# TheBinaryCodeX/RayMarchRenderer

Hardware: AMD Instinct MI355X
Metric: Msamples/sec (pixels×spp) at 1920×1080; PSNR vs GLSL reference (higher is better)
Workload: dtype f32; 1 GPU; C2 Cornell-5 SDF (RayMarch.glsl semantics) 1920x1080 64 spp 4 bounces; config=c2, width=1920, height=1080, spp=64, max_bounces=4, tile=32, tile_order=rows, parallelism=tiles1, frame_streams=2, grid_reserve=64, launch_streams=0

## Files before the change

include/rmr.h:

```cpp
#ifndef RMR_H
#define RMR_H

#include <stddef.h>
#include <stdint.h>
#include "rmr_tables.h"

#ifdef __cplusplus
extern "C" {
#endif

#define RMR_OK          0
#define RMR_E_INVALID  (-1)
#define RMR_E_HIP      (-2)
#define RMR_E_SCENE    (-3)
#define RMR_E_IO       (-4)
#define RMR_E_STATE    (-5)
#define RMR_E_NOMEM    (-6)
#define RMR_E_UNSUPPORTED (-7)

typedef struct rmr_ctx rmr_ctx;

typedef struct rmr_params {
    float   max_dist;
    int32_t max_steps;
// ... 174 lines not shown
int rmr_read_tonemapped(rmr_ctx* ctx, float* rgba, size_t bytes);
void* rmr_tonemapped_device_ptr(rmr_ctx* ctx);
int rmr_read_exposure(rmr_ctx* ctx, double* log2_scale, float* scale);
int rmr_luminance_histogram(rmr_ctx* ctx, int source, uint32_t hist[256], uint64_t* skipped);
int rmr_tonemap_reset(rmr_ctx* ctx);
int rmr_luminance_bins(const float* rgba, size_t n, int32_t* bins);
int rmr_exposure_from_histogram(const uint32_t hist[256], const rmr_tonemap_params* p, double l_prev, double* l_out);
int rmr_tonemap_pixels(const rmr_tonemap_params* p, float scale, const float* rgba, size_t n, float* out);

#define RMR_OUTPUT_BLOOM 4
typedef struct rmr_bloom_params {
    int32_t levels;
    float threshold;
    float clamp;
    float scatter;
    float intensity;
    int32_t reserved[3];
} rmr_bloom_params;
void rmr_default_bloom_params(rmr_bloom_params* p);
int rmr_check_bloom_params(const rmr_bloom_params* p);
int rmr_bloom(rmr_ctx* ctx, int source, const rmr_bloom_params* p);
int rmr_read_bloom(rmr_ctx* ctx, float* rgba, size_t bytes);
void* rmr_bloom_device_ptr(rmr_ctx* ctx);
int rmr_bloom_pixels(const rmr_bloom_params* p, const float* rgba, int w, int h, float* out);

typedef struct rmr_ray {
    float   o[3], time;
    float   d[3], rc;
    int32_t gx, gy;
} rmr_ray;

#define RMR_CAMERA_VIEW 0
#define RMR_CAMERA_THIN_LENS 1
#define RMR_CAMERA_EQUIRECT 2
#define RMR_CAMERA_ORTHO 3
typedef struct rmr_camera_model {
    int32_t model;
    float   aperture;
    float   focus;
    float   width;
    float   height;
} rmr_camera_model;
void rmr_default_camera_model(rmr_camera_model* m);
int rmr_check_camera_model(const rmr_camera_model* m);
int rmr_set_camera_model(rmr_ctx* ctx, const rmr_camera_model* m);
int rmr_get_camera_model(const rmr_ctx* ctx, rmr_camera_model* m);
int rmr_camera_frame(const float view[15], float out[9]);
int rmr_check_rays(const rmr_ray* rays, size_t n);
int rmr_trace_rays(rmr_ctx* ctx, const rmr_ray* rays, size_t n, float* out_rgba);
int rmr_camera_rays(rmr_ctx* ctx, const float* times, uint32_t nspp, int x0, int y0, int x1, int y1, rmr_ray* out);

typedef struct rmr_hit {
    float pos[3], t;
    float n[3], id;
} rmr_hit;
#define RMR_CAST_NORMALS 1
int rmr_cast_rays(rmr_ctx* ctx, const rmr_ray* rays, size_t n, int flags, rmr_hit* out);
int rmr_eval_map(rmr_ctx* ctx, const float* xyz, size_t n, float* out_dist_id);
int rmr_trace_rays_device(rmr_ctx* ctx, const rmr_ray* d_rays, size_t n, float origin_extent, float* d_out_rgba);
int rmr_cast_rays_device(rmr_ctx* ctx, const rmr_ray* d_rays, size_t n, int flags, rmr_hit* d_out);
int rmr_eval_map_device(rmr_ctx* ctx, const float* d_xyz, size_t n, float* d_out_dist_id);
int rmr_query_rejects(rmr_ctx* ctx, uint64_t* out);
int rmr_set_query_grid(rmr_ctx* ctx, int blocks);

int rmr_display(rmr_ctx* ctx, float centre_x, float centre_y, float zoom, float min_x, float min_y, float max_x,
                float max_y, int screen_w, int screen_h, uint8_t* rgba8, size_t nbytes);
int rmr_display_device(rmr_ctx* ctx, float centre_x, float centre_y, float zoom, float min_x, float min_y,
                       float max_x, float max_y, int screen_w, int screen_h, void* rgba8_dev, size_t nbytes);
int rmr_srgb_thresholds(float out[256]);
int rmr_candidate_grid(const float* prims, int n, int n_large, double E, double target, double pad, int32_t idims[5],
                       float geom[12], uint32_t* cells, size_t cells_cap, uint16_t* list, size_t list_cap);
int rmr_set_jit(rmr_ctx* ctx, int mode);
#define RMR_CULL_ESCAPE 1
#define RMR_CULL_NPC 2
#define RMR_CULL_APPROX 4
#define RMR_CULL_EYE 8
int rmr_set_culling(rmr_ctx* ctx, int flags);
#define RMR_INSTR_COUNT_FLOPS 1
int rmr_set_instrument(rmr_ctx* ctx, int flags);
int rmr_jit_compile_scene(int variant, const char* json, size_t len, char* log, size_t loglen);
int rmr_jit_compile_scene_rays(int variant, const char* json, size_t len, char* log, size_t loglen);
int rmr_set_tuning(rmr_ctx* ctx, int shade_threshold, int grid_per_cu, long long samp_budget_bytes);
int rmr_set_grid_reserve(rmr_ctx* ctx, int blocks);
int rmr_trace_samples(rmr_ctx* ctx, const float* times, int x0, int y0, int x1, int y1, uint32_t nspp, float* out);
int rmr_abi_sizes(int32_t* out, int n);

#ifdef __cplusplus
}
#endif
#endif
```

raymarchrenderer_amd/_lib.py:

```python
import ctypes as C
import os

from . import abi

HERE = os.path.dirname(os.path.abspath(__file__))
LIB_PATH = os.path.join(HERE, "librmr.so")
LIB_DIAG_PATH = os.path.join(HERE, "librmr_diag.so")
_libs = {}

EXPORTS = [
    "rmr_create", "rmr_destroy", "rmr_last_error", "rmr_build_info", "rmr_set_stream",
    "rmr_set_image_size", "rmr_get_image_size", "rmr_set_params", "rmr_get_params",
    "rmr_default_params", "rmr_set_view", "rmr_camera_view", "rmr_load_scene_json",
    "rmr_load_scene_tables", "rmr_load_builtin_scene", "rmr_reload", "rmr_render",
    "rmr_render_spp", "rmr_render_tiles", "rmr_read_accum", "rmr_write_accum",
    "rmr_accum_device_ptr", "rmr_bind_accum", "rmr_save_bmp", "rmr_encode_bmp",
    "rmr_save_accum", "rmr_load_accum", "rmr_sync", "rmr_get_stats", "rmr_reset_stats", "rmr_get_section_cycles", "rmr_get_counters", "rmr_get_counters_n", "rmr_set_culling",
    "rmr_set_kernel", "rmr_set_tuning", "rmr_set_grid_reserve", "rmr_trace_samples", "rmr_abi_sizes", "rmr_set_jit", "rmr_set_instrument", "rmr_jit_compile_scene", "rmr_set_env_map",
    "rmr_scene_compile", "rmr_scene_view", "rmr_scene_free", "rmr_display", "rmr_display_device",
    "rmr_srgb_thresholds", "rmr_candidate_grid", "rmr_set_call_batching", "rmr_set_launch_streams", "rmr_get_launch_streams",
    "rmr_default_denoise_params", "rmr_render_guides", "rmr_read_guide", "rmr_guide_device_ptr", "rmr_denoise",
    "rmr_read_denoised", "rmr_denoised_device_ptr", "rmr_set_output_source", "rmr_encode_pfm",
    "rmr_set_error_estimate", "rmr_read_half_accum", "rmr_half_device_ptr", "rmr_tile_error", "rmr_tile_error_images",
    "rmr_default_adaptive_params", "rmr_check_adaptive_params", "rmr_render_adaptive", "rmr_read_sample_counts",
    "rmr_adaptive_select",
    "rmr_default_camera_model", "rmr_check_camera_model", "rmr_set_camera_model", "rmr_get_camera_model",
    "rmr_camera_frame", "rmr_check_rays", "rmr_trace_rays", "rmr_camera_rays", "rmr_jit_compile_scene_rays",
    "rmr_cast_rays", "rmr_eval_map", "rmr_trace_rays_device", "rmr_cast_rays_device", "rmr_eval_map_device",
    "rmr_query_rejects", "rmr_set_query_grid",
    "rmr_default_variance_params", "rmr_check_variance_params", "rmr_denoise_variance", "rmr_read_variance",
    "rmr_variance_device_ptr", "rmr_denoise_variance_images",
    "rmr_default_temporal_params", "rmr_check_temporal_params", "rmr_temporal_view_inverse", "rmr_temporal_accumulate",
    "rmr_temporal_reset", "rmr_read_temporal", "rmr_read_temporal_count", "rmr_temporal_device_ptr", "rmr_temporal_images",
    "rmr_default_tonemap_params", "rmr_check_tonemap_params", "rmr_tonemap", "rmr_read_tonemapped",
    "rmr_tonemapped_device_ptr", "rmr_read_exposure", "rmr_luminance_histogram", "rmr_tonemap_reset",
    "rmr_luminance_bins", "rmr_exposure_from_histogram", "rmr_tonemap_pixels",
    "rmr_default_bloom_params", "rmr_check_bloom_params", "rmr_bloom", "rmr_read_bloom", "rmr_bloom_device_ptr",
    "rmr_bloom_pixels",
]


class RMRError(RuntimeError):
    def __init__(self, code, msg):
        super().__init__("%s (%d): %s" % (abi.ERRORS.get(code, "RMR_E?"), code, msg))
        self.code = code


def build():
    import subprocess
    subprocess.check_call(["make", "-s", "-C", os.path.join(HERE, "csrc"), "-j8"])


def lib(diag=None):
    if diag is None:
        diag = os.environ.get("RMR_LIB", "") == "diag"
    if isinstance(diag, str):
        path = os.path.abspath(diag)
    else:
        path = LIB_DIAG_PATH if diag else LIB_PATH
    if path in _libs:
        return _libs[path]
    if not os.path.exists(path):
        raise RuntimeError("%s not built: run `python -c 'import __graft_entry__ as g; g.build()'` "
                           "(expected at %s)" % (os.path.basename(path), path))
    try:
        import torch
    except ImportError:
        pass
    L = C.CDLL(path)
    vp, fp, ip = C.c_void_p, C.POINTER(C.c_float), C.POINTER(C.c_int)
    dp = C.POINTER(C.c_double)
    sig = {
        "rmr_create": (C.c_int, [C.POINTER(vp), C.c_int]),
        "rmr_destroy": (None, [vp]),
        "rmr_last_error": (C.c_char_p, [vp]),
        "rmr_build_info": (C.c_char_p, []),
        "rmr_set_stream": (C.c_int, [vp, vp]),
        "rmr_set_image_size": (C.c_int, [vp, C.c_int, C.c_int]),
        "rmr_get_image_size": (C.c_int, [vp, ip, ip]),
        "rmr_set_params": (C.c_int, [vp, C.POINTER(abi.Params)]),
        "rmr_get_params": (C.c_int, [vp, C.POINTER(abi.Params)]),
        "rmr_default_params": (None, [C.POINTER(abi.Params)]),
        "rmr_set_view": (C.c_int, [vp, fp, fp, fp, fp, fp]),
        "rmr_camera_view": (None, [dp, dp, C.c_float, C.c_float, fp, fp, fp, fp, fp]),
        "rmr_load_scene_json": (C.c_int, [vp, C.c_int, C.c_char_p, C.c_size_t]),
        "rmr_load_scene_tables": (C.c_int, [vp, C.POINTER(abi.Scene)]),
        "rmr_load_builtin_scene": (C.c_int, [vp, C.c_int]),
        "rmr_reload": (C.c_int, [vp]),
        "rmr_render": (C.c_int, [vp, C.c_float, C.c_float, C.c_float, C.c_float, C.c_float, C.c_uint32]),
        "rmr_render_spp": (C.c_int, [vp, fp, C.c_int, C.c_int, C.c_int, C.c_int, C.c_uint32, C.c_uint32]),
        "rmr_render_tiles": (C.c_int, [vp, fp, C.POINTER(C.c_int32), C.c_int, C.c_int, C.c_uint32, C.c_uint32]),
        "rmr_read_accum": (C.c_int, [vp, fp, C.c_size_t]),
        "rmr_write_accum": (C.c_int, [vp, fp, C.c_size_t]),
        "rmr_accum_device_ptr": (vp, [vp]),
        "rmr_bind_accum": (C.c_int, [vp, vp, C.c_size_t]),
        "rmr_save_bmp": (C.c_int, [vp, C.c_char_p]),
        "rmr_encode_bmp": (C.c_int, [fp, C.c_int, C.c_int, C.c_char_p]),
        "rmr_save_accum": (C.c_int, [vp, C.c_char_p, C.c_uint32]),
        "rmr_load_accum": (C.c_int, [vp, C.c_char_p, C.POINTER(C.c_uint32)]),
        "rmr_sync": (C.c_int, [vp]),
        "rmr_get_stats": (C.c_int, [vp, C.POINTER(abi.Stats)]),
        "rmr_reset_stats": (C.c_int, [vp]),
        "rmr_get_section_cycles": (C.c_int, [vp, C.POINTER(C.c_uint64)]),
        "rmr_get_counters": (C.c_int, [vp, C.POINTER(C.c_uint64)]),
        "rmr_get_counters_n": (C.c_int, [vp, C.POINTER(C.c_uint64), C.c_int]),
        "rmr_set_culling": (C.c_int, [vp, C.c_int]),
        "rmr_set_kernel": (C.c_int, [vp, C.c_int]),
        "rmr_set_tuning": (C.c_int, [vp, C.c_int, C.c_int, C.c_longlong]),
        "rmr_set_grid_reserve": (C.c_int, [vp, C.c_int]),
        "rmr_set_call_batching": (C.c_int, [vp, C.c_int]),
        "rmr_set_launch_streams": (C.c_int, [vp, C.c_int]),
        "rmr_get_launch_streams": (C.c_int, [vp]),
        "rmr_set_jit": (C.c_int, [vp, C.c_int]),
        "rmr_set_instrument": (C.c_int, [vp, C.c_int]),
        "rmr_set_env_map": (C.c_int, [vp, C.c_void_p, C.c_int, C.c_int]),
        "rmr_jit_compile_scene": (C.c_int, [C.c_int, C.c_char_p, C.c_size_t, C.c_char_p, C.c_size_t]),
        "rmr_trace_samples": (C.c_int, [vp, fp, C.c_int, C.c_int, C.c_int, C.c_int, C.c_uint32, fp]),
        "rmr_abi_sizes": (C.c_int, [C.POINTER(C.c_int32), C.c_int]),
        "rmr_scene_compile": (C.c_int, [C.c_int, C.c_char_p, C.c_size_t, C.POINTER(vp), C.c_char_p, C.c_size_t]),
        "rmr_scene_view": (C.c_int, [vp, C.POINTER(abi.Scene)]),
        "rmr_scene_free": (None, [vp]),
        "rmr_display": (C.c_int, [vp] + [C.c_float] * 7 + [C.c_int, C.c_int, C.c_void_p, C.c_size_t]),
        "rmr_display_device": (C.c_int, [vp] + [C.c_float] * 7 + [C.c_int, C.c_int, C.c_void_p, C.c_size_t]),
        "rmr_srgb_thresholds": (C.c_int, [fp]),
        "rmr_candidate_grid": (C.c_int, [fp, C.c_int, C.c_int, C.c_double, C.c_double, C.c_double,
                                         C.POINTER(C.c_int32), fp, C.POINTER(C.c_uint32), C.c_size_t,
                                         C.POINTER(C.c_uint16), C.c_size_t]),
        "rmr_default_denoise_params": (None, [C.POINTER(abi.DenoiseParams)]),
        "rmr_render_guides": (C.c_int, [vp, C.c_int, C.c_int, C.c_int, C.c_int]),
        "rmr_read_guide": (C.c_int, [vp, C.c_int, fp, C.c_size_t]),
        "rmr_guide_device_ptr": (vp, [vp, C.c_int]),
        "rmr_denoise": (C.c_int, [vp, C.POINTER(abi.DenoiseParams)]),
        "rmr_read_denoised": (C.c_int, [vp, fp, C.c_size_t]),
        "rmr_denoised_device_ptr": (vp, [vp]),
        "rmr_set_output_source": (C.c_int, [vp, C.c_int]),
        "rmr_encode_pfm": (C.c_int, [fp, C.c_int, C.c_int, C.c_char_p]),
        "rmr_set_error_estimate": (C.c_int, [vp, C.c_int]),
        "rmr_read_half_accum": (C.c_int, [vp, fp, C.c_size_t]),
        "rmr_half_device_ptr": (vp, [vp]),
        "rmr_tile_error": (C.c_int, [vp, C.c_float, fp, C.c_size_t]),
        "rmr_tile_error_images": (C.c_int, [vp, fp, fp, C.c_int, C.c_int, C.c_float, fp]),
        "rmr_default_adaptive_params": (None, [C.POINTER(abi.AdaptiveParams)]),
        "rmr_check_adaptive_params": (C.c_int, [C.POINTER(abi.AdaptiveParams)]),
        "rmr_render_adaptive": (C.c_int, [vp, fp, C.POINTER(abi.AdaptiveParams), C.POINTER(abi.AdaptiveResult)]),
        "rmr_read_sample_counts": (C.c_int, [vp, C.POINTER(C.c_uint32), C.c_size_t]),
        "rmr_adaptive_select": (C.c_int, [fp, C.c_int, C.c_int, C.c_int, C.c_float, C.POINTER(C.c_uint8)]),
        "rmr_default_camera_model": (None, [C.POINTER(abi.CameraModel)]),
        "rmr_check_camera_model": (C.c_int, [C.POINTER(abi.CameraModel)]),
        "rmr_set_camera_model": (C.c_int, [vp, C.POINTER(abi.CameraModel)]),
        "rmr_get_camera_model": (C.c_int, [vp, C.POINTER(abi.CameraModel)]),
        "rmr_camera_frame": (C.c_int, [fp, fp]),
        "rmr_check_rays": (C.c_int, [C.c_void_p, C.c_size_t]),
        "rmr_trace_rays": (C.c_int, [vp, C.c_void_p, C.c_size_t, fp]),
        "rmr_camera_rays": (C.c_int, [vp, fp, C.c_uint32, C.c_int, C.c_int, C.c_int, C.c_int, C.c_void_p]),
        "rmr_jit_compile_scene_rays": (C.c_int, [C.c_int, C.c_char_p, C.c_size_t, C.c_char_p, C.c_size_t]),
        "rmr_cast_rays": (C.c_int, [vp, C.c_void_p, C.c_size_t, C.c_int, C.c_void_p]),
        "rmr_eval_map": (C.c_int, [vp, fp, C.c_size_t, fp]),
        "rmr_trace_rays_device": (C.c_int, [vp, C.c_void_p, C.c_size_t, C.c_float, C.c_void_p]),
        "rmr_cast_rays_device": (C.c_int, [vp, C.c_void_p, C.c_size_t, C.c_int, C.c_void_p]),
        "rmr_eval_map_device": (C.c_int, [vp, C.c_void_p, C.c_size_t, C.c_void_p]),
        "rmr_query_rejects": (C.c_int, [vp, C.POINTER(C.c_uint64)]),
        "rmr_set_query_grid": (C.c_int, [vp, C.c_int]),
        "rmr_default_variance_params": (None, [C.POINTER(abi.VarianceParams)]),
        "rmr_check_variance_params": (C.c_int, [C.POINTER(abi.VarianceParams)]),
        "rmr_denoise_variance": (C.c_int, [vp, C.POINTER(abi.DenoiseParams), C.POINTER(abi.VarianceParams)]),
        "rmr_read_variance": (C.c_int, [vp, C.c_int, fp, C.c_size_t]),
        "rmr_variance_device_ptr": (vp, [vp, C.c_int]),
        "rmr_denoise_variance_images": (C.c_int, [vp, fp, fp, fp, fp, C.c_int, C.c_int, C.POINTER(abi.DenoiseParams),
                                                  C.POINTER(abi.VarianceParams), fp, fp, fp]),
        "rmr_default_temporal_params": (None, [C.POINTER(abi.TemporalParams)]),
        "rmr_check_temporal_params": (C.c_int, [C.POINTER(abi.TemporalParams)]),
        "rmr_temporal_view_inverse": (C.c_int, [fp, dp]),
        "rmr_temporal_accumulate": (C.c_int, [vp, C.c_int, C.c_float, C.POINTER(abi.TemporalParams)]),
        "rmr_temporal_reset": (C.c_int, [vp]),
        "rmr_read_temporal": (C.c_int, [vp, fp, C.c_size_t]),
        "rmr_read_temporal_count": (C.c_int, [vp, fp, C.c_size_t]),
        "rmr_temporal_device_ptr": (vp, [vp]),
        "rmr_temporal_images": (C.c_int, [vp, fp, fp, fp, fp, fp, fp, fp, fp, fp, C.c_int, C.c_int, C.c_float,
                                          C.POINTER(abi.TemporalParams), fp, fp, fp]),
        "rmr_default_tonemap_params": (None, [C.POINTER(abi.TonemapParams)]),
        "rmr_check_tonemap_params": (C.c_int, [C.POINTER(abi.TonemapParams)]),
        "rmr_tonemap": (C.c_int, [vp, C.c_int, C.POINTER(abi.TonemapParams)]),
        "rmr_read_tonemapped": (C.c_int, [vp, fp, C.c_size_t]),
        "rmr_tonemapped_device_ptr": (vp, [vp]),
        "rmr_read_exposure": (C.c_int, [vp, dp, fp]),
        "rmr_luminance_histogram": (C.c_int, [vp, C.c_int, C.POINTER(C.c_uint32), C.POINTER(C.c_uint64)]),
        "rmr_tonemap_reset": (C.c_int, [vp]),
        "rmr_luminance_bins": (C.c_int, [fp, C.c_size_t, C.POINTER(C.c_int32)]),
        "rmr_exposure_from_histogram": (C.c_int, [C.POINTER(C.c_uint32), C.POINTER(abi.TonemapParams), C.c_double, dp]),
        "rmr_tonemap_pixels": (C.c_int, [C.POINTER(abi.TonemapParams), C.c_float, fp, C.c_size_t, fp]),
        "rmr_default_bloom_params": (None, [C.POINTER(abi.BloomParams)]),
        "rmr_check_bloom_params": (C.c_int, [C.POINTER(abi.BloomParams)]),
# ... 21 lines not shown
```

raymarchrenderer_amd/csrc/rmr_api.cpp:

```cpp
#include <hip/hip_runtime.h>

#include <algorithm>
#include <cfloat>
#include <cmath>
#include <cstddef>
#include <cstdio>
#include <cstdlib>
#include <cstring>
#include <fstream>
#include <initializer_list>
#include <new>
#include <sstream>
#include <string>
#include <thread>
#include <unordered_map>
#include <vector>

#include "../../include/rmr.h"
#include "rmr_internal.h"
#include "accel.hpp"
#include "adaptive.hpp"
#include "rmr_camera.hpp"
#include "rmr_ray_check.h"
#include "rmr_jit.hpp"
#include "scene.hpp"
#include "temporal.hpp"
#include "tonemap.hpp"
#include "bloom.hpp"
#include "stage_state.hpp"

namespace rmr {
hipError_t launch_trace(const KParams& P, int variant, int np, bool prog, bool persistent, int grid, hipStream_t s);
hipError_t launch_fold(const KParams& P, hipStream_t s);
hipError_t launch_trace_rays(const KParams& P, const float4* rays, int variant, int np, bool prog, bool persistent,
                             int grid, hipStream_t s);
int trace_rays_occupancy(int variant, int np, bool prog, int* blocks_per_cu);
hipError_t launch_camera_rays(const KParams& P, const CamParams& C, float4* rays, hipStream_t s);
hipError_t launch_ray_exit(const KParams& P, const float* rays, float* out, int n, hipStream_t s);
hipError_t launch_display(const float4* accum, int img_w, int img_h, float cx, float cy, float zoom, float min_x,
                          float min_y, float max_x, float max_y, int scr_w, int scr_h, uint32_t* rgba8,
                          const float* thr, hipStream_t s);
int trace_occupancy(int variant, int np, bool prog, int* blocks_per_cu);
hipError_t launch_guides(const KParams& P, int np, float4* ray, float4* hit, float4* nrm, hipStream_t s);
hipError_t launch_atrous(const DenoisePass& A, bool tiled, hipStream_t s);
hipError_t launch_fold_half(const KParams& P, float4* half, hipStream_t s);
hipError_t launch_tile_error(const float4* A, const float4* B, int W, int H, float offset, float* out, hipStream_t s);
hipError_t launch_cast_rays(const KParams& P, int np, bool normals, const rmr_ray* rays, uint64_t n, rmr_hit* out,
                            unsigned long long* rejects, unsigned long long* first_bad, int grid_cap, hipStream_t s);
hipError_t launch_eval_map(const KParams& P, int np, const float* xyz, uint64_t n, float* out, int grid_cap, hipStream_t s);
hipError_t launch_pack_rays(const rmr_ray* rays, uint64_t n, uint64_t u0, uint32_t units, float extent, float4* rec,
                            unsigned long long* rejects, unsigned long long* first_bad, hipStream_t s);
hipError_t launch_unpack_rgba(const float4* samp, const float4* rec, float* out, uint32_t cnt, hipStream_t s);
}

using rmr::CompiledScene;
using rmr::KParams;
using rmr::TileXY;

struct EventPair { hipEvent_t a, b, c; };

constexpr int kSlotGridReserve = 32;
constexpr int kDenoiseTiledSteps = 3;
constexpr int kDenoiseVarTiledSteps = 3;

struct rmr_ctx {
    int device = 0;
    int n_cu = 256;
    hipStream_t stream = nullptr;
    bool own_stream = false;
    int W = 1024, H = 1024;
    int pend_W = 1024, pend_H = 1024;
    rmr_params params{};
    float view[15];
    bool view_set = false;
    CompiledScene scene;
    bool scene_loaded = false;
    rmr_prim* d_prims = nullptr;
    rmr_op* d_ops = nullptr;
    float* d_consts = nullptr;
    rmr_material* d_mats = nullptr;
    rmr_spectral* d_spec = nullptr;
    rmr_rm2_consts* d_rm2 = nullptr;
    rmr::DPrim* d_dprims = nullptr;
    rmr::DMat* d_dmats = nullptr;
    rmr::BvhNode* d_bvh = nullptr;
    rmr::SceneAccel accel;
    KParams scene_kp{};
    float* d_esc = nullptr;
    double esc_infl_dev = -1.0;
    float4* d_env = nullptr;
    float* d_srgb_thr = nullptr;
    uint32_t* d_screen = nullptr;
    size_t screen_cap = 0;
    int env_w = 0, env_h = 0;
    uint4* d_grid = nullptr;
    uint16_t* d_grid_list = nullptr;
    int npc_ksel = 0;
    float4* d_accum = nullptr;
    bool accum_external = false;
    float4* d_samp = nullptr;
    size_t samp_cap = 0;
    rmr_camera_model camera{RMR_CAMERA_VIEW, 0.0f, 1.0f, 1.0f, 1.0f};
    float4* d_rays = nullptr;
    size_t rays_cap = 0;
    unsigned long long* d_query = nullptr;
    void* d_qin = nullptr;
    void* d_qout = nullptr;
    size_t qin_cap = 0, qout_cap = 0;
    int query_grid = 0;
    rmr::StageState st;
    float4* d_guide[3] = {nullptr, nullptr, nullptr};
    float4* d_dn[2] = {nullptr, nullptr};
    int output_source = RMR_OUTPUT_ACCUM;
    int dn_tiled_steps = kDenoiseTiledSteps;
    float* d_var[3] = {nullptr, nullptr, nullptr};
    int dnv_tiled_steps = kDenoiseVarTiledSteps;
    float4* d_tcol[2] = {nullptr, nullptr};
    float* d_tn[2] = {nullptr, nullptr};
    float4* d_tguide[2] = {nullptr, nullptr};
    float t_view[15];
    bool t_keep = false;
    float4* d_tm = nullptr;
    uint32_t* d_tm_slab = nullptr;
    rmr::ToneState* d_tm_state = nullptr;
    double* d_tm_lc = nullptr;
    double tm_lc[255];
    int tm_used = 0;
    double tm_ev = 0.0;
    float tm_scale = 1.0f;
    bool tm_fold = false;
    float4* d_bl = nullptr;
    float4* d_bl_pyr = nullptr;
    int bl_tail = rmr::kBloomTailDefault;
    bool est_on = false;
    bool est_valid = false;
    bool rendered = false;
    float4* d_half = nullptr;
    float* d_tile_err = nullptr;
    std::vector<uint32_t> sample_counts;
    struct Slot {
        hipStream_t s = nullptr;
        float4* samp = nullptr;
        size_t cap = 0;
        unsigned long long* queue = nullptr;
        bool queue_dirty = true;
        hipEvent_t done = nullptr, freed = nullptr;
        bool in_use = false;
    };
    std::vector<Slot> slots;
    int launch_streams = 2;
    int slot_reserve = kSlotGridReserve;
    size_t next_slot = 0;
    float4* last_samp = nullptr;
    hipEvent_t trace_end = nullptr;
    struct TileList { std::vector<TileXY> host; TileXY* dev; uint64_t hash; uint64_t used; };
    std::vector<TileList> tile_cache;
    uint64_t tile_clock = 0;
    float* d_times = nullptr;
    float* h_times = nullptr;
    size_t times_cap = 0, times_pos = 0;
    bool queue_dirty = false;
    std::vector<rmr::DeferredCall> deferred;
    uint64_t deferred_units = 0;
    int call_batching = -1;
    unsigned long long* d_queue = nullptr;
    unsigned long long* d_counters = nullptr;
    std::vector<EventPair> pending, pool;
    rmr_stats stats{};
    int kernel_mode = 0;
    int shade_threshold = 16;
    bool shade_auto = true;
    int refill_threshold = -1;
    int lane_slots = -1;
    int park_threshold = 0, slot_threshold = 0;
    int jit_slots = -1;
    int full_threshold = 40 | (8 << 8);
    int cull = RMR_CULL_ESCAPE | RMR_CULL_NPC | RMR_CULL_APPROX | RMR_CULL_EYE;
    int instrument = 0;
    int grid_per_cu = 0;
    int grid_reserve = 0;
    bool diag_no_fold = false;
    int small_chunk = 64;
    int jit_mode = 2;
    uint64_t jit_min_units = (uint64_t)1 << 16;
    bool jit_ready = false;
    bool jit_failed = false;
    rmr::JitKernel jit;
    bool jit_rays_ready = false;
    rmr::JitKernel jit_rays;
    std::string jit_struct_src;
    std::vector<rmr_prim> jit_base;
    std::vector<char> jit_live;
    std::vector<rmr::JitKernel> jit_loaded;
    size_t samp_budget = (size_t)48 << 30;
    std::string err;
    std::unordered_map<const void*, size_t> dev_caps;
};

namespace {

int refill_for(int setting, int shade_t) {
    if (setting > 0) return setting;
    if (setting == 0) return shade_t;
    return std::max(2, shade_t / 2);
}

int fail(rmr_ctx* c, int code, const std::string& m) {
    if (c) c->err = m;
    return code;
}
#define HIPCHK(ctx, expr)                                                                          \
    do {                                                                                           \
        hipError_t e_ = (expr);                                                                    \
        if (e_ != hipSuccess) return fail(ctx, RMR_E_HIP, std::string(#expr ": ") + hipGetErrorString(e_)); \
    } while (0)

template <class T>
int dev_upload(rmr_ctx* c, T** dst, const T* src, size_t n) {
    const size_t bytes = std::max<size_t>(1, n) * sizeof(T);
    size_t& cap = c->dev_caps[(const void*)dst];
    if (!*dst || cap < bytes) {
        if (*dst) {
            HIPCHK(c, hipStreamSynchronize(c->stream));
            (void)hipFree(*dst);
            *dst = nullptr;
        }
        HIPCHK(c, hipMalloc((void**)dst, bytes));
        cap = bytes;
    }
    if (n) {
        HIPCHK(c, hipMemcpyAsync(*dst, src, n * sizeof(T), hipMemcpyHostToDevice, c->stream));
        HIPCHK(c, hipStreamSynchronize(c->stream));
    }
    return RMR_OK;
}

struct Buf {
    void** p;
    size_t bytes;
    template <class T>
    Buf(T** q, size_t b = 0) : p((void**)q), bytes(b) {}
};
int alloc_all(rmr_ctx* c, std::initializer_list<Buf> list, const char* msg) {
    for (const Buf* a = list.begin(); a != list.end(); ++a) {
        if (hipMalloc(a->p, a->bytes) == hipSuccess) continue;
        (void)hipGetLastError();
        *a->p = nullptr;
        for (const Buf* k = list.begin(); k != a; ++k) { (void)hipFree(*k->p); *k->p = nullptr; }
        return fail(c, RMR_E_NOMEM, msg);
    }
    return RMR_OK;
}
void free_all(std::initializer_list<Buf> list) {
    for (const Buf& b : list) { if (*b.p) (void)hipFree(*b.p); *b.p = nullptr; }
}

int read_back(rmr_ctx* c, void* dst, const void* src, size_t bytes) {
// ... 172 lines not shown
    if ((r = dev_upload(c, &c->d_dprims, a.dprims.data(), a.dprims.size()))) return r;
    if (a.map_np == -2 && (r = dev_upload(c, &c->d_bvh, a.nodes.data(), a.nodes.size()))) return r;
    if (a.grid_on) {
        if ((r = dev_upload(c, &c->d_grid, a.grid_cells.data(), a.grid_cells.size()))) return r;
        if ((r = dev_upload(c, &c->d_grid_list, a.grid.list.data(), a.grid.list.size()))) return r;
    }
    a.grid_cells = {};
    a.grid.cells = {};
    a.grid.list = {};
    c->esc_infl_dev = -1.0;
    c->scene_kp = scene_params(c);
    c->st.scene_loaded();
    c->scene_loaded = true;
    c->jit_ready = false;
    c->jit_rays_ready = false;
    c->jit_failed = false;
    c->stats.flops_per_map = s.flops_per_map();
    return RMR_OK;
}

int slots_request(const rmr_ctx* c) {
    if (c->params.separate_channels != 0 || c->params.use_env_tex != 0 || c->params.max_bounces >= (1 << 21)) return 0;
    return c->lane_slots;
}

int ensure_jit(rmr_ctx* c, bool rays = false) {
    const int slots = rays ? 0 : slots_request(c);
    rmr::JitKernel& jk = rays ? c->jit_rays : c->jit;
    bool& ready = rays ? c->jit_rays_ready : c->jit_ready;
    if (ready && (rays || c->jit_slots == slots)) return RMR_OK;
    ready = false;
    if (!rays) c->jit_slots = slots;
    const std::string struct_src = rmr::jit_source(c->scene, c->accel.has_prog, false, c->cull);
    const auto& prims = c->scene.prims;
    if (struct_src != c->jit_struct_src || c->jit_base.size() != prims.size()) {
        c->jit_base = prims;
        c->jit_live.assign(prims.size(), 0);
    } else {
        for (size_t j = 0; j < prims.size(); j++)
            if (std::memcmp(&prims[j], &c->jit_base[j], sizeof(rmr_prim)) != 0) c->jit_live[j] = 1;
    }
    c->jit_struct_src = struct_src;
    const rmr::CacheFacts cache = rmr::cache_kernel_facts(c->accel, c->accel.grid_on);
    rmr::JitFacts facts;
    const std::string src = rmr::jit_source(c->scene, c->accel.has_prog, true, c->cull, &c->jit_live,
                                            c->npc_ksel ? c->npc_ksel : cache.npc_k, cache.npc_spheres, &facts, slots, rays);
    std::vector<char> code;
    std::string key, log;
    std::vector<std::string> opts;
    if (c->instrument & RMR_INSTR_COUNT_FLOPS) opts.push_back("-DRMR_COUNT_FLOPS");
    if (!rmr::jit_compile(src, code, key, log, opts)) {
        c->jit_failed = true;
        return fail(c, RMR_E_HIP, "hipRTC specialisation failed: " + log.substr(0, 2000));
    }
    for (const auto& k : c->jit_loaded) {
        if (k.key == key) {
            jk = k;
            ready = true;
            return RMR_OK;
        }
    }
    rmr::JitKernel k;
    k.key = key;
    if (hipModuleLoadData(&k.module, code.data()) != hipSuccess) {
        c->jit_failed = true;
        return fail(c, RMR_E_HIP, "hipModuleLoadData of the specialised kernel failed (key " + key + ")");
    }
    const char* entry = rays ? "rmr_jit_trace_rays" : "rmr_jit_trace";
    if (hipModuleGetFunction(&k.fn, k.module, entry) != hipSuccess) {
        (void)hipModuleUnload(k.module);
        c->jit_failed = true;
        return fail(c, RMR_E_HIP, std::string(entry) + " missing from the specialised code object (key " + key + ")");
    }
    k.block = 256;
    k.chunk = facts.chunk();
    int b = 0;
    if (hipModuleOccupancyMaxActiveBlocksPerMultiprocessor(&b, k.fn, k.block, 0) != hipSuccess || b <= 0) b = 4;
    k.blocks_per_cu = b;
    k.shade_t = facts.shade_t();
    k.slots = facts.slots;
    k.park_t = facts.park_t();
    k.slot_t = facts.slot_t();
    k.slot_t_small = facts.slot_t_small();
    c->jit_loaded.push_back(k);
    jk = k;
    ready = true;
    return RMR_OK;
}

int ensure_rays(rmr_ctx* c, size_t units) {
    if (units <= c->rays_cap) return RMR_OK;
    if (c->d_rays) {
        HIPCHK(c, hipStreamSynchronize(c->stream));
        (void)hipFree(c->d_rays);
        c->d_rays = nullptr;
        c->rays_cap = 0;
    }
    if (hipMalloc((void**)&c->d_rays, units * rmr::kRayRecordBytes) != hipSuccess) {
        (void)hipGetLastError();
        c->d_rays = nullptr;
        return fail(c, RMR_E_NOMEM, "cannot allocate the ray buffer (" + std::to_string(units * rmr::kRayRecordBytes) +
                                        " bytes; lower the plane budget, rmr_set_tuning)");
    }
    c->rays_cap = units;
    return RMR_OK;
}

int ensure_samp(rmr_ctx* c, size_t n) {
    if (n <= c->samp_cap) return RMR_OK;
    if (c->d_samp) { (void)hipFree(c->d_samp); c->d_samp = nullptr; c->samp_cap = 0; }
    HIPCHK(c, hipMalloc((void**)&c->d_samp, n * sizeof(float4)));
    c->samp_cap = n;
    return RMR_OK;
}


int make_slots(rmr_ctx* c) {
    c->slots.resize(c->launch_streams >= 2 ? (size_t)c->launch_streams : 0);
    c->next_slot = 0;
    for (auto& S : c->slots) {
        if (S.s) continue;
        HIPCHK(c, hipStreamCreateWithFlags(&S.s, hipStreamNonBlocking));
        HIPCHK(c, hipEventCreateWithFlags(&S.done, hipEventDisableTiming));
        HIPCHK(c, hipEventCreateWithFlags(&S.freed, hipEventDisableTiming));
        HIPCHK(c, hipMalloc((void**)&S.queue, rmr::kQueueBytes));
        S.queue_dirty = true;
    }
    return RMR_OK;
}

int slot_prepare(rmr_ctx* c, size_t units, rmr_ctx::Slot** out) {
    int r;
    if (c->slots.empty() || !c->slots[0].s) {
        if ((r = make_slots(c))) return r;
    }
    if (units > c->slots[c->next_slot].cap) {
        for (auto& T : c->slots) {
            if (units <= T.cap) continue;
            if (T.samp) {
                if (T.in_use) HIPCHK(c, hipEventSynchronize(T.freed));
                (void)hipFree(T.samp);
                T.samp = nullptr;
                T.cap = 0;
            }
            HIPCHK(c, hipMalloc((void**)&T.samp, units * sizeof(float4)));
            T.cap = units;
        }
    }
    rmr_ctx::Slot& S = c->slots[c->next_slot];
    c->next_slot = (c->next_slot + 1) % c->slots.size();
    if (S.in_use) HIPCHK(c, hipStreamWaitEvent(S.s, S.freed, 0));
    *out = &S;
    return RMR_OK;
}

int free_slots(rmr_ctx* c) {
    if (c->slots.empty() && !c->trace_end) return RMR_OK;
    const hipError_t e = c->stream ? hipStreamSynchronize(c->stream) : hipSuccess;
    for (auto& S : c->slots) {
        if (S.s) {
            (void)hipStreamSynchronize(S.s);
            (void)hipStreamDestroy(S.s);
        }
        if (S.done) (void)hipEventDestroy(S.done);
        if (S.freed) (void)hipEventDestroy(S.freed);
        if (S.samp) (void)hipFree(S.samp);
// ... 271 lines not shown
    }
    const TileXY* d_tiles = nullptr;
    if (!rl) {
        c->st.accum_changed();
        c->rendered = true;
        if ((r = tile_list(c, tiles, &d_tiles))) return r;
    }
    const size_t plane = rl ? 64 : tiles.size() * 64;
    const rmr::SamplePlan sp = rmr::plan_samples(plane, nspp, c->samp_budget, rays ? 0 : c->launch_streams,
                                                 rays ? sizeof(float4) + rmr::kRayRecordBytes : sizeof(float4));
    const size_t chunk = sp.per_launch;
    if (sp.slotted && c->slots.size() != (size_t)c->launch_streams) {
        if ((r = free_slots(c)) || (r = make_slots(c))) return r;
    }
    KParams P;
    if ((r = view_params(c, P, org_extent))) return r;
    P.x0 = x0; P.y0 = y0; P.x1 = x1; P.y1 = y1;
    P.tiles = d_tiles;
    P.n_tiles = rl ? 1 : (int)tiles.size();

    bool use_jit = false;
    if (c->kernel_mode == 0 && c->jit_mode != 0 && !(c->jit_mode == 2 && c->jit_failed)) {
        if (c->jit_mode == 1 || (uint64_t)chunk * plane >= c->jit_min_units) {
            const int jr = ensure_jit(c, rays);
            if (jr == RMR_OK) use_jit = true;
            else if (c->jit_mode == 1) return jr;
        }
    }
    const rmr::JitKernel& jk = rays ? c->jit_rays : c->jit;
    int bpc = c->grid_per_cu;
    if (bpc <= 0) {
        if (use_jit) bpc = jk.blocks_per_cu;
        else if ((rays ? rmr::trace_rays_occupancy(c->scene.variant, c->accel.map_np, c->accel.has_prog, &bpc)
                       : rmr::trace_occupancy(c->scene.variant, c->accel.map_np, c->accel.has_prog, &bpc)) != 0 || bpc <= 0)
            bpc = 4;
    }
    const int full_grid = c->n_cu * bpc;
    for (uint32_t k0 = 0; k0 < nspp; k0 += (uint32_t)chunk) {
        const uint32_t n = (uint32_t)std::min<size_t>(chunk, nspp - k0);
        rmr_ctx::Slot* S = nullptr;
        if (sp.slotted && c->trace_end && hipEventQuery(c->trace_end) == hipErrorNotReady) {
            if ((r = slot_prepare(c, plane * n, &S))) return r;
            P.samp = S->samp;
            P.queue = S->queue;
        } else {
            if ((r = ensure_samp(c, plane * n))) return r;
            P.samp = c->d_samp;
            P.queue = c->d_queue;
        }
        if (rays && (r = ensure_rays(c, plane * n))) return r;
        const float* d_times = nullptr;
        if (!rl && n > 1 && (r = stage_times(c, times + k0, n, &d_times, S ? S->s : c->stream))) return r;
        c->last_samp = P.samp;
        P.nspp = n;
        P.first_sample = first_sample + k0;
        P.times = d_times;
        P.time1 = rl ? 0.0f : times[k0];
        P.n_units = (uint64_t)n * plane;
        std::vector<float4> h_rays;
        if (rl && rl->d_rays) {
            HIPCHK(c, rmr::launch_pack_rays(rl->d_rays, rl->n, (uint64_t)k0 * 64, (uint32_t)P.n_units, rl->extent, c->d_rays,
                                            c->d_query + kQueryRejects, c->d_query + kQueryFirstBad, c->stream));
        } else if (rl) {
            h_rays.resize(3 * (size_t)P.n_units);
            pack_rays(*rl, (size_t)k0 * 64, h_rays);
            HIPCHK(c, hipMemcpyAsync(c->d_rays, h_rays.data(), h_rays.size() * sizeof(float4), hipMemcpyHostToDevice, c->stream));
        } else if (rays) {
            HIPCHK(c, rmr::launch_camera_rays(P, cam, c->d_rays, c->stream));
        }
        const int reserve = (S && c->grid_reserve == 0) ? c->slot_reserve : c->grid_reserve;
        const rmr::GridPlan gp = rmr::plan_grid(P.n_units, full_grid, reserve, (use_jit ? jk.block : 256) / 64,
                                                use_jit ? jk.chunk : 128, c->small_chunk, P.max_bounces,
                                                c->grid_per_cu, c->kernel_mode);
        P.chunk_units = gp.chunk_units;
        if (c->shade_auto) {
            P.shade_threshold = use_jit ? jk.shade_t : 16;
            P.refill_threshold = refill_for(c->refill_threshold, P.shade_threshold);
        }
        if (use_jit && jk.slots) {
            const int park = c->park_threshold > 0 ? c->park_threshold : jk.park_t;
            const bool small = P.n_units < (uint64_t)gp.grid * (uint64_t)(jk.block / 64) * (uint64_t)jk.chunk *
                                               (uint64_t)rmr::JitFacts::kSlotSmallClaims;
            const int batch = c->slot_threshold > 0 ? c->slot_threshold : (small ? jk.slot_t_small : jk.slot_t);
            P.shade_threshold = park | (batch << 8);
            P.refill_threshold = refill_for(c->refill_threshold, park);
        }
        if ((r = submit_launch(c, P, S, use_jit, gp.grid, rays ? c->d_rays : nullptr, !rl))) return r;
        if (rl && rl->d_rays) {
            const size_t u0 = (size_t)k0 * 64, cnt = std::min<size_t>((size_t)P.n_units, rl->n - u0);
            HIPCHK(c, rmr::launch_unpack_rgba(P.samp, c->d_rays, rl->d_out + 4 * u0, (uint32_t)cnt, c->stream));
        } else if (rl) {
            const size_t u0 = (size_t)k0 * 64, cnt = std::min<size_t>((size_t)P.n_units, rl->n - u0);
            HIPCHK(c, hipMemcpyAsync(rl->out + 4 * u0, P.samp, cnt * sizeof(float4), hipMemcpyDeviceToHost, c->stream));
            HIPCHK(c, hipStreamSynchronize(c->stream));
        }
    }
    return RMR_OK;
}

using rmr::rect_tiles;

const float4* source_image(const rmr_ctx* c, int source, int i) {
    switch (source) {
    case RMR_OUTPUT_DENOISED: return c->d_dn[i];
    case RMR_OUTPUT_TEMPORAL: return c->d_tcol[i];
    case RMR_OUTPUT_TONEMAPPED: return c->d_tm;
    case RMR_OUTPUT_BLOOM: return c->d_bl;
    default: return c->d_accum;
    }
}
const char* const kSourceName[5] = {"", "denoised", "temporal", "tonemapped", "bloom"};
const char* const kSourceCall[5] = {"", "rmr_denoise", "rmr_temporal_accumulate", "rmr_tonemap", "rmr_bloom"};
int no_valid(rmr_ctx* c, int source) {
    return fail(c, RMR_E_STATE, std::string("no valid ") + kSourceName[source] + " image (call " + kSourceCall[source] + ")");
}

int output_image(rmr_ctx* c, const char* who, const float4** out) {
    const int src = c->output_source, i = c->st.readable(src);
    if (i < 0)
        return fail(c, RMR_E_STATE, std::string(who) + ": output source is the " + kSourceName[src] + " image, but none is valid (call " +
                                        kSourceCall[src] + ")");
    *out = source_image(c, src, i);
    return RMR_OK;
}

bool batching_on(const rmr_ctx* c) {
    return c->call_batching > 0 || (c->call_batching < 0 && c->own_stream && !c->accum_external);
}

constexpr uint64_t kDeferredUnitsMax = (uint64_t)1 << 28;
constexpr size_t kDeferredRectsMax = 4096;

int flush_calls(rmr_ctx* c) {
    if (c->deferred.empty()) return RMR_OK;
    std::vector<rmr::DeferredCall> d;
    d.swap(c->deferred);
    c->deferred_units = 0;
    for (const rmr::CallLaunch& l : rmr::group_deferred(d)) {
        const int r = render_tiles(c, rect_tiles(l.x0, l.y0, l.x1, l.y1), l.x0, l.y0, l.x1, l.y1, l.times, l.s0, l.n);
        if (r) return r;
    }
    return RMR_OK;
}

bool flushed(rmr_ctx* c) { return c->deferred.empty() || flush_calls(c) == RMR_OK; }

#if RMR_DIAG
template <class Round>
int timed_rounds(rmr_ctx* c, bool fold, bool run_meter, int n, float* ms, Round round) {
    const size_t px = (size_t)c->W * c->H;
    const int blocks = rmr::lum_hist_blocks(px);
    rmr_tonemap_params tq;
    rmr_default_tonemap_params(&tq);
    const rmr::ToneMeter M = rmr::tonemap_meter(tq);
    hipEvent_t ev[2] = {nullptr, nullptr};
    HIPCHK(c, hipEventCreate(&ev[0]));
    hipError_t e = hipEventCreate(&ev[1]);
    if (e == hipSuccess) e = rmr::launch_lum_hist(c->d_accum, px, c->d_tm_slab, blocks, fold, c->stream);
    for (int i = 0; i < 32 && e == hipSuccess; i++)
        e = rmr::launch_meter(c->d_tm_slab, blocks, c->d_tm_state, c->d_tm_lc, M, run_meter, c->stream);
    if (e == hipSuccess) e = hipEventRecord(ev[0], c->stream);
    for (int i = 0; i < n && e == hipSuccess; i++) e = round();
    if (e == hipSuccess) e = hipEventRecord(ev[1], c->stream);
    const hipError_t es = hipStreamSynchronize(c->stream);
    if (e == hipSuccess) e = es;
    float t = 0.0f;
    if (e == hipSuccess) e = hipEventElapsedTime(&t, ev[0], ev[1]);
// ... 597 lines not shown
                           (float)rgba8[4 * i + 2] / 255.0f, (float)rgba8[4 * i + 3] / 255.0f);
    int r;
    if ((r = dev_upload(c, &c->d_env, t.data(), t.size()))) return r;
    c->env_w = w;
    c->env_h = h;
    return RMR_OK;
}

int rmr_set_jit(rmr_ctx* c, int mode) {
    if (!c || mode < 0 || mode > 2) return RMR_E_INVALID;
    RMR_FLUSH(c);
    c->jit_mode = mode;
    c->jit_failed = false;
    return RMR_OK;
}

int rmr_set_culling(rmr_ctx* c, int flags) {
    if (!c || (flags & ~(RMR_CULL_ESCAPE | RMR_CULL_NPC | RMR_CULL_APPROX | RMR_CULL_EYE))) return RMR_E_INVALID;
    RMR_FLUSH(c);
    if (flags != c->cull) c->jit_ready = c->jit_rays_ready = false;
    c->cull = flags;
    return RMR_OK;
}

static int jit_compile_scene(int variant, const char* json, size_t len, char* log, size_t loglen, bool rays) {
    std::string lg;
    try {
        CompiledScene s = (json && len) ? rmr::compile_scene(std::string(json, len), variant) : rmr::builtin_scene(variant);
        rmr::AccelOptions opt;
        opt.grid = false;
        const rmr::SceneAccel a = rmr::build_scene_accel(s, opt);
        const rmr::CacheFacts cache = rmr::cache_kernel_facts(a, true);
        std::vector<char> code;
        std::string key;
        const bool ok = rmr::jit_compile(
            rmr::jit_source(s, a.has_prog, true, RMR_CULL_ESCAPE | RMR_CULL_NPC | RMR_CULL_APPROX | RMR_CULL_EYE, nullptr,
                            cache.npc_k, cache.npc_spheres, nullptr, -1, rays),
            code, key, lg);
        if (log && loglen) std::snprintf(log, loglen, "%s", ok ? key.c_str() : lg.c_str());
        return ok ? RMR_OK : RMR_E_HIP;
    } catch (const std::exception& e) {
        if (log && loglen) std::snprintf(log, loglen, "%s", e.what());
        return RMR_E_SCENE;
    }
}
int rmr_jit_compile_scene(int variant, const char* json, size_t len, char* log, size_t loglen) {
    return jit_compile_scene(variant, json, len, log, loglen, false);
}
int rmr_jit_compile_scene_rays(int variant, const char* json, size_t len, char* log, size_t loglen) {
    return jit_compile_scene(variant, json, len, log, loglen, true);
}

int rmr_set_instrument(rmr_ctx* c, int flags) {
    if (!c || (flags & ~RMR_INSTR_COUNT_FLOPS)) return RMR_E_INVALID;
    RMR_FLUSH(c);
    if (flags != c->instrument) {
        c->instrument = flags;
        c->jit_ready = c->jit_rays_ready = false;
        c->jit_failed = false;
    }
    return RMR_OK;
}

int rmr_set_tuning(rmr_ctx* c, int shade_threshold, int grid_per_cu, long long samp_budget_bytes) {
    if (!c) return RMR_E_INVALID;
    RMR_FLUSH(c);
    if (shade_threshold > 0) {
        if (shade_threshold & 0xff) {
            c->shade_threshold = std::max(1, std::min(64, shade_threshold & 0xff));
            c->shade_auto = false;
        }
        const int tr = (shade_threshold >> 8) & 0xff;
        if ((shade_threshold & 0xffff) || !(shade_threshold & (1 << 23)))
            c->refill_threshold = tr ? std::min(64, tr) : -1;
        if (shade_threshold & (1 << 23)) {
            const int park = (shade_threshold >> 16) & 0x7f;
            c->lane_slots = park == 127 ? 0 : -1;
            c->park_threshold = park == 127 ? 0 : std::min(64, park);
            c->slot_threshold = std::min(64, (shade_threshold >> 24) & 0x7f);
        }
    }
    if (grid_per_cu >= 0) c->grid_per_cu = grid_per_cu;
    if (samp_budget_bytes > 0) c->samp_budget = (size_t)samp_budget_bytes;
    return RMR_OK;
}

int rmr_set_grid_reserve(rmr_ctx* c, int blocks) {
    if (!c || blocks < 0) return RMR_E_INVALID;
    RMR_FLUSH(c);
    c->grid_reserve = blocks;
    return RMR_OK;
}

int rmr_trace_samples(rmr_ctx* c, const float* times, int x0, int y0, int x1, int y1, uint32_t nspp, float* out) {
    if (!c || !times || !out) return RMR_E_INVALID;
    RMR_FLUSH(c);
    if (!rmr::clamp_rect(c->W, c->H, x0, y0, x1, y1) || nspp == 0) return RMR_OK;
    std::vector<TileXY> tiles = rect_tiles(x0, y0, x1, y1);
    const size_t saved_budget = c->samp_budget;
    const size_t plane = tiles.size() * 64;
    const size_t unit_bytes = sizeof(float4) + (c->camera.model != RMR_CAMERA_VIEW ? rmr::kRayRecordBytes : 0);
    c->samp_budget = std::max(saved_budget, plane * nspp * unit_bytes);
    std::vector<float> keep((size_t)c->W * c->H * 4);
    int r = rmr_read_accum(c, keep.data(), keep.size() * sizeof(float));
    if (!r) r = render_tiles(c, tiles, x0, y0, x1, y1, times, 0, nspp);
    c->samp_budget = saved_budget;
    if (r) return r;
    std::vector<float4> h(plane * nspp);
    HIPCHK(c, hipMemcpyAsync(h.data(), c->last_samp, h.size() * sizeof(float4), hipMemcpyDeviceToHost, c->stream));
    HIPCHK(c, hipStreamSynchronize(c->stream));
    const int w = x1 - x0, hh = y1 - y0;
    const int tx = (w + 7) / 8;
    for (uint32_t k = 0; k < nspp; k++)
        for (int y = 0; y < hh; y++)
            for (int x = 0; x < w; x++) {
                const size_t tile = (size_t)(y / 8) * tx + (x / 8);
                const size_t lane = (size_t)(y % 8) * 8 + (x % 8);
                const float4 v = h[(size_t)k * plane + tile * 64 + lane];
                float* o = out + (((size_t)k * hh + y) * w + x) * 4;
                o[0] = v.x; o[1] = v.y; o[2] = v.z; o[3] = v.w;
            }
    return rmr_write_accum(c, keep.data(), keep.size() * sizeof(float));
}

int rmr_set_camera_model(rmr_ctx* c, const rmr_camera_model* m) {
    if (!c || !m) return RMR_E_INVALID;
    RMR_FLUSH(c);
    if (!rmr::camera_model_ok(*m))
        return fail(c, RMR_E_INVALID, "bad camera model (thin lens: aperture finite >= 0, focus finite > 0; ortho: width, "
                                      "height finite > 0)");
    c->camera = *m;
    return RMR_OK;
}

int rmr_get_camera_model(const rmr_ctx* c, rmr_camera_model* m) {
    if (!c || !m) return RMR_E_INVALID;
    *m = c->camera;
    return RMR_OK;
}

int rmr_trace_rays(rmr_ctx* c, const rmr_ray* rays, size_t n, float* out_rgba) {
    if (!c || (n && (!rays || !out_rgba))) return RMR_E_INVALID;
    RMR_FLUSH(c);
    int r;
    if ((r = launch_precheck(c))) return r;
    if (c->params.separate_channels != 0)
        return fail(c, RMR_E_STATE, "rmr_trace_rays with separate_channels set: a caller's ray has no channel passes");
    if (n >= ((size_t)1 << 37)) return fail(c, RMR_E_INVALID, "rmr_trace_rays: too many rays");
    const long long bad = rmr::first_bad_ray(rays, n);
    if (bad >= 0)
        return fail(c, RMR_E_INVALID, "rmr_trace_rays: ray " + std::to_string(bad) + " fails rmr_check_rays");
    if (n == 0) return RMR_OK;
    HIPCHK(c, hipSetDevice(c->device));
    const RayList rl{rays, n, out_rgba, nullptr, nullptr, 0.0f};
    return render_tiles(c, std::vector<TileXY>(), 0, 0, 0, 0, nullptr, 0, 0, &rl);
}

int rmr_camera_rays(rmr_ctx* c, const float* times, uint32_t nspp, int x0, int y0, int x1, int y1, rmr_ray* out) {
    if (!c || (nspp && (!times || !out))) return RMR_E_INVALID;
    RMR_FLUSH(c);
    if (!rmr::clamp_rect(c->W, c->H, x0, y0, x1, y1) || nspp == 0) return RMR_OK;
    HIPCHK(c, hipSetDevice(c->device));
    if (!c->view_set) default_view(c);
    const rmr_camera_model& m = c->camera;
    rmr::CamParams cam{};
    cam.model = m.model;
// ... 1050 lines not shown
```

raymarchrenderer_amd/csrc/rmr_internal.h:

```cpp
#pragma once
#ifndef __HIPCC_RTC__
#include <stdint.h>
#endif
#include "../../include/rmr_tables.h"

namespace rmr {

struct TileXY { int32_t x, y; };

struct DPrim {
    float c[3];
    float r[3];
    int32_t type;
    float mat_id;
};

enum MatKind : int32_t {
    MAT_NONE = 0,
    MAT_DIFFUSE = 1,
    MAT_EMISSION = 2,
    MAT_PROGRAM = 3,
};
struct DMat {
    int32_t kind;
    float c[3];
    float p[3];
    float gray1;
};

struct BvhNode {
    float lo[3];
    int32_t first;
    float hi[3];
    int32_t count;
    int32_t skip;
    int32_t pad[3];
};

constexpr size_t kQueueBytes = 8192;
constexpr int kQueueWordStride = 32;

constexpr int kCounterSlots = 32;
constexpr int kCntOverflow = 16;
constexpr int kCntProfClaim = 17;
constexpr int kCntProfRays = 18;
constexpr int kCntProfUhits = 19;
constexpr int kCntProfUhitsCheap = 20;
constexpr int kCntProfFullLanes = 21;
constexpr int kCntProfOuter = 22;
constexpr int kCntProfPark = 23;
constexpr int kCntProfParkOvf = 24;
constexpr int kCntProfLostFin = 25;
constexpr int kCntProfLostWait = 26;
constexpr int kCntProfBatchEv = 27;
constexpr int kCntProfLostIdle = 28;
constexpr int kCntProfLostIdleExh = 29;
constexpr int kCntProfReadyWait = 30;

struct KParams {
    const rmr_prim* prims;
    const rmr_op* ops;
    const float* consts;
    const rmr_material* mats;
    const rmr_spectral* spec;
    const rmr_rm2_consts* rm2;
    const DPrim* dprims;
    const DMat* dmats;
    const BvhNode* bvh;
    int32_t n_nodes;
    float am_dmax;
    const uint4* grid;
    const uint16_t* grid_list;
    float grid_lo[3];
    float grid_inv;
    int32_t grid_dim[3];
    float grid_dimf[3];
    int32_t grid_n_large;
    float grid_sbox[6];
    float bvh_margin;
    float am_r2;
    float npc_eps0;
    float cert_k;
    int32_t esc_on;
    int32_t eye_step;
    const float* esc_boxes;
    int32_t n_esc;
    int32_t full_threshold;
    int32_t n_prims;
    int32_t n_mats;
    int32_t v2_begin, v2_end;
    rmr_spectral spec_sky;
    float sky[3];
    const float4* env;
    int32_t env_w, env_h, use_env;
    float rm2_light[3];
    float rm2_light_power;
    int32_t rm2_node_id;
    float max_dist, step_mult;
    int32_t max_steps, max_bounces, separate_channels;
    float eye[3], r00[3], r01[3], r10[3], r11[3];
    int32_t W, H;
    float dr01[3], dr11[3];
    float Wf, Hf;
    float env_wf[4];
    float eye_xy;
    int32_t x0, y0, x1, y1;
    const TileXY* tiles;
    int32_t n_tiles;
    uint32_t nspp;
    uint32_t first_sample;
    const float* times;
    float time1;
    uint64_t n_units;
    uint32_t chunk_units;
    float4* samp;
    float4* accum;
    unsigned long long* queue;
    unsigned long long* counters;
    int32_t flops_static;
    int32_t transc_static;
    int32_t shade_threshold;
    int32_t refill_threshold;
};

struct DenoisePass {
    const float4* in;
// ... 78 lines not shown
```

raymarchrenderer_amd/csrc/rmr_jit.cpp:

```cpp
#include "rmr_jit.hpp"

#include "../../include/rmr.h"

#include <hip/hiprtc.h>

#include <atomic>
#include <cmath>
#include <cstdio>
#include <cstring>
#include <cstdlib>
#include <fstream>
#include <map>
#include <mutex>
#include <sstream>
#include <sys/stat.h>
#include <thread>
#include <unistd.h>

#include "rmr_jit_src.inc"

namespace rmr {
namespace {

std::string flit(float v) {
// ... 1 lines not shown
    std::snprintf(b, sizeof b, "%af", (double)v);
    return b;
}
std::string v3lit(const float* c) { return "v3(" + flit(c[0]) + ", " + flit(c[1]) + ", " + flit(c[2]) + ")"; }
bool am_packable(float id) { return std::fabs(id) < 32768.0f && std::floor(id) == id; }
float am_pack_host(float id, int j) {
    uint32_t b;
    std::memcpy(&b, &id, 4);
    b |= (uint32_t)j;
    float r;
    std::memcpy(&r, &b, 4);
    return r;
}

uint64_t fnv1a(const std::string& s, uint64_t h = 1469598103934665603ull) {
    for (unsigned char ch : s) {
        h ^= ch;
        h *= 1099511628211ull;
    }
    return h;
}

const char* kOptions[] = {"--offload-arch=gfx950", "-O3", "-std=c++17", "-ffp-contract=off", "-Wno-unused-function",
                          "-fno-slp-vectorize", "-DRMR_MANDELBULB_INLINE=1",
#ifdef RMR_PROFILE
                          "-DRMR_PROFILE",
#endif
#define RMR_STR2(x) #x
#define RMR_STR(x) RMR_STR2(x)
#ifdef RMR_FAST_WAVES
                          "-DRMR_FAST_WAVES=" RMR_STR(RMR_FAST_WAVES),
#endif
#ifdef RMR_NPC_K
                          "-DRMR_NPC_K=" RMR_STR(RMR_NPC_K),
#endif
#ifdef RMR_GENERAL_WAVES
                          "-DRMR_GENERAL_WAVES=" RMR_STR(RMR_GENERAL_WAVES),
#endif
};
constexpr int kNumOptions = sizeof(kOptions) / sizeof(kOptions[0]);

std::mutex g_mu;

void write_cache(const std::string& dir, const std::string& path, const std::vector<char>& code) {
    std::string acc;
    for (size_t i = 1; i <= dir.size(); i++) {
        if (i == dir.size() || dir[i] == '/') {
            acc = dir.substr(0, i);
            mkdir(acc.c_str(), 0755);
        }
    }
    static std::atomic<unsigned> seq{0};
    const std::string tmp = path + ".tmp" + std::to_string((long)getpid()) + "." +
                            std::to_string(std::hash<std::thread::id>()(std::this_thread::get_id())) + "." +
                            std::to_string(seq.fetch_add(1));
    std::ofstream f(tmp, std::ios::binary);
    if (f && f.write(code.data(), (std::streamsize)code.size())) {
        f.close();
        std::rename(tmp.c_str(), path.c_str());
    }
}
std::map<std::string, std::vector<char>> g_code;

std::string cache_dir() {
    if (const char* d = std::getenv("RMR_JIT_CACHE")) return d;
    if (const char* h = std::getenv("HOME")) return std::string(h) + "/.cache/rmr-jit";
    return "";
}

}

namespace {
std::string opnd(const CompiledScene& s, int ref, bool allow_p) {
    if (ref == RMR_OPND_NONE) return "v3s(0.0f)";
    if (allow_p && ref == RMR_OPND_P) return "p";
    if (RMR_OPND_IS_CONST(ref)) return v3lit(&s.consts[3 * (size_t)RMR_OPND_CONST_INDEX(ref)]);
    if (ref >= 0) return "nv" + std::to_string(ref);
    return "v3s(0.0f)";
}
constexpr size_t kMaxInlinePrims = 32;
constexpr int kSlotsDefault = 1;
constexpr int kBatchProbesDefault = 1;
constexpr int kSlotOverflowDefault = 1;

std::string var_decls() {
    std::string d = "    V3 nv0 = v3s(0.0f)";
    for (int i = 1; i < RMR_MAX_VARS; i++) d += ", nv" + std::to_string(i) + " = v3s(0.0f)";
    return d + ";\n";
}
}

std::string jit_source(const CompiledScene& s, bool prog, bool bake, int cull_flags, const std::vector<char>* live,
                       int npc_k, bool npc_spheres, JitFacts* facts, int slots, bool rays) {
    std::ostringstream o;
    if (rays) slots = 0;
    o << "// generated by rmr_jit.cpp for one scene\n";
    o << "#define RMR_NT_PLANES " << ((s.variant == RMR_VARIANT_RM2 || s.prims.size() > kMaxInlinePrims) ? 1 : 0) << "\n";
    if (npc_k == 1 && s.prims.size() > kMaxInlinePrims) o << "#define RMR_NPC_K 1\n";
    if (npc_spheres && s.prims.size() > kMaxInlinePrims) o << "#define RMR_NPC_SPHERES 1\n";
    if (s.prims.size() > kMaxInlinePrims) {
        o << "#define RMR_NPC_NPRIMS " << s.prims.size() << "\n";
        o << "#define RMR_NPC_DP_LDS " << (s.prims.size() <= 256 ? 1 : 0) << "\n";
        bool simple_q = true;
        for (const rmr_prim& q : s.prims) simple_q = simple_q && (q.type == RMR_PRIM_SPHERE || q.type == RMR_PRIM_BOX);
        const bool cache_q = simple_q && (cull_flags & RMR_CULL_NPC) && !prog && s.variant != RMR_VARIANT_RM2;
        if (cache_q && s.prims.size() <= 256) o << "#define RMR_NPC_TAB_SOA 1\n";
        bool packed = s.prims.size() <= 256;
        for (const rmr_prim& q : s.prims) packed = packed && am_packable(q.mat_id);
        if (packed) o << "#define RMR_NPC_PACKED 1\n";
    }
    o << "#include \"rmr_trace.h\"\nnamespace rmr {\n";
    for (size_t j = 0; j < s.prims.size(); j++) {
        const rmr_prim& q = s.prims[j];
        if (q.type != RMR_PRIM_PROGRAM) continue;
        o << "RMR_D float jit_obj_" << j << "(V3 p) {\n" << var_decls();
        for (int k = q.prog_begin; k < q.prog_end; k++) {
            const rmr_op& op = s.ops[(size_t)k];
            if (op.out[0] < 0) continue;
            o << "    nv" << op.out[0] << " = obj_node(" << op.code << ", " << opnd(s, op.in[0], true) << ", "
              << opnd(s, op.in[1], true) << ", " << opnd(s, op.in[2], true) << ");\n";
        }
        o << "    return nv" << q.dist_var << ".x;\n}\n";
    }
    bool general = false;
    bool cache_map = false;
    bool simple = true;
    for (const rmr_prim& q : s.prims) simple = simple && (q.type == RMR_PRIM_SPHERE || q.type == RMR_PRIM_BOX);
    bool cert = false;
    bool sched_mc = false;
    int fast_waves = 0;
    bool am_direct = false;
    const bool inline_map = s.prims.size() <= kMaxInlinePrims;
    bool has_mb = false;
    for (const rmr_prim& q : s.prims) has_mb = has_mb || q.type == RMR_PRIM_MANDELBULB;
    int cull = has_mb ? 1 : 0;
    if (const char* e = RMR_ENV("RMR_JIT_CULL")) cull = std::atoi(e);
    if (const char* e = RMR_ENV("RMR_JIT_BAKE")) bake = std::atoi(e) != 0;
    if (!inline_map) {
        general = !simple;
        const bool ho = !prog && s.variant != RMR_VARIANT_RM2;
        const int np = simple ? ((cull_flags & RMR_CULL_NPC) && ho ? -3 : -2) : -1;
        cache_map = np == -3;
        o << "struct JitMap : TableMap<" << np << "> {};\n";
    } else {
    const bool approx = (cull_flags & RMR_CULL_APPROX) && simple && s.prims.size() >= 4 && cull == 0;
    sched_mc = !prog;
    am_direct = approx && s.variant == RMR_VARIANT_RM1;
    fast_waves = (!prog && (s.variant == RMR_VARIANT_RM3 || (approx && s.variant == RMR_VARIANT_RM1))) ? 7 : 0;
    auto loaded = [&](size_t j) { return !bake || (live && j < live->size() && (*live)[j]); };
    bool any_loaded = false;
    for (size_t j = 0; j < s.prims.size(); j++) any_loaded = any_loaded || loaded(j);
    std::vector<std::string> stmt(s.prims.size());
    int n_mb = 0;
    size_t mb_j = 0;
    std::string mb_c, mb_r, mb_m;
    for (size_t j = 0; j < s.prims.size(); j++) {
        const rmr_prim& q = s.prims[j];
        const std::string mid = flit(q.mat_id);
        std::ostringstream st;
        if (loaded(j) && (q.type == RMR_PRIM_SPHERE || q.type == RMR_PRIM_BOX || q.type == RMR_PRIM_MANDELBULB)) {
            const std::string J = std::to_string(j);
            const std::string c = "v3(pr[" + J + "].c[0], pr[" + J + "].c[1], pr[" + J + "].c[2])";
            const std::string r = "v3(pr[" + J + "].r[0], pr[" + J + "].r[1], pr[" + J + "].r[2])";
            const std::string m = "pr[" + J + "].mat_id";
            if (q.type == RMR_PRIM_SPHERE) st << "        opu(d, sd_sphere(p, " << c << ", pr[" << J << "].r[0]), " << m << ");\n";
            else if (q.type == RMR_PRIM_BOX) st << "        opu(d, sd_box(p, " << c << ", " << r << "), " << m << ");\n";
            else {
                general = true;
                st << "        opu(d, sd_mandelbulb(p, " << c << ", " << r << ", P.counters), " << m << ");\n";
                n_mb++; mb_j = j; mb_c = c; mb_r = r; mb_m = m;
            }
            stmt[j] = st.str();
            continue;
        }
        switch (q.type) {
        case RMR_PRIM_SPHERE:
            if (j > 0 && (cull & 2))
                st << "        opu_sphere_culled(d, p, " << v3lit(q.c) << ", " << flit(q.r[0]) << ", " << mid << ");\n";
            else
                st << "        opu(d, sd_sphere(p, " << v3lit(q.c) << ", " << flit(q.r[0]) << "), " << mid << ");\n";
            break;
        case RMR_PRIM_BOX:
            if (j > 0 && (cull & 1))
                st << "        opu_box_culled(d, p, " << v3lit(q.c) << ", " << v3lit(q.r) << ", " << mid << ");\n";
            else
                st << "        opu(d, sd_box(p, " << v3lit(q.c) << ", " << v3lit(q.r) << "), " << mid << ");\n";
            break;
        case RMR_PRIM_MANDELBULB:
            general = true;
            st << "        opu(d, sd_mandelbulb(p, " << v3lit(q.c) << ", " << v3lit(q.r) << ", P.counters), " << mid << ");\n";
            n_mb++; mb_j = j; mb_c = v3lit(q.c); mb_r = v3lit(q.r); mb_m = mid;
            break;
        default:
            general = true;
            st << "        opu(d, jit_obj_" << j << "(p), " << mid << ");\n";
            break;
        }
        stmt[j] = st.str();
    }
    bool stepped = n_mb == 1;
    if (const char* e = RMR_ENV("RMR_JIT_STEP")) stepped = stepped && std::atoi(e) != 0;
    const char* pr_decl = any_loaded ? "        CPrim* pr = (CPrim*)P.prims;\n" : "";
    cert = approx && !prog && s.variant != RMR_VARIANT_RM2 && s.prims.size() <= 256;
    if (const char* e = RMR_ENV("RMR_JIT_CERT")) cert = cert && std::atoi(e) != 0;
    for (const rmr_prim& q : s.prims) cert = cert && am_packable(q.mat_id);
    o << "struct JitMap {\n    static constexpr bool kCache = false;\n    static constexpr bool kCounts = false;\n"
      << "    static constexpr bool kStepped = " << (stepped ? "RMR_MB_STEPPED" : "false") << ";\n"
      << "    static constexpr bool kCert = " << (cert ? "true" : "false") << ";\n";
    if (stepped) {
        o << "    static RMR_D void begin(const KParams& P, V3 p, MBStep& s) {\n" << pr_decl
          << "        const V3 prm = " << mb_r << ";\n"
          << "        mb_begin(s, p - " << mb_c << ", (int)prm.y, prm.z);\n    }\n"
          << "    static RMR_D bool step(const KParams& P, MBStep& s) {\n" << pr_decl
          << "        const V3 prm = " << mb_r << ";\n"
          << "        return mb_step(s, prm.x, (int)prm.y, prm.z, P.counters);\n    }\n"
          << "    static RMR_D V2 finish_exact(const KParams& P, V3 p, float db) {\n" << pr_decl
          << "        V2 d = v2(P.max_dist, -1.0f);\n";
        for (size_t j = 0; j < mb_j; j++) o << stmt[j];
        o << "        opu(d, db, " << mb_m << ");\n";
        for (size_t j = mb_j + 1; j < s.prims.size(); j++) o << stmt[j];
        o << "        return d;\n    }\n";
        o << "    static RMR_D V2 finish(const KParams& P, V3 p, const MBStep& s) {\n" << pr_decl
          << "        return finish_exact(P, p, mb_de(s.r, s.dr));\n    }\n";
    }
    o << "    static RMR_D V2 " << (approx ? "exact" : "eval") << "(const KParams& P, V3 p) {\n" << pr_decl
      << "        V2 d = v2(P.max_dist, -1.0f);\n";
    for (size_t j = 0; j < s.prims.size(); j++) o << stmt[j];
    o << "        return d;\n    }\n";
    if (approx) {
        if (cert)
            o << "    static RMR_D V2 eval(const KParams& P, V3 p) {\n        int w;\n        bool c;\n"
              << "        return eval_c(P, p, w, c);\n    }\n"
              << "    static RMR_D V2 eval_c(const KParams& P, V3 p, int& w, bool& cert) {\n        AMin m;\n";
        else
            o << "    static RMR_D V2 eval(const KParams& P, V3 p) {\n        AMin m;\n";
        if (any_loaded) o << "        CPrim* pr = (CPrim*)P.prims;\n";
        size_t nbox = 0;
        for (const rmr_prim& q : s.prims) nbox += q.type == RMR_PRIM_BOX;
        bool bkey = nbox >= 2;
        if (const char* e = RMR_ENV("RMR_JIT_BKEY")) bkey = bkey && std::atoi(e) != 0;
        bool first = true;
        for (int pass = bkey ? 0 : 1; pass < 2; pass++) {
            if (pass == 1 && bkey) {
                o << "        am_boxes(m, b);\n";
                first = false;
            }
            bool bfirst = true;
            for (size_t j = 0; j < s.prims.size(); j++) {
                const rmr_prim& q = s.prims[j];
                if (bkey && (pass == 0) != (q.type == RMR_PRIM_BOX)) continue;
                const std::string J = std::to_string(j);
                const bool lit = !loaded(j);
                const std::string c = lit ? v3lit(q.c) : "v3(pr[" + J + "].c[0], pr[" + J + "].c[1], pr[" + J + "].c[2])";
                const std::string r = lit ? v3lit(q.r) : "v3(pr[" + J + "].r[0], pr[" + J + "].r[1], pr[" + J + "].r[2])";
                const std::string r0 = lit ? flit(q.r[0]) : "pr[" + J + "].r[0]";
                const std::string m = !cert ? (lit ? flit(q.mat_id) : "pr[" + J + "].mat_id")
                                            : (lit ? flit(am_pack_host(q.mat_id, (int)j)) : "am_pack(pr[" + J + "].mat_id, " + J + ")");
                if (pass == 0) {
                    if (bfirst) o << "        BMin b;\n";
                    o << "        bm_box" << (bfirst ? "0" : "") << "(b, p, " << c << ", " << r << ", " << m << ");\n";
                    bfirst = false;
                    continue;
                }
                const char* f0 = first ? "0" : "";
                first = false;
                if (q.type == RMR_PRIM_SPHERE) o << "        am_sphere" << f0 << "(m, p, " << c << ", " << r0 << ", " << m << ");\n";
                else o << "        am_box" << f0 << "(m, p, " << c << ", " << r << ", " << m << ");\n";
            }
        }
        const std::string r2 = !any_loaded ? flit(2.0f * max_sphere_radius(s)) : std::string("P.am_r2");
        o << "        V2 d = " << (cert ? "am_result_packed" : "am_result") << "(P, m);\n"
          << "        const bool amb = !am_unique(m, " << r2 << ") | am_far(P, m);\n";
        if (cert) o << "        w = am_w_of(m.id);\n        cert = am_normal_cert(P, m);\n";
        bool ambcount = false;
        if (const char* e = RMR_ENV("RMR_JIT_AMBCOUNT")) ambcount = std::atoi(e) != 0;
        if (ambcount) {
            o << "        const uint64_t bal = __ballot(amb);\n"
              << "        if (bal) {\n            if (amb) d = exact(P, p);\n"
              << "            const float sm_ = p.x + p.y + p.z;\n"
              << "            const uint64_t bn = __ballot(amb && !(sm_ == sm_)), bt = __ballot(amb && m.s2 == m.a);\n"
              << "            const uint64_t bs = __ballot(amb && fabsf(m.a) < 0.01f), bl = __ballot(amb && m.l2 > 0.0f && m.l2 < 0x1p-96f);\n"
              << "            if (__lane_id() == __ffsll((unsigned long long)bal) - 1) {\n"
              << "                atomicAdd(P.counters + 4, (unsigned long long)__popcll(bal));\n"
              << "                atomicAdd(P.counters + 5, 1ull);\n"
              << "                atomicAdd(P.counters + 6, (unsigned long long)__popcll(bn));\n"
              << "                atomicAdd(P.counters + 7, (unsigned long long)__popcll(bt));\n"
              << "                atomicAdd(P.counters + 9, (unsigned long long)__popcll(bs));\n"
              << "                atomicAdd(P.counters + 10, (unsigned long long)__popcll(bl));\n            }\n"
              << "            if (bt && __lane_id() == __ffsll((unsigned long long)bt) - 1) {   // one sample tie point\n"
              << "                atomicExch(P.counters + 11, (unsigned long long)__float_as_uint(p.x));\n"
              << "                atomicExch(P.counters + 12, (unsigned long long)__float_as_uint(p.y));\n"
              << "                atomicExch(P.counters + 13, (unsigned long long)__float_as_uint(p.z));\n"
              << "                atomicExch(P.counters + 14, (unsigned long long)__float_as_uint(m.a));\n"
              << "                atomicExch(P.counters + 15, (unsigned long long)__float_as_uint(m.id));\n            }\n        }\n";
        } else {
            o << "        if (amb) d = exact(P, p);\n";
        }
        o << "        return d;\n    }\n";
    }
    o << "};\n";
    }
    if (prog) {
        for (size_t m = 0; m < s.materials.size(); m++) {
            const rmr_material& mt = s.materials[m];
            if (!mt.defined) continue;
            o << "RMR_D void jit_mat_" << m << "(const KParams& P, Lane& L, V3& oc, V3& od, V3& oi, V3& oh) {\n"
              << var_decls();
            for (int k = mt.prog_begin; k < mt.prog_end; k++) {
                const rmr_op& op = s.ops[(size_t)k];
                o << "    {\n        const V3 in[7] = {";
                for (int i = 0; i < 7; i++) o << (i ? ", " : "") << opnd(s, op.in[i], false);
                o << "};\n        V3 o0, o1, o2, o3;\n        mat_node(P, L, " << op.code << ", in, o0, o1, o2, o3);\n";
                for (int w = 0; w < 4; w++)
                    if (op.out[w] >= 0) o << "        nv" << op.out[w] << " = o" << w << ";\n";
                o << "    }\n";
            }
            if (mt.color_var >= 0) o << "    oc = nv" << mt.color_var << ";\n";
            if (mt.dir_var >= 0) o << "    od = nv" << mt.dir_var << ";\n";
            if (mt.inside_var >= 0) o << "    oi = nv" << mt.inside_var << ";\n";
            if (mt.hit_var >= 0) o << "    oh = nv" << mt.hit_var << ";\n";
            o << "}\n";
        }
        o << "struct JitMats : TableMats {\n    static RMR_D void run(const KParams& P, Lane& L, int m, V3& oc, V3& od, V3& oi, V3& oh) {\n"
          << "        switch (m) {\n";
        for (size_t m = 0; m < s.materials.size(); m++)
            if (s.materials[m].defined)
                o << "        case " << m << ": jit_mat_" << m << "(P, L, oc, od, oi, oh); break;\n";
        o << "        default: break;\n        }\n    }\n};\n";
    }
    const bool v2mats = s.variant == RMR_VARIANT_RM2 && s.v2_end > s.v2_begin;
    if (v2mats) {
        o << "struct JitV2Mats : TableMats {\n    static RMR_D void run_v2(const KParams& P, Lane& L, V3 pos, V3 pdir, V3 N, "
             "V3 t0, V3 t1, V3 t2, V3& mat_color, V3& new_dir, bool& will_break) {\n"
          << var_decls();
        auto slot = [](int i) { return "nv" + std::to_string(i); };
        for (int k = s.v2_begin; k < s.v2_end; k++) {
            const rmr_op& op = s.ops[(size_t)k];
            const bool o0 = op.out[0] >= 0 && op.out[0] < RMR_MAX_VARS, o1 = op.out[1] >= 0 && op.out[1] < RMR_MAX_VARS;
            o << "    {\n";
            switch (op.code) {
            case RMR_OP_V2_DIFFUSE:
                o << "        const V3 dd = mat_mul(t0, t1, t2, diffuse_sample(L));\n";
                if (o0) o << "        " << slot(op.out[0]) << " = dd;\n";
                if (o1) o << "        " << slot(op.out[1]) << " = " << opnd(s, op.in[0], false) << ";\n";
                break;
            case RMR_OP_V2_GLOSSY: {
                const float rough = RMR_OPND_IS_CONST(op.in[1]) ? s.consts[3 * (size_t)RMR_OPND_CONST_INDEX(op.in[1])] : 0.0f;
                o << "        const V3 dd = mat_mul(t0, t1, t2, glossy_sample(L, pdir, N, " << flit(rough) << "));\n";
                if (o0) o << "        " << slot(op.out[0]) << " = dd;\n";
                if (o1) o << "        " << slot(op.out[1]) << " = " << opnd(s, op.in[0], false) << ";\n";
                break;
            }
            case RMR_OP_V2_FRESNEL:
                if (o0)
                    o << "        " << slot(op.out[0])
                      << " = v3s(pow5(1.0f - clampf(dot(N, pdir), 0.0f, 1.0f)) * 0.96f + 0.04f);\n";
                break;
            case RMR_OP_V2_MIX:
                o << "        const float r = lrand(L, v2(pos.x, pos.z));\n"
                  << "        const bool second = r <= " << opnd(s, op.in[4], false) << ".x;\n"
                  << "        const V3 dsel = second ? " << opnd(s, op.in[2], false) << " : " << opnd(s, op.in[0], false) << ";\n"
                  << "        const V3 rsel = second ? " << opnd(s, op.in[3], false) << " : " << opnd(s, op.in[1], false) << ";\n";
                if (o0) o << "        " << slot(op.out[0]) << " = dsel;\n";
                if (o1) o << "        " << slot(op.out[1]) << " = rsel;\n";
                break;
            default:
                break;
            }
            o << "    }\n";
        }
        o << "    v2_tail(L, pos, nv1, nv0, mat_color, new_dir, will_break);\n    }\n};\n";
    }
    o << "}  // namespace rmr\n";
    const bool slots_ok = cert && s.variant == RMR_VARIANT_RM1 && !prog && inline_map;
    if (slots < 0) {
        slots = kSlotsDefault;
        if (const char* e = RMR_ENV("RMR_JIT_SLOTS")) slots = std::atoi(e) != 0;
    }
    const bool slots_on = slots_ok && slots != 0;
    if (slots_on) fast_waves = 6;
    const int var = s.variant;
    const std::string waves = cache_map ? std::string("(RMR_CACHE_WAVES)")
                                        : std::string("(rmr::trace_waves<") + std::to_string(var) + ", " +
                                              (general ? "true" : "false") + ", " + (prog ? "true" : "false") + ">())";
    bool sched_occ = cache_map;
    if (const char* e = RMR_ENV("RMR_JIT_SCHED")) {
        sched_mc = sched_mc && std::atoi(e) != 0;
        sched_occ = sched_occ && std::atoi(e) != 0;
    }
    int postsched = 0;
    if (const char* e = RMR_ENV("RMR_JIT_POSTSCHED")) postsched = std::atoi(e) != 0;
    if (sched_mc)
        o << "//@opts -mllvm --amdgpu-sched-strategy=max-memory-clause -mllvm -enable-post-misched=" << postsched << "\n";
    if (sched_occ) o << "//@opts -mllvm --amdgpu-sched-strategy=iterative-maxocc\n";
    if (rays) {
        o << "extern \"C\" __global__ __launch_bounds__(256, " << waves
          << ") void rmr_jit_trace_rays(rmr::KParams P, const float4* rays) {\n"
          << "    rmr::trace_main<" << var << ", rmr::JitMap, true, "
          << (prog ? "true, rmr::JitMats" : (v2mats ? "false, rmr::JitV2Mats" : "false, rmr::TableMats")) << ", (RMR_RAY_SRC != 0)>(P, rays);\n}\n";
    } else {
    o << "extern \"C\" __global__ __launch_bounds__(256, " << waves << ") void rmr_jit_trace(rmr::KParams P) {\n"
      << "    rmr::trace_main<" << var << ", rmr::JitMap, true, "
      << (prog ? "true, rmr::JitMats" : (v2mats ? "false, rmr::JitV2Mats" : "false")) << ">(P);\n}\n";
    }
    std::string src = o.str();
    if (facts) {
        facts->variant = var;
        facts->cache = cache_map;
        facts->general = general;
        facts->prog = prog;
        facts->cert = cert;
        facts->slots_ok = slots_ok;
        facts->slots = slots_on;
    }
    if (rays) src.insert(src.find('\n') + 1, "#define RMR_RAY_SRC 1\n");
    if (slots_on) src.insert(src.find('\n') + 1, "#define RMR_LANE_SLOTS 1\n");
    int bprobes = kBatchProbesDefault;
    if (const char* e = RMR_ENV("RMR_JIT_BPROBES")) bprobes = std::atoi(e) != 0;
    if (slots_on && bprobes) src.insert(src.find('\n') + 1, "#define RMR_BATCH_PROBES 1\n");
    int overflow = kSlotOverflowDefault;
    if (const char* e = RMR_ENV("RMR_JIT_OVERFLOW")) overflow = std::atoi(e) != 0;
    if (slots_on && overflow) src.insert(src.find('\n') + 1, "#define RMR_SLOT_OVERFLOW 1\n");
    if (facts) facts->overflow = slots_on && overflow != 0;
    if (am_direct) src.insert(src.find('\n') + 1, "#ifndef RMR_AM_DIRECT\n#define RMR_AM_DIRECT 1\n#endif\n");
    if (sched_mc && fast_waves)
        src.insert(src.find('\n') + 1, "#ifndef RMR_FAST_WAVES\n#define RMR_FAST_WAVES " + std::to_string(fast_waves) + "\n#endif\n");
    if (prog)
        src.insert(src.find('\n') + 1, "#ifndef RMR_PROG_WAVES\n#define RMR_PROG_WAVES 6\n#endif\n");
    return src;
}

bool jit_compile(const std::string& src, std::vector<char>& code, std::string& key, std::string& log,
                 const std::vector<std::string>& caller_opts) {
    uint64_t h = fnv1a(src);
    for (int i = 0; i < kJitHeaderCount; i++) h = fnv1a(kJitHeaders[i], h);
    for (int i = 0; i < kNumOptions; i++) h = fnv1a(kOptions[i], h);
    std::vector<std::string> extra(caller_opts);
    if (const char* e = RMR_ENV("RMR_JIT_OPTS")) {
        std::istringstream is(e);
        for (std::string w; is >> w;) extra.push_back(w);
    }
    for (size_t at = src.find("//@opts "); at != std::string::npos; at = src.find("//@opts ", at + 1)) {
        const size_t e = src.find('\n', at);
        std::istringstream is(src.substr(at + 8, e == std::string::npos ? std::string::npos : e - at - 8));
        for (std::string w; is >> w;) extra.push_back(w);
    }
    for (const auto& w : extra) h = fnv1a(w, h);
    {
        int maj = 0, mnr = 0;
        (void)hiprtcVersion(&maj, &mnr);
        h = fnv1a("hiprtc " + std::to_string(maj) + "." + std::to_string(mnr) + " " + std::to_string(HIP_VERSION), h);
    }
    char kb[32];
    std::snprintf(kb, sizeof kb, "%016llx", (unsigned long long)h);
    key = kb;
    if (const char* d = RMR_ENV("RMR_JIT_DUMP")) {
        std::ofstream f(std::string(d) + "/" + key + ".hip");
        f << src;
    }
    const std::string dir = cache_dir();
    const std::string path = dir.empty() ? "" : dir + "/" + key + ".hsaco";
    bool hit = false;
    {
        std::lock_guard<std::mutex> lk(g_mu);
        auto it = g_code.find(key);
        if (it != g_code.end()) {
            code = it->second;
            hit = true;
        }
    }
    if (hit) {
        struct stat st;
        if (!path.empty() && stat(path.c_str(), &st) != 0) write_cache(dir, path, code);
        return true;
    }
    if (!path.empty()) {
        std::ifstream f(path, std::ios::binary);
        if (f) {
            std::vector<char> c((std::istreambuf_iterator<char>(f)), std::istreambuf_iterator<char>());
            if (!c.empty()) {
                code = c;
                std::lock_guard<std::mutex> lk(g_mu);
                g_code[key] = c;
                return true;
            }
        }
    }
    hiprtcProgram prog;
    if (hiprtcCreateProgram(&prog, src.c_str(), "rmr_jit_scene.hip", kJitHeaderCount, kJitHeaders, kJitHeaderNames) !=
        HIPRTC_SUCCESS) {
        log = "hiprtcCreateProgram failed";
        return false;
    }
    std::vector<const char*> opts(kOptions, kOptions + kNumOptions);
    for (const auto& w : extra) opts.push_back(w.c_str());
    const hiprtcResult rc = hiprtcCompileProgram(prog, (int)opts.size(), opts.data());
    size_t ls = 0;
    hiprtcGetProgramLogSize(prog, &ls);
    if (ls > 1) {
        std::string l(ls, '\0');
        hiprtcGetProgramLog(prog, &l[0]);
        log = l;
    }
    if (rc != HIPRTC_SUCCESS) {
        hiprtcDestroyProgram(&prog);
        if (log.empty()) log = hiprtcGetErrorString(rc);
// ... 17 lines not shown
```

raymarchrenderer_amd/csrc/rmr_jit.hpp:

```cpp
#pragma once
#include <hip/hip_runtime.h>

#include <string>
#include <vector>

#include "scene.hpp"

#ifndef RMR_DIAG
#define RMR_DIAG 0
#endif
#if RMR_DIAG
#define RMR_ENV(name) std::getenv(name)
#else
#define RMR_ENV(name) ((const char*)nullptr)
#endif

namespace rmr {

struct JitKernel {
    std::string key;
    hipModule_t module = nullptr;
    hipFunction_t fn = nullptr;
    int blocks_per_cu = 0;
    int shade_t = 16;
    int block = 256;
    int chunk = 128;
    bool slots = false;
    int park_t = 0, slot_t = 0;
    int slot_t_small = 0;
};

struct JitFacts {
    int variant = 0;
    bool cache = false, general = false, prog = false, cert = false;
    bool slots_ok = false, slots = false;
    bool overflow = false;
    int chunk() const { return (cache || slots) ? 64 : 128; }
    int park_t() const { return 8; }
    int slot_t() const { return overflow ? 48 : 32; }
    int slot_t_small() const { return 32; }
    static constexpr int kSlotSmallClaims = 64;
    int shade_t() const {
        if (variant == RMR_VARIANT_RM1 && general && !prog) return 10;
        if (prog || cache || cert) return 20;
        return 16;
    }
};

std::string jit_source(const CompiledScene& s, bool prog, bool bake = true, int cull = 7,
                       const std::vector<char>* live = nullptr, int npc_k = 2, bool npc_spheres = false,
                       JitFacts* facts = nullptr, int slots = -1, bool rays = false);
bool jit_compile(const std::string& src, std::vector<char>& code, std::string& key, std::string& log,
                 const std::vector<std::string>& opts = {});

}
```

raymarchrenderer_amd/csrc/rmr_trace.h:

```cpp
#pragma once
#ifndef __HIPCC_RTC__
#include <hip/hip_runtime.h>
#endif
#include "rmr_math.h"
#include "rmr_internal.h"
#include "rmr_slot_rule.h"

namespace rmr {

typedef const __attribute__((address_space(4))) rmr_prim CPrim;
typedef const __attribute__((address_space(4))) rmr_op COp;
typedef const __attribute__((address_space(4))) float CFloat;
typedef const __attribute__((address_space(4))) rmr_material CMat;
typedef const __attribute__((address_space(4))) DPrim CDPrim;

#define PI_F 3.14159274101257324219f

enum Phase : int {
    PH_MARCH = 0,
    PH_NORMAL = 1,
    PH_SHADOW = 2,
    PH_IDLE = 3,
    PH_RESTART = 4,
    PH_HIT = 5,
    PH_MISS = 6,
    PH_NEE = 7,
};

struct Lane {
    uint32_t unit;
    float gxt, gyt, rc;
    V3 o, d;
    float t;
    int ctr;
    V3 hit;
    float mid;
    V3 nrm;
    V3 color;
    int chan, bounces;
    bool inside;
    float time;
    V3 fin;
    uint32_t wl;
    float power;
    int phase;
    int cw, cw2;
    float cs, cta;
    float texit;
    V3 e;
};
RMR_D void init_probe(Lane& L) { L.e = v3s(-0.0f); }
template <bool HO> RMR_D V3& hitref(Lane& L) {
    if constexpr (HO) return L.o;
    else return L.hit;
}
template <bool HO> RMR_D const V3& hitref(const Lane& L) {
    if constexpr (HO) return L.o;
    else return L.hit;
}
template <int VAR, bool PROG> constexpr bool hit_in_origin() { return VAR != RMR_VARIANT_RM2 && !PROG; }

#ifdef RMR_COUNT_FLOPS
RMR_D void count_work(unsigned long long* cnt, uint64_t lanes, uint64_t flops_per_lane, uint64_t transc_per_lane,
                      uint64_t mb_flops_per_lane = 0) {
    const uint64_t m = __ballot(1);
    if (cnt && lanes && __lane_id() == __ffsll((unsigned long long)m) - 1) {
        atomicAdd(cnt + 11, (unsigned long long)(lanes * flops_per_lane));
        if (transc_per_lane) atomicAdd(cnt + 12, (unsigned long long)(lanes * transc_per_lane));
        if (mb_flops_per_lane) atomicAdd(cnt + 13, (unsigned long long)(lanes * mb_flops_per_lane));
    }
}
#define RMR_COUNT(cnt, lanes, f, t) count_work((cnt), (lanes), (f), (t))
#define RMR_COUNT_MB(cnt, lanes, power)                                                            \
    ((power) == 8.0f ? (RMR_MB_POLY ? count_work((cnt), (lanes), 51, 2, 51) : count_work((cnt), (lanes), 59, 2, 59)) \
                     : count_work((cnt), (lanes), 27, 10, 27))
#else
#define RMR_COUNT(cnt, lanes, f, t) ((void)0)
#define RMR_COUNT_MB(cnt, lanes, power) ((void)0)
#endif
RMR_D uint64_t active_lanes() { return (uint64_t)__popcll(__ballot(1)); }

RMR_D float rand_step(float gxt, float gyt, float& rc, V2 co) {
    co.x = fmaf(gxt, rc, co.x);
    co.y = fmaf(gyt, rc, co.y);
    float dt = dot2(co, v2(12.9898f, 78.233f));
    float sn = mod_314(dt);
    rc = fractf(det_sin(sn) * 43758.5453f);
    return rc;
}
// ... 1817 lines not shown
    L.cta = L.t;
}


RMR_D float opq() {
    float v;
    __asm__ volatile("; lane init %0" : "=v"(v));
    return v;
}
RMR_D V3 opq3() { return v3(opq(), opq(), opq()); }
RMR_D void lane_define(Lane& L) {
    L.unit = __float_as_uint(opq());
    L.gxt = opq(); L.gyt = opq(); L.rc = opq();
    L.o = opq3(); L.d = opq3();
    L.t = opq();
    L.ctr = __float_as_int(opq());
    L.hit = opq3();
    L.mid = opq();
    L.nrm = opq3();
    L.color = opq3();
    L.chan = __float_as_int(opq()); L.bounces = __float_as_int(opq());
    L.inside = false;
    L.time = opq();
    L.fin = opq3();
    L.wl = __float_as_uint(opq());
    L.power = opq();
    L.cw = __float_as_int(opq()); L.cw2 = __float_as_int(opq());
    L.cs = opq(); L.cta = opq(); L.texit = opq();
    L.e = opq3();
}
RMR_D bool is_active(int ph) { return (uint32_t)ph <= (uint32_t)PH_SHADOW; }
RMR_D bool is_shade(int ph) { return ph >= PH_HIT; }

#ifndef RMR_FAST_WAVES
#define RMR_FAST_WAVES 8
#endif
#ifndef RMR_GENERAL_WAVES
#define RMR_GENERAL_WAVES 8
#endif
#ifndef RMR_CACHE_WAVES
#define RMR_CACHE_WAVES 6
#endif
#ifndef RMR_PROG_WAVES
#define RMR_PROG_WAVES 1
#endif
#ifndef RMR_RM2_WAVES
#define RMR_RM2_WAVES 1
#endif
template <int VAR, bool GENERAL, bool PROG>
constexpr int trace_waves() {
    return PROG ? RMR_PROG_WAVES
                : (VAR == RMR_VARIANT_RM2 ? RMR_RM2_WAVES : (GENERAL ? RMR_GENERAL_WAVES : RMR_FAST_WAVES));
}

#define RMR_MARCH_POINT(L) (HO ? march_point<HO>(L) : ((L.phase == PH_NORMAL) ? probe_point<HO>(L) : vfma(L.d, L.t, L.o)))
#ifndef RMR_CHUNK
#define RMR_CHUNK 128
#endif
#ifndef RMR_QUEUE_PARTS
#define RMR_QUEUE_PARTS 32
#endif
#ifndef RMR_QUEUE_SEQ
#define RMR_QUEUE_SEQ 1
#endif
#define RMR_QUEUE_STRIDE 32
static_assert(RMR_QUEUE_STRIDE == kQueueWordStride, "fold_main zeroes the counters at this stride");
static_assert(RMR_QUEUE_PARTS >= 1 && RMR_QUEUE_PARTS <= 64 && RMR_QUEUE_PARTS * RMR_QUEUE_STRIDE * 4 <= (int)kQueueBytes,
              "queue counters: one per lane of the scan");
#ifndef RMR_CHUNK_CACHE
#define RMR_CHUNK_CACHE 64
#endif
#ifndef RMR_LANE_SLOTS
#define RMR_LANE_SLOTS 0
#endif
#ifndef RMR_CHUNK_SLOTS
#define RMR_CHUNK_SLOTS 64
#endif
#ifndef RMR_BATCH_PROBES
#define RMR_BATCH_PROBES 0
#endif
#ifndef RMR_SLOT_OVERFLOW
#define RMR_SLOT_OVERFLOW 0
#endif
#ifndef RMR_EYE_CHUNK
#define RMR_EYE_CHUNK 1
#endif
typedef uint32_t WCount;
template <int VAR, class MAP, bool PERSIST, bool PROG, class MATS = TableMats, bool RAYS = false>
RMR_D void trace_main(const KParams& P, const float4* rays = nullptr) {
    constexpr bool HO = hit_in_origin<VAR, PROG>();
    constexpr bool CERT = HO && (MAP::kCert || (MAP::kCache && RMR_NPC_K == 1 && RMR_CACHE_CERT));
    Lane L;
    lane_define(L);
    L.phase = PH_IDLE;
    init_probe(L);
    MBStep mbs{};
    mbs.i = -1;
    mbs.fin = false;
    WCount maps = 0, iters = 0, shades = 0, fulls = 0, shaded = 0, bmaps = 0, ovfs = 0;
    constexpr bool SLOTS = RMR_LANE_SLOTS && PERSIST && VAR == RMR_VARIANT_RM1 && CERT && MAP::kCert && !MAP::kCache &&
                           !MAP::kStepped && !RAYS;
    constexpr bool BP = SLOTS && RMR_BATCH_PROBES;
    constexpr bool EYEC = SLOTS && RMR_EYE_CHUNK;
    constexpr bool OVF = SLOTS && RMR_SLOT_OVERFLOW;
    constexpr uint32_t CHUNK = MAP::kCache ? RMR_CHUNK_CACHE : (SLOTS ? RMR_CHUNK_SLOTS : RMR_CHUNK);
    const uint32_t n_units = (uint32_t)P.n_units;
    const uint32_t CK = P.chunk_units - 1u < CHUNK ? P.chunk_units : CHUNK;
    uint32_t rnext = 0, rend = 0;
    const uint32_t n_chunks = (n_units + CK - 1) / CK;
    auto part_begin = [&](uint32_t q) -> uint32_t {
        return (uint32_t)(((uint64_t)n_chunks * q) / (uint32_t)RMR_QUEUE_PARTS) * CK;
    };
    uint32_t part = blockIdx.x % (uint32_t)RMR_QUEUE_PARTS, tried = 0;
    const uint32_t q_seq = n_chunks < gridDim.x * 16u ? (uint32_t)RMR_QUEUE_SEQ : (uint32_t)RMR_QUEUE_PARTS;
    bool exhausted = false;
    if (!PERSIST) {
        const uint32_t u = blockIdx.x * blockDim.x + threadIdx.x;
        if (u < n_units) begin_trace<VAR, HO, RAYS>(P, L, u, true, rays);
        exhausted = true;
    }
    const int T = P.shade_threshold, TR = P.refill_threshold;
    const int PK = T & 0xff, T2 = (T >> 8) & 0xff;
    int sst = 0;
    uint32_t nev = 0;
    const bool eye1 = HO && !MAP::kCache && !RAYS && P.eye_step != 0;
    V2 meye = v2(0.0f, 0.0f);
    if (eye1) {
        meye = MAP::eval(P, v3(P.eye[0], P.eye[1], P.eye[2]));
        meye = v2(__int_as_float(__builtin_amdgcn_readfirstlane(__float_as_int(meye.x))),
                  __int_as_float(__builtin_amdgcn_readfirstlane(__float_as_int(meye.y))));
    }
    float eye_t1 = 0.0f;
    if (EYEC && eye1) {
        const float t1 = fmaf(meye.x, P.step_mult, 0.0f);
        if (meye.x >= 0.001f && P.max_steps > 1 && t1 > 0.0f && t1 < P.max_dist) eye_t1 = t1;
        eye_t1 = __int_as_float(__builtin_amdgcn_readfirstlane(__float_as_int(eye_t1)));
    }
#ifdef RMR_PROFILE
    uint64_t cyc[4] = {0, 0, 0, 0};
    uint64_t full_lanes = 0;
    uint64_t cyc_claim = 0, cyc_rays = 0;
    uint64_t uhits = 0, uhits_cheap = 0;
    uint64_t n_outer = 0, n_park = 0, n_park_ovf = 0, lost_fin = 0, lost_wait = 0, batch_ev = 0;
    uint64_t lost_idle = 0, lost_idle_exh = 0, ready_wait = 0;
    const uint64_t c_begin = __builtin_amdgcn_s_memtime();
#define RMR_STAMP(v) const uint64_t v = __builtin_amdgcn_s_memtime()
#else
#define RMR_STAMP(v)
#endif
    __shared__ ChunkRayT<RAYS> s_ray[4][CHUNK];
    __shared__ int s_tab[4][CERT ? 64 : 1];
    constexpr bool kStash = MAP::kCache && HO;
    __shared__ float s_cold[kStash ? kColdWords : 1][kStash ? 256 : 1];
    __shared__ float s_slot[SLOTS ? kSlotWords : 1][SLOTS ? 256 : 1];
    __shared__ float4 s_dp[MAP::kCache ? 2 * RMR_NPC_LDS_MAX : 1];
#ifndef RMR_SEED_LDS
#define RMR_SEED_LDS 1
#endif
    constexpr bool kSeeds = MAP::kStepped && PERSIST && RMR_SEED_LDS;
    __shared__ float s_rng[kSeeds ? 3 : 1][4][kSeeds ? 64 : 1];
    const bool dp_lds = MAP::kCache && (RMR_NPC_DP_LDS >= 0 ? RMR_NPC_DP_LDS == 1 : P.n_prims <= RMR_NPC_LDS_MAX);
    if (dp_lds) {
        if constexpr (kNpcPacked) {
            for (int i = (int)threadIdx.x; i < P.n_prims; i += (int)blockDim.x) {
                float4 a = ((const float4*)P.dprims)[2 * i], b = ((const float4*)P.dprims)[2 * i + 1];
                npc_pack_entry(a, b);
                s_dp[kTabStep * i] = a;
                s_dp[kTabStep * i + kTabHi] = b;
            }
        } else {
            for (int i = (int)threadIdx.x; i < 2 * P.n_prims; i += (int)blockDim.x)
                s_dp[kTabStep * (i >> 1) + (i & 1) * kTabHi] = ((const float4*)P.dprims)[i];
        }
        __syncthreads();
    }
#define RMR_PRIM_DIST(k, p, mid, j) (dp_lds ? prim_dist_tab(s_dp + kTabStep * (k), p, mid, j) : prim_dist(P, k, p, mid, j))
    static_assert(!RMR_NPC_TAB_SOA || MAP::kCache, "an SoA table kernel reads dtab as the LDS copy only");
#define RMR_DTAB (dp_lds ? (const float4*)s_dp : (const float4*)P.dprims)
    const int wv = __builtin_amdgcn_readfirstlane((threadIdx.x >> 6) & 3);
    uint32_t chunk_base = 0;
#ifdef RMR_WAVE_TIMES
    unsigned long long t_exh = 0;
    if (lane_now() == 0) atomicMax(P.counters + 9, ~(unsigned long long)__builtin_amdgcn_s_memrealtime());
#endif
    for (;;) {
        RMR_STAMP(c0);
        bool fresh = false;
        uint32_t fu = 0;
        if constexpr (SLOTS) {
            const bool tk = L.phase == PH_IDLE && sst == 2;
            if (__ballot(tk)) {
                if (tk) {
                    {
                        const int st = (wv << 6) + (int)lane_now();
                        slot_start_ray(s_slot, st, L, slot_read_ray(s_slot, st));
                    }
                    sst = 0;
                }
            }
        }
        if (PERSIST && !exhausted) {
            uint64_t idle = __ballot(L.phase == PH_IDLE);
            uint64_t act0 = __ballot(is_active(L.phase));
            if (idle && (__popcll(idle) >= TR || act0 == 0)) {
                if (rnext >= rend) {
                    unsigned int base = 0;
#ifdef RMR_PROFILE
                    const uint64_t q0 = __builtin_amdgcn_s_memtime();
#endif
                    for (;;) {
                        const uint32_t pb = part_begin(part), pe = part_begin(part + 1);
                        unsigned int off = 0;
                        if (lane_now() == 0) off = atomicAdd((unsigned int*)P.queue + RMR_QUEUE_STRIDE * part, CK);
                        off = __builtin_amdgcn_readfirstlane(off);
                        if (off < pe - pb) {
                            base = pb + off;
                            rend = n_units - base > CK ? base + CK : n_units;
                            break;
                        }
                        if (++tried < q_seq) {
                            part = part + 1 == (uint32_t)RMR_QUEUE_PARTS ? 0 : part + 1;
                            continue;
                        }
                        if (q_seq >= (uint32_t)RMR_QUEUE_PARTS) {
                            exhausted = true;
                            break;
                        }
                        const uint32_t q = lane_now();
                        bool left = false;
                        if (q < (uint32_t)RMR_QUEUE_PARTS) {
                            const unsigned int c = __hip_atomic_load((unsigned int*)P.queue + RMR_QUEUE_STRIDE * q,
                                                                     __ATOMIC_RELAXED, __HIP_MEMORY_SCOPE_AGENT);
                            left = c < part_begin(q + 1) - part_begin(q);
                        }
                        const uint64_t lm = __ballot(left);
                        if (lm == 0) {
                            exhausted = true;
                            break;
                        }
                        uint64_t m = lm;
                        for (int k = (int)((blockIdx.x * 4u + (uint32_t)wv + tried) % (uint32_t)__popcll(lm)); k > 0; k--)
                            m &= m - 1;
                        part = (uint32_t)__builtin_ctzll(m);
                    }
                    rnext = base;
#ifdef RMR_PROFILE
                    const uint64_t q1 = __builtin_amdgcn_s_memtime();
                    cyc_claim += q1 - q0;
#endif
#ifdef RMR_WAVE_TIMES
                    if (exhausted && lane_now() == 0) {
                        const unsigned long long te = __builtin_amdgcn_s_memrealtime();
                        t_exh = te;
                        atomicMax(P.counters + 11, ~te);
                        atomicMax(P.counters + 10, te);
                    }
#endif
                    if (!exhausted) {
                        chunk_base = base;
                        for (uint32_t sl = lane_now(); sl < CK; sl += 64) {
                            if (base + sl < rend) {
// ... 125 lines not shown
                    RMR_STAMP(f1);
                    cyc[3] += f1 - f0;
                    full_lanes += (uint64_t)nf;
#endif
                }
#ifdef RMR_NPC_CHECK
                if (done) {
                    const V2 ex = map_bvh(P, p);
                    if (__float_as_uint(ex.x) != __float_as_uint(m.x) || __float_as_uint(ex.y) != __float_as_uint(m.y))
                        printf("NPC mismatch unit %u ph %d ctr %d t %a cta %a p (%a %a %a) m (%a %a) exact (%a %a) ok %d "
                               "cw %d cw2 %d F %a cs %a\n",
                               L.unit, L.phase, L.ctr, L.t, L.cta, p.x, p.y, p.z, m.x, m.y, ex.x, ex.y, (int)ok, L.cw, L.cw2,
                               F, L.cs);
                }
#endif
                if (done) {
                    if (L.phase == PH_NORMAL) normal_update(L, m.x);
                    else march_update<HO, true>(P, L, m, 0, false, p);
                }
                const uint64_t dm = __ballot(done);
                maps += (WCount)__popcll(dm);
                iters += dm ? 1 : 0;
                const uint64_t sm = __ballot(is_shade(L.phase));
                go = __ballot(is_active(L.phase)) && __popcll(sm) < T;
            }
            if constexpr (kStash) {
                if (amask) {
                    __asm__ volatile("" ::: "memory");
                    cold_get<VAR>(s_cold, (int)threadIdx.x, L);
                }
            }
        } else if constexpr (MAP::kStepped) {
          if (amask) {
            if (is_active(L.phase) && mbs.i < 0) MAP::begin(P, RMR_MARCH_POINT(L), mbs);
            uint32_t lmaps = 0, liters = 0;
            for (;;) {
                if (is_active(L.phase) && !mbs.fin) mbs.fin = MAP::step(P, mbs);
                liters++;
                const uint64_t fm = __ballot(is_active(L.phase) && mbs.fin);
                const uint64_t rm = __ballot(is_active(L.phase) && !mbs.fin);
                if (fm && (!rm || __popcll(fm) >= RMR_MB_FIN)) {
#ifdef RMR_MB_STATS
                    {
                        const bool fin_l = is_active(L.phase) && mbs.fin;
                        const bool nrm_l = L.phase == PH_NORMAL;
                        uint32_t it_m = (fin_l && !nrm_l) ? (uint32_t)mbs.i : 0u, it_n = (fin_l && nrm_l) ? (uint32_t)mbs.i : 0u;
                        for (int o = 32; o > 0; o >>= 1) {
                            it_m += (uint32_t)__shfl_xor((int)it_m, o);
                            it_n += (uint32_t)__shfl_xor((int)it_n, o);
                        }
                        const uint64_t bm_ = __ballot(fin_l && !nrm_l), bn_ = __ballot(fin_l && nrm_l);
                        if (lane_now() == 0) {
                            atomicAdd(P.counters + 9, (unsigned long long)__popcll(bm_));
                            atomicAdd(P.counters + 10, (unsigned long long)it_m);
                            atomicAdd(P.counters + 12, (unsigned long long)__popcll(bn_));
                            atomicAdd(P.counters + 13, (unsigned long long)it_n);
                            atomicAdd(P.counters + 11, (unsigned long long)liters);
                            atomicAdd(P.counters + 15, 1ull);
                        }
                        liters = 0;
                    }
#endif
                    if (is_active(L.phase) && mbs.fin) {
                        if constexpr (!MAP::kCounts)
                            RMR_COUNT(P.counters, active_lanes(), (uint64_t)P.flops_static, (uint64_t)P.transc_static);
                        const V2 m = MAP::finish(P, RMR_MARCH_POINT(L), mbs);
                        if (L.phase == PH_NORMAL) normal_update(L, m.x);
                        else march_update<HO>(P, L, m);
                        mbs.i = -1;
                        if (is_active(L.phase)) MAP::begin(P, RMR_MARCH_POINT(L), mbs);
                    }
                    lmaps += (uint32_t)__popcll(fm);
                    const uint64_t sm = __ballot(is_shade(L.phase));
                    const uint64_t am = __ballot(is_active(L.phase));
                    if (!am || __popcll(sm) >= T) break;
                }
            }
            maps += (WCount)__builtin_amdgcn_readfirstlane(lmaps);
            iters += (WCount)__builtin_amdgcn_readfirstlane(liters);
          }
        } else if (amask) {
            uint64_t am = amask;
            uint32_t lmaps = 0, liters = 0;
            const int TL = SLOTS ? __popcll(__ballot(is_shade(L.phase))) + PK : T;
#ifdef RMR_PROFILE
            const uint64_t wait0 = __ballot(is_shade(L.phase));
            uint64_t sm0 = wait0;
#endif
            for (;;) {
#ifdef RMR_PROFILE
                lost_wait += (uint64_t)__popcll(wait0);
                lost_fin += (uint64_t)__popcll(sm0 & ~wait0);
                if (exhausted) lost_idle_exh += (uint64_t)__popcll(__ballot(L.phase == PH_IDLE));
                else lost_idle += (uint64_t)__popcll(__ballot(L.phase == PH_IDLE));
                if constexpr (SLOTS) ready_wait += (uint64_t)__popcll(__ballot(sst == 2));
#endif
                if (is_active(L.phase)) {
                    const V3 p = BP ? vfma(L.d, L.t, L.o) : RMR_MARCH_POINT(L);
                    if constexpr (!MAP::kCounts)
                        RMR_COUNT(P.counters, active_lanes(), (uint64_t)P.flops_static, (uint64_t)P.transc_static);
                    if constexpr (BP) {
                        int w;
                        bool cert;
                        const V2 m = MAP::eval_c(P, p, w, cert);
                        march_update<HO, false, true, true>(P, L, m, w, cert);
                    } else if constexpr (MAP::kCert && HO) {
                        int w;
                        bool cert;
                        const V2 m = MAP::eval_c(P, p, w, cert);
                        if (L.phase == PH_NORMAL) normal_update(L, m.x);
                        else march_update<HO, false, SLOTS>(P, L, m, w, cert);
                    } else {
                        const V2 m = MAP::eval(P, p);
                        if (L.phase == PH_NORMAL) normal_update(L, m.x);
                        else march_update<HO>(P, L, m);
                    }
                }
                lmaps += (uint32_t)__popcll(am);
                liters++;
                const uint64_t sm = __ballot(is_shade(L.phase));
                am = __ballot(is_active(L.phase));
#ifdef RMR_PROFILE
                sm0 = sm;
#endif
                if (!am || __popcll(sm) >= TL) break;
            }
            maps += (WCount)__builtin_amdgcn_readfirstlane(lmaps);
            iters += (WCount)__builtin_amdgcn_readfirstlane(liters);
        }
        RMR_STAMP(c2);
        if constexpr (SLOTS) {
#ifdef RMR_PROFILE
            n_outer++;
#endif
            for (;;) {
                const int st = (wv << 6) + (int)lane_now();
                const bool sh = is_shade(L.phase);
                if (__ballot(sh)) {
#ifdef RMR_PROFILE
                    n_park++;
#endif
#ifdef RMR_PROFILE
                    const bool uhit0 = L.phase == PH_HIT && L.ctr >= 0;
#endif
                    bool cheap = false;
                    if (sh) {
                        V3 nc = v3s(0.0f);
                        if (L.phase == PH_MISS) {
                            const float g = 1.0f;
                            nc = sky_color(P, L.d) * g;
                            cheap = true;
                        } else {
                            const int id = (int)L.mid;
                            int kind = MAT_NONE;
                            DMat dm{};
                            if (id >= 0 && id < P.n_mats) {
                                dm = P.dmats[id];
                                kind = dm.kind;
                            }
                            if (kind == MAT_DIFFUSE) nc = v3(dm.c[0], dm.c[1], dm.c[2]);
                            else if (kind == MAT_EMISSION) nc = v3(dm.c[0], dm.c[1], dm.c[2]) * dm.gray1;
                            cheap = kind != MAT_DIFFUSE || !(L.bounces < P.max_bounces);
                        }
                        if (cheap) {
                            const V3 res = L.color * nc;
                            store_sample(P.samp + __float_as_uint(s_slot[16][st]), make_float4(res.x, res.y, res.z, 1.0f));
                            L.phase = PH_IDLE;
                            L.e = v3s(-0.0f);
                        }
                    }
                    shaded += (WCount)__popcll(__ballot(cheap));
#ifdef RMR_PROFILE
                    {
                        const bool uh = uhit0 && (cheap || sst != 1);
                        uhits += (uint64_t)__popcll(__ballot(uh));
                        uhits_cheap += (uint64_t)__popcll(__ballot(uh && cheap));
                    }
#endif
                    const bool park = sh && !cheap && sst != 1;
                    if (__ballot(park)) {
                        if (park) {
                            const bool swap = sst == 2;
                            SlotRay r{};
                            if (swap) r = slot_read_ray(s_slot, st);
                            slot_put_event<BP>(s_slot, st, L, vfma(L.d, L.t, L.o), st);
                            L.phase = PH_IDLE;
                            if (swap) slot_start_ray(s_slot, st, L, r);
                            L.e = v3s(-0.0f);
                            sst = 1;
                        }
                        nev += (uint32_t)__popcll(__ballot(park));
                    }
                    if constexpr (OVF) {
                        const bool cand = is_shade(L.phase);
                        const uint64_t cm = __ballot(cand);
                        if (cm) {
                            const bool free_ = sst == 0;
                            const uint64_t em = __ballot(free_);
                            if (em) {
                                const int n = slot_deposits(cm, em);
                                const int rk_e = (int)__builtin_amdgcn_mbcnt_hi((uint32_t)(em >> 32), __builtin_amdgcn_mbcnt_lo((uint32_t)em, 0u));
                                if (slot_in_step(free_, rk_e, n)) {
                                    s_tab[wv][rk_e] = st & 63;
                                    sst = 1;
                                }
                                __builtin_amdgcn_wave_barrier();
                                const int rk_c = (int)__builtin_amdgcn_mbcnt_hi((uint32_t)(cm >> 32), __builtin_amdgcn_mbcnt_lo((uint32_t)cm, 0u));
                                const bool give = slot_in_step(cand, rk_c, n);
#ifdef RMR_PROFILE
                                uhits += (uint64_t)__popcll(__ballot(give && L.ctr >= 0));
#endif
// ... 45 lines not shown
                    maps += (WCount)(6 * __popcll(cm));
                    bmaps += (WCount)(6 * __popcll(cm));
#ifdef RMR_COUNT_FLOPS
                    const uint64_t bm = __ballot(mine && (__float_as_int(((const float4*)(P.dprims + E.cw))[1].z) & 0xff) == RMR_PRIM_BOX);
                    RMR_COUNT(P.counters, (uint64_t)__popcll(bm), 6 * (22 + 2), 6);
                    RMR_COUNT(P.counters, (uint64_t)__popcll(cm & ~bm), 6 * (10 + 2), 6);
#endif
                }
                if constexpr (BP) {
                    const bool mine = ev && E.ctr >= 0;
                    const uint64_t um = __ballot(mine);
                    if (um) {
                        probe_normals<true, MAP>(P, E, mine, um, s_tab[wv]);
                        maps += (WCount)(6 * __popcll(um));
                        bmaps += (WCount)(6 * __popcll(um));
                        if constexpr (!MAP::kCounts)
                            RMR_COUNT(P.counters, (uint64_t)(6 * __popcll(um)), (uint64_t)P.flops_static, (uint64_t)P.transc_static);
                    }
                    slot_get_shading(s_slot, st, E);
                }
                if (ev) {
                    shade<VAR, PROG, MATS, CERT>(P, E);
                    sst = 0;
                    if (E.phase == PH_MARCH) {
                        slot_put_ray(s_slot, st, E);
                        sst = 2;
                    }
                }
                if (__ballot(is_shade(L.phase)) == 0) break;
            }
        }
        const uint64_t smask = __ballot(is_shade(L.phase));
        const uint64_t amask2 = __ballot(is_active(L.phase));
        if (!SLOTS && smask && (__popcll(smask) >= T || amask2 == 0)) {
            shades++;
            shaded += (WCount)__popcll(smask);
            if constexpr (CERT) {
                const bool mine = L.phase == PH_HIT && L.ctr < 0;
                const uint64_t cm = __ballot(mine);
                if (cm) cert_normals(P, L, mine, cm, s_tab[wv], RMR_DTAB);
                maps += (WCount)(6 * __popcll(cm));
                bmaps += (WCount)(6 * __popcll(cm));
#ifdef RMR_COUNT_FLOPS
                const uint64_t bm = __ballot(L.phase == PH_HIT && L.ctr < 0 &&
                                             (__float_as_int(((const float4*)(P.dprims + L.cw))[1].z) & 0xff) == RMR_PRIM_BOX);
                RMR_COUNT(P.counters, (uint64_t)__popcll(bm), 6 * (22 + 2), 6);
                RMR_COUNT(P.counters, (uint64_t)__popcll(cm & ~bm), 6 * (10 + 2), 6);
#endif
            }
            if (is_shade(L.phase)) {
                uint32_t ln = 0;
                if constexpr (kSeeds) {
                    ln = lane_now();
                    L.gxt = s_rng[0][wv][ln];
                    L.gyt = s_rng[1][wv][ln];
                    L.rc = s_rng[2][wv][ln];
                }
                if constexpr (HO) {
                    L.o = vfma(L.d, L.t, L.o);
                    L.e = v3s(-0.0f);
                }
                shade<VAR, PROG, MATS, CERT>(P, L);
                if constexpr (kSeeds) s_rng[2][wv][ln] = L.rc;
            }
        }
        if (L.phase == PH_DONE) L.phase = PH_IDLE;
#ifdef RMR_PROFILE
        RMR_STAMP(c3);
        cyc[0] += c1 - c0;
        cyc[1] += c2 - c1;
        cyc[2] += c3 - c2;
#endif
        const uint64_t live = __ballot(L.phase != PH_IDLE);
        const bool last = live == 0 && exhausted && (!SLOTS || __ballot(sst != 0) == 0);
        if (last || ((maps | shaded) >> 30) != 0) {
            if (lane_now() == 0) {
                atomicAdd(P.counters + 0, (unsigned long long)maps);
                atomicAdd(P.counters + 1, (unsigned long long)iters);
                atomicAdd(P.counters + 2, (unsigned long long)shades);
                if (MAP::kCache) atomicAdd(P.counters + 3, (unsigned long long)fulls);
                atomicAdd(P.counters + 8, (unsigned long long)shaded);
                if (CERT) atomicAdd(P.counters + 14, (unsigned long long)bmaps);
                if (OVF) atomicAdd(P.counters + kCntOverflow, (unsigned long long)ovfs);
            }
            maps = iters = shades = fulls = shaded = bmaps = ovfs = 0;
        }
        if (last) break;
    }
#ifdef RMR_WAVE_TIMES
    if (lane_now() == 0) {
        const unsigned long long tn = __builtin_amdgcn_s_memrealtime();
        atomicMax(P.counters + 12, ~tn);
        atomicMax(P.counters + 13, tn);
        if (t_exh) atomicAdd(P.counters + 15, tn - t_exh);
    }
#endif
    if (lane_now() == 0) {
#ifdef RMR_PROFILE
        atomicAdd(P.counters + 4, (unsigned long long)cyc[0]);
        atomicAdd(P.counters + 5, (unsigned long long)cyc[1]);
        atomicAdd(P.counters + 6, (unsigned long long)cyc[2]);
        if (MAP::kCache) {
            atomicAdd(P.counters + 9, (unsigned long long)cyc[3]);
            atomicAdd(P.counters + kCntProfFullLanes, (unsigned long long)full_lanes);
        }
        atomicAdd(P.counters + kCntProfClaim, (unsigned long long)cyc_claim);
        atomicAdd(P.counters + kCntProfRays, (unsigned long long)cyc_rays);
        if (SLOTS) {
            atomicAdd(P.counters + kCntProfUhits, (unsigned long long)uhits);
            atomicAdd(P.counters + kCntProfUhitsCheap, (unsigned long long)uhits_cheap);
            atomicAdd(P.counters + kCntProfOuter, (unsigned long long)n_outer);
            atomicAdd(P.counters + kCntProfPark, (unsigned long long)n_park);
            atomicAdd(P.counters + kCntProfParkOvf, (unsigned long long)n_park_ovf);
            atomicAdd(P.counters + kCntProfLostFin, (unsigned long long)lost_fin);
            atomicAdd(P.counters + kCntProfLostWait, (unsigned long long)lost_wait);
            atomicAdd(P.counters + kCntProfBatchEv, (unsigned long long)batch_ev);
            atomicAdd(P.counters + kCntProfLostIdle, (unsigned long long)lost_idle);
            atomicAdd(P.counters + kCntProfLostIdleExh, (unsigned long long)lost_idle_exh);
            atomicAdd(P.counters + kCntProfReadyWait, (unsigned long long)ready_wait);
        }
        atomicAdd(P.counters + 7, (unsigned long long)(__builtin_amdgcn_s_memtime() - c_begin));
#endif
    }
}


RMR_D void fold_main(const KParams& P) {
    const int gid = blockIdx.x * blockDim.x + threadIdx.x;
    if (gid < (int)(kQueueBytes / (4 * kQueueWordStride))) ((uint32_t*)P.queue)[gid * kQueueWordStride] = 0u;
    const int tile = gid >> 6, lane = gid & 63;
    if (tile >= P.n_tiles) return;
    const TileXY txy = P.tiles[tile];
    const int px = txy.x + (lane & 7), py = txy.y + (lane >> 3);
    if (px < P.x0 || py < P.y0 || px >= P.x1 || py >= P.y1) return;
    float4* ap = P.accum + (size_t)py * P.W + px;
    float4 acc = *ap;
    const size_t plane = (size_t)P.n_tiles * 64;
    for (uint32_t k = 0; k < P.nspp; k++) {
        const float4 c = P.samp[(size_t)k * plane + (size_t)tile * 64 + lane];
        const uint32_t n = P.first_sample + k;
        if (n != 0u) {
            const float f1 = 1.0f / (float)(n + 1u);
            const float f2 = (float)n / (float)(n + 1u);
            acc.x = c.x * f1 + acc.x * f2;
            acc.y = c.y * f1 + acc.y * f2;
            acc.z = c.z * f1 + acc.z * f2;
        } else {
            acc.x = c.x; acc.y = c.y; acc.z = c.z;
        }
        acc.w = 1.0f;
    }
    *ap = acc;
}

}
```

raymarchrenderer_amd/renderer.py:

```python
import ctypes as C
import json
import math
import os
import time as _time

import numpy as np

from . import abi
from ._lib import RMRError, lib


def _fp(a):
    return a.ctypes.data_as(C.POINTER(C.c_float))


def _check(ctx, code, L=None):
    if code != abi.RMR_OK:
        msg = (L or lib()).rmr_last_error(ctx) if ctx else b""
        raise RMRError(code, (msg or b"").decode(errors="replace"))


def time_schedule(nspp, frame=0, first_sample=0):
    s = np.arange(first_sample, first_sample + nspp, dtype=np.float64)
    return (1000.0 * frame + 0.016 * s).astype(np.float32)
# ... 37 lines not shown
        if self._ctx:
            self._L.rmr_destroy(self._ctx)
            self._ctx = C.c_void_p()

    def __del__(self):
        try:
            self.close()
        except Exception:
            pass

    @property
    def ctx(self):
        return self._ctx

    @property
    def lib(self):
        return self._L

    def _chk(self, code):
        _check(self._ctx, code, self._L)

    def set_image_size(self, w, h):
        self._chk(self._L.rmr_set_image_size(self._ctx, int(w), int(h)))

    def image_size(self):
        w, h = C.c_int(), C.c_int()
        self._chk(self._L.rmr_get_image_size(self._ctx, C.byref(w), C.byref(h)))
        return w.value, h.value

    def set_params(self, params=None, **kw):
        p = params if params is not None else abi.default_params()
        for k, v in kw.items():
            setattr(p, k, v)
        self._chk(self._L.rmr_set_params(self._ctx, C.byref(p)))

    def params(self):
        p = abi.Params()
        self._chk(self._L.rmr_get_params(self._ctx, C.byref(p)))
        return p

    def set_view(self, view15):
        v = np.ascontiguousarray(view15, np.float32).reshape(15)
        parts = [np.ascontiguousarray(v[3 * i:3 * i + 3]) for i in range(5)]
        self._chk(self._L.rmr_set_view(self._ctx, *[_fp(x) for x in parts]))
        self._view = v

    def load_scene(self, scene, variant):
        if isinstance(variant, str):
            variant = abi.VARIANTS[variant]
        if isinstance(scene, dict):
            text = json.dumps(scene)
        elif isinstance(scene, str) and os.path.exists(scene):
            with open(scene, "r") as f:
                text = f.read()
        else:
            text = scene
        b = text.encode()
        self._chk(self._L.rmr_load_scene_json(self._ctx, variant, b, len(b)))
        self.variant = variant

    def load_builtin(self, variant):
        if isinstance(variant, str):
            variant = abi.VARIANTS[variant]
        self._chk(self._L.rmr_load_builtin_scene(self._ctx, variant))
        self.variant = variant

    def load_tables(self, tables):
        s = tables.to_ctypes()
        self._chk(self._L.rmr_load_scene_tables(self._ctx, C.byref(s)))
        self.variant = tables.variant

    def reload(self):
        self._chk(self._L.rmr_reload(self._ctx))

    def set_kernel(self, k):
        self._chk(self._L.rmr_set_kernel(self._ctx, int(k)))

    def set_tuning(self, shade_threshold=0, grid_per_cu=-1, samp_budget=0, park=None, slot_batch=None, lane_slots=None):
        st = int(shade_threshold)
        if not (park is None and slot_batch is None and lane_slots is None):
            p = 127 if lane_slots is False else min(64, int(park or 0))
            st |= 1 << 23 | p << 16 | min(64, int(slot_batch or 0)) << 24
        self._chk(self._L.rmr_set_tuning(self._ctx, st, int(grid_per_cu), int(samp_budget)))

    def set_grid_reserve(self, blocks):
        self._chk(self._L.rmr_set_grid_reserve(self._ctx, int(blocks)))
        self._grid_reserve = int(blocks)

    @property
    def grid_reserve(self):
        return getattr(self, "_grid_reserve", 0)

    def set_env_map(self, rgba8):
        if rgba8 is None:
            self._chk(self._L.rmr_set_env_map(self._ctx, None, 0, 0))
            return
        a = np.ascontiguousarray(rgba8, np.uint8)
        self._env = a
        self._chk(self._L.rmr_set_env_map(self._ctx, a.ctypes.data, a.shape[1], a.shape[0]))

    def set_jit(self, mode):
        self._chk(self._L.rmr_set_jit(self._ctx, int(mode)))

    def set_instrument(self, flags):
        self._chk(self._L.rmr_set_instrument(self._ctx, int(flags)))

    def set_culling(self, flags):
        self._chk(self._L.rmr_set_culling(self._ctx, int(flags)))

    def set_stream(self, hip_stream_handle):
        self._chk(self._L.rmr_set_stream(self._ctx, C.c_void_p(hip_stream_handle)))

    def render(self, time, vmin, vmax, current_sample):
        self._chk(self._L.rmr_render(self._ctx, float(time), float(vmin[0]), float(vmin[1]),
                                           float(vmax[0]), float(vmax[1]), int(current_sample)))

    def set_call_batching(self, mode):
        self._chk(self._L.rmr_set_call_batching(self._ctx, int(mode)))

    def set_launch_streams(self, n):
        self._chk(self._L.rmr_set_launch_streams(self._ctx, int(n)))

    @property
    def launch_streams(self):
        return int(self._L.rmr_get_launch_streams(self._ctx))

    def render_spp(self, times, rect=None, first_sample=0):
        times = np.ascontiguousarray(times, np.float32)
        if rect is None:
            w, h = self.image_size()
            rect = (0, 0, w, h)
        x0, y0, x1, y1 = rect
        self._chk(self._L.rmr_render_spp(self._ctx, _fp(times), x0, y0, x1, y1, int(first_sample), len(times)))

    def render_tiles(self, times, tiles_xy, tile_size, first_sample=0):
        times = np.ascontiguousarray(times, np.float32)
        t = np.ascontiguousarray(tiles_xy, np.int32).reshape(-1, 2)
        self._chk(self._L.rmr_render_tiles(self._ctx, _fp(times), t.ctypes.data_as(C.POINTER(C.c_int32)),
                                                 len(t), int(tile_size), int(first_sample), len(times)))

    def trace_samples(self, times, rect):
        times = np.ascontiguousarray(times, np.float32)
        x0, y0, x1, y1 = rect
        out = np.zeros((len(times), y1 - y0, x1 - x0, 4), np.float32)
        self._chk(self._L.rmr_trace_samples(self._ctx, _fp(times), x0, y0, x1, y1, len(times), _fp(out)))
        return out

    def set_camera_model(self, model=abi.CAMERA_VIEW, **fields):
        m = model if isinstance(model, abi.CameraModel) else abi.default_camera_model(model, **fields)
        self._chk(self._L.rmr_set_camera_model(self._ctx, C.byref(m)))

    def camera_model(self):
        m = abi.CameraModel()
        self._chk(self._L.rmr_get_camera_model(self._ctx, C.byref(m)))
        return m

    def camera_rays(self, times, rect=None):
        times = np.ascontiguousarray(times, np.float32)
        w, h = self.image_size()
        x0, y0, x1, y1 = (int(v) for v in (rect if rect is not None else (0, 0, w, h)))
        x0, y0, x1, y1 = max(x0, 0), max(y0, 0), min(x1, w), min(y1, h)
        out = np.zeros((len(times), max(y1 - y0, 0), max(x1 - x0, 0)), np.dtype(abi.RAY_DTYPE))
        self._chk(self._L.rmr_camera_rays(self._ctx, _fp(times), len(times), x0, y0, x1, y1, out.ctypes.data))
        return out

    def trace_rays(self, rays):
# ... 353 lines not shown
        w, h = self.image_size()
        out = np.zeros((h, w), np.float32)
        self._chk(self._L.rmr_read_variance(self._ctx, which, _fp(out), out.nbytes))
        return out

    def variance_device_ptr(self, which="filtered"):
        which = self._variance_plane("variance_device_ptr", which)
        return self._L.rmr_variance_device_ptr(self._ctx, which)

    def denoise_variance_images(self, A, B, hit, normal, params=None, variance=None, **kw):
        p, v = self._guided_params("denoise_variance_images", params, variance, kw)
        imgs = [np.ascontiguousarray(x, np.float32) for x in (A, B, hit, normal)]
        if imgs[0].ndim != 3 or imgs[0].shape[2] != 4 or any(x.shape != imgs[0].shape for x in imgs):
            raise ValueError("denoise_variance_images: A, B, hit and normal must be (h, w, 4) images of one shape, got %s"
                             % ", ".join(str(x.shape) for x in imgs))
        h, w = imgs[0].shape[:2]
        out = np.zeros((h, w, 4), np.float32)
        seed = np.zeros((h, w), np.float32)
        var = np.zeros((h, w), np.float32)
        self._chk(self._L.rmr_denoise_variance_images(self._ctx, _fp(imgs[0]), _fp(imgs[1]), _fp(imgs[2]), _fp(imgs[3]),
                                                       w, h, C.byref(p), C.byref(v), _fp(out), _fp(seed), _fp(var)))
        return out, seed, var

    def set_error_estimate(self, on=True):
        self._chk(self._L.rmr_set_error_estimate(self._ctx, 1 if on else 0))

    def read_half(self):
        w, h = self.image_size()
        out = np.zeros((h, w, 4), np.float32)
        self._chk(self._L.rmr_read_half_accum(self._ctx, _fp(out), out.nbytes))
        return out

    def half_device_ptr(self):
        return self._L.rmr_half_device_ptr(self._ctx)

    def tile_error(self, offset=1e-4):
        w, h = self.image_size()
        out = np.zeros(((h + 7) // 8, (w + 7) // 8), np.float32)
        self._chk(self._L.rmr_tile_error(self._ctx, float(offset), _fp(out), out.nbytes))
        return out

    def tile_error_images(self, A, B, offset=1e-4):
        A = np.ascontiguousarray(A, np.float32)
        B = np.ascontiguousarray(B, np.float32)
        if A.ndim != 3 or A.shape[2] != 4 or A.shape != B.shape:
            raise ValueError("tile_error_images: A and B must be (h, w, 4) images of one shape, got %s and %s"
                             % (A.shape, B.shape))
        h, w = A.shape[:2]
        out = np.zeros(((h + 7) // 8, (w + 7) // 8), np.float32)
        self._chk(self._L.rmr_tile_error_images(self._ctx, _fp(A), _fp(B), w, h, float(offset), _fp(out)))
        return out

    def render_adaptive(self, times, params=None, **kw):
        times = np.ascontiguousarray(times, np.float32)
        if params is not None and not isinstance(params, abi.AdaptiveParams):
            raise TypeError("render_adaptive: params must be an abi.AdaptiveParams")
        p = abi.default_adaptive_params() if params is None else abi.AdaptiveParams.from_buffer_copy(params)
        for k, v in kw.items():
            if k not in abi.ADAPTIVE_FIELDS:
                raise TypeError("render_adaptive: unknown parameter %r" % k)
            setattr(p, k, v)
        if p.max_samples == 0:
            p.max_samples = len(times)
        if p.max_samples > len(times):
            raise ValueError("render_adaptive: max_samples %d exceeds the %d seeds given" % (p.max_samples, len(times)))
        res = abi.AdaptiveResult()
        self._chk(self._L.rmr_render_adaptive(self._ctx, _fp(times), C.byref(p), C.byref(res)))
        return res

    def sample_counts(self):
        w, h = self.image_size()
        out = np.zeros(((h + 7) // 8, (w + 7) // 8), np.uint32)
        self._chk(self._L.rmr_read_sample_counts(self._ctx, out.ctypes.data_as(C.POINTER(C.c_uint32)), out.nbytes))
        return out

    def stats(self):
        s = abi.Stats()
        self._chk(self._L.rmr_get_stats(self._ctx, C.byref(s)))
        return s

    def reset_stats(self):
        self._chk(self._L.rmr_reset_stats(self._ctx))

    def counters(self):
        raw = (C.c_uint64 * 32)()
        self._chk(self._L.rmr_get_counters_n(self._ctx, raw, 32))
        return [int(v) for v in raw]


def jit_compile_scene(scene, variant, diag=None):
    if isinstance(variant, str):
        variant = abi.VARIANTS[variant]
    if scene is None:
        text = b""
    elif isinstance(scene, dict):
        text = json.dumps(scene).encode()
    elif os.path.exists(scene):
        text = open(scene, "rb").read()
    else:
        text = scene.encode()
    log = C.create_string_buffer(65536)
    rc = lib(diag=diag).rmr_jit_compile_scene(int(variant), text or None, len(text), log, len(log))
    if rc != abi.RMR_OK:
        raise RMRError(rc, log.value.decode(errors="replace"))
    return log.value.decode()


def camera_frame(view):
    v = np.ascontiguousarray(view, np.float32).reshape(15)
    out = np.zeros(9, np.float32)
    rc = lib().rmr_camera_frame(_fp(v), _fp(out))
    if rc != abi.RMR_OK:
        raise RMRError(rc, "rmr_camera_frame: degenerate view")
    return out.reshape(3, 3)


def check_camera_model(model, **fields):
    m = model if isinstance(model, abi.CameraModel) else abi.default_camera_model(model, **fields)
    return lib().rmr_check_camera_model(C.byref(m)) == abi.RMR_OK


def check_rays(rays):
    r = np.ascontiguousarray(rays, np.dtype(abi.RAY_DTYPE)).reshape(-1)
    return lib().rmr_check_rays(r.ctypes.data, len(r)) == abi.RMR_OK


def check_temporal_params(params=None, **fields):
    p = params if isinstance(params, abi.TemporalParams) else abi.default_temporal_params(**fields)
    return lib().rmr_check_temporal_params(C.byref(p)) == abi.RMR_OK


def check_bloom_params(params=None, **fields):
    p = params if isinstance(params, abi.BloomParams) else abi.default_bloom_params(**fields)
    return lib().rmr_check_bloom_params(C.byref(p)) == abi.RMR_OK


def bloom_pixels(rgba, params=None, **fields):
    p = params if isinstance(params, abi.BloomParams) else abi.default_bloom_params(**fields)
    a = np.ascontiguousarray(rgba, np.float32)
    if a.ndim != 3 or a.shape[2] != 4:
        raise ValueError("bloom_pixels: an (H, W, 4) image, got shape %r" % (a.shape,))
    out = np.zeros_like(a)
    rc = lib().rmr_bloom_pixels(C.byref(p), _fp(a), a.shape[1], a.shape[0], _fp(out))
    if rc != abi.RMR_OK:
        raise RMRError(rc, "rmr_bloom_pixels: bad params or image")
    return out


def check_tonemap_params(params=None, **fields):
    p = params if isinstance(params, abi.TonemapParams) else abi.default_tonemap_params(**fields)
    return lib().rmr_check_tonemap_params(C.byref(p)) == abi.RMR_OK


def luminance_bins(rgba):
    a = np.ascontiguousarray(rgba, np.float32).reshape(-1, 4)
    out = np.zeros(len(a), np.int32)
    rc = lib().rmr_luminance_bins(_fp(a), len(a), out.ctypes.data_as(C.POINTER(C.c_int32)))
    if rc != abi.RMR_OK:
        raise RMRError(rc, "rmr_luminance_bins")
    return out


def exposure_from_histogram(hist, l_prev=None, params=None, **fields):
    p = params if isinstance(params, abi.TonemapParams) else abi.default_tonemap_params(**fields)
    h = np.ascontiguousarray(hist, np.uint32).reshape(256)
    out = C.c_double(0.0)
    rc = lib().rmr_exposure_from_histogram(h.ctypes.data_as(C.POINTER(C.c_uint32)), C.byref(p),
                                           C.c_double(float("nan") if l_prev is None else l_prev), C.byref(out))
    if rc != abi.RMR_OK:
# ... 237 lines not shown
```

Measured before the change: 3343 Msamples/s.

## Add trailing march steps reusing winner primitive distance between full map evaluations

After each full SDF map evaluation, the march loop now takes up to a few extra cheap steps that evaluate only the winning primitive's distance, read from a copy in LDS. Each step is accepted only when a conservative bound built from the anchor distance and the travelled distance shows that no other primitive can be closer. This cuts the number of full map evaluations per ray. In exchange it adds ballot and divergence overhead, more register pressure and an LDS copy of the primitive table, and it adds counters and an API setter for the step count.

```diff
diff --git a/include/rmr.h b/include/rmr.h
--- a/include/rmr.h
+++ b/include/rmr.h
@@ -280,6 +280,7 @@
 int rmr_jit_compile_scene_rays(int variant, const char* json, size_t len, char* log, size_t loglen);
 int rmr_set_tuning(rmr_ctx* ctx, int shade_threshold, int grid_per_cu, long long samp_budget_bytes);
 int rmr_set_grid_reserve(rmr_ctx* ctx, int blocks);
+int rmr_set_trail_steps(rmr_ctx* ctx, int steps);
 int rmr_trace_samples(rmr_ctx* ctx, const float* times, int x0, int y0, int x1, int y1, uint32_t nspp, float* out);
 int rmr_abi_sizes(int32_t* out, int n);
 
diff --git a/profiles/trailing_steps_map_loop.s b/profiles/trailing_steps_map_loop.s
--- /dev/null
+++ b/profiles/trailing_steps_map_loop.s
@@ -0,0 +1,616 @@
+.LBB0_86:
+	v_cmp_gt_u32_e64 s[4:5], 3, v0
+	s_mov_b64 vcc, s[4:5]
+	s_cbranch_vccz .LBB0_124
+	s_mov_b32 s70, s54
+	s_mov_b32 s71, s55
+	s_mov_b32 s54, s76
+	s_mov_b32 s92, s69
+	s_mov_b32 s97, s66
+	v_cmp_lt_i32_e32 vcc, 4, v0
+	s_bcnt1_i32_b64 s6, vcc
+	v_readlane_b32 s7, v78, 30
+	s_add_i32 s35, s7, s6
+	s_mov_b32 s34, 0
+	s_mov_b32 s55, 0
+	s_mov_b32 s31, 0
+	s_mov_b32 s66, 0
+	s_mov_b32 s69, 0
+	s_branch .LBB0_89
+.LBB0_88:
+	s_add_i32 s66, s66, 1
+	v_cmp_lt_i32_e32 vcc, 4, v0
+	v_cmp_gt_u32_e64 s[4:5], 3, v0
+	s_cmp_lg_u64 s[4:5], 0
+	s_cselect_b64 s[6:7], -1, 0
+	s_bcnt1_i32_b64 s8, vcc
+	s_cmp_gt_u32 s35, s8
+	s_cselect_b64 s[8:9], -1, 0
+	s_and_b64 s[6:7], s[6:7], s[8:9]
+	s_and_b64 vcc, exec, s[6:7]
+	s_cbranch_vccz .LBB0_123
+.LBB0_89:
+	v_cmp_gt_u32_e32 vcc, 3, v0
+	v_mov_b32_e32 v22, 0
+	v_mov_b32_e32 v6, 0
+	v_mov_b32_e32 v7, 0
+	s_and_saveexec_b64 s[10:11], vcc
+	s_cbranch_execz .LBB0_102
+	v_fma_f32 v6, v15, v37, v18
+	v_fma_f32 v7, v16, v37, v19
+	v_fma_f32 v8, v17, v37, v14
+	v_add_f32_e32 v10, 0x3f833333, v7
+	v_add_f32_e64 v11, |v6|, -4.0
+	v_add_f32_e64 v10, |v10|, s82
+	v_add_f32_e64 v12, |v8|, -4.0
+	v_max3_f32 v13, v11, v10, v12
+	v_min_f32_e32 v13, 0, v13
+	v_max_f32_e32 v11, 0, v11
+	v_max_f32_e32 v10, 0, v10
+	v_max_f32_e32 v22, 0, v12
+	v_mul_f32_e32 v27, v22, v22
+	v_fma_f32 v33, v10, v10, v27
+	v_fmac_f32_e32 v33, v11, v11
+	v_add_f32_e32 v10, v13, v33
+	v_add_f32_e32 v11, 0x40400000, v6
+	v_add_f32_e32 v22, -1.0, v7
+	v_add_f32_e64 v11, |v11|, s82
+	v_add_f32_e64 v24, |v22|, s83
+	v_max_f32_e32 v12, v24, v12
+	v_max_f32_e32 v22, v11, v12
+	v_min_f32_e32 v22, 0, v22
+	v_max_f32_e32 v11, 0, v11
+	v_max_f32_e32 v24, 0, v24
+	v_fmac_f32_e32 v27, v24, v24
+	v_fma_f32 v32, v11, v11, v27
+	v_add_f32_e32 v11, v22, v32
+	v_max_f32_e32 v25, v10, v11
+	v_cmp_lt_f32_e32 vcc, v11, v10
+	s_nop 1
+	v_cndmask_b32_e32 v10, v10, v11, vcc
+	v_cndmask_b32_e32 v11, 0, v48, vcc
+	v_add_f32_e32 v24, 0xc0400000, v6
+	v_add_f32_e64 v26, |v24|, s82
+	v_max_f32_e32 v12, v26, v12
+	v_min_f32_e32 v24, 0, v12
+	v_max_f32_e32 v12, 0, v26
+	v_fmac_f32_e32 v27, v12, v12
+	v_add_f32_e32 v12, v24, v27
+	v_med3_f32 v28, v10, v12, v25
+	v_cmp_lt_f32_e32 vcc, v12, v10
+	s_nop 1
+	v_cndmask_b32_e32 v10, v10, v12, vcc
+	v_cndmask_b32_e32 v11, v11, v49, vcc
+	v_add_f32_e32 v12, -4.0, v7
+	v_add_f32_e64 v26, |v6|, s0
+	v_add_f32_e64 v12, |v12|, s82
+	v_add_f32_e64 v29, |v8|, s0
+	v_max3_f32 v25, v26, v12, v29
+	v_min_f32_e32 v25, 0, v25
+	v_max_f32_e32 v31, 0, v26
+	v_max_f32_e32 v12, 0, v12
+	v_max_f32_e32 v26, 0, v29
+	v_mul_f32_e32 v26, v26, v26
+	v_fmac_f32_e32 v26, v12, v12
+	v_fmac_f32_e32 v26, v31, v31
+	v_add_f32_e32 v12, v25, v26
+	v_med3_f32 v28, v10, v12, v28
+	v_cmp_lt_f32_e32 vcc, v12, v10
+	s_nop 1
+	v_cndmask_b32_e32 v10, v10, v12, vcc
+	v_cndmask_b32_e32 v29, v11, v50, vcc
+	v_cmp_lt_f32_e32 vcc, 0, v10
+	v_sqrt_f32_e32 v11, v10
+	s_nop 0
+	v_cndmask_b32_e32 v12, v10, v11, vcc
+	v_max_f32_e32 v34, 0, v10
+	v_cndmask_b32_e64 v10, v10, 0, vcc
+	v_cmp_lt_f32_e32 vcc, 0, v28
+	v_sqrt_f32_e32 v11, v28
+	s_nop 0
+	v_cndmask_b32_e32 v11, v28, v11, vcc
+	v_mul_f32_e32 v28, v8, v8
+	v_fmac_f32_e32 v28, v7, v7
+	v_fmac_f32_e32 v28, v6, v6
+	v_sqrt_f32_e32 v31, v28
+	s_nop 0
+	v_add_f32_e32 v35, -1.0, v31
+	v_med3_f32 v11, v12, v35, v11
+	v_cmp_lt_f32_e32 vcc, v35, v12
+	s_nop 1
+	v_cndmask_b32_e32 v12, v12, v35, vcc
+	v_cndmask_b32_e32 v35, v34, v28, vcc
+	v_cndmask_b32_e64 v34, v10, -1.0, vcc
+	v_cndmask_b32_e64 v10, v29, 3, vcc
+	v_sqrt_f32_e32 v29, v35
+	s_nop 0
+	v_add_u32_e32 v58, -1, v29
+	v_add_u32_e32 v59, 1, v29
+	v_fma_f32 v60, -v58, v29, v35
+	v_fma_f32 v61, -v59, v29, v35
+	v_cmp_ge_f32_e32 vcc, 0, v60
+	s_nop 1
+	v_cndmask_b32_e32 v29, v29, v58, vcc
+	v_cmp_lt_f32_e32 vcc, 0, v61
+	s_nop 1
+	v_cndmask_b32_e32 v29, v29, v59, vcc
+	v_add_f32_e32 v34, v34, v29
+	v_and_b32_e32 v29, 0x7fc00000, v10
+	v_add_f32_e64 v58, |v11|, |v12|
+	v_add_f32_e32 v58, 2.0, v58
+	v_fmamk_f32 v58, v58, 0x35800000, v45
+	v_add_u32_e32 v35, -1, v35
+	v_cmp_gt_u32_e32 vcc, s99, v35
+	v_sub_f32_e32 v35, v11, v12
+	v_cmp_ngt_f32_e64 s[6:7], v35, v58
+	s_or_b64 s[6:7], vcc, s[6:7]
+	v_cmp_ngt_f32_e32 vcc, s33, v12
+	s_or_b64 s[6:7], vcc, s[6:7]
+	s_and_saveexec_b64 s[8:9], s[6:7]
+	s_cbranch_execz .LBB0_97
+	v_sqrt_f32_e32 v29, v33
+	s_nop 0
+	v_add_u32_e32 v34, -1, v29
+	v_add_u32_e32 v35, 1, v29
+	v_fma_f32 v58, -v34, v29, v33
+	v_fma_f32 v59, -v35, v29, v33
+	v_cmp_ge_f32_e32 vcc, 0, v58
+	s_nop 1
+	v_cndmask_b32_e32 v29, v29, v34, vcc
+	v_cmp_lt_f32_e32 vcc, 0, v59
+	s_nop 1
+	v_cndmask_b32_e32 v29, v29, v35, vcc
+	v_cmp_gt_f32_e32 vcc, s78, v33
+	v_cmp_neq_f32_e64 s[6:7], 0, v33
+	s_and_b64 s[6:7], vcc, s[6:7]
+	s_and_saveexec_b64 s[48:49], s[6:7]
+	s_cbranch_execnz .LBB0_118
+.LBB0_92:
+	s_or_b64 exec, exec, s[48:49]
+	v_sqrt_f32_e32 v33, v32
+	s_nop 0
+	v_add_u32_e32 v34, -1, v33
+	v_add_u32_e32 v35, 1, v33
+	v_fma_f32 v58, -v34, v33, v32
+	v_fma_f32 v59, -v35, v33, v32
+	v_cmp_ge_f32_e32 vcc, 0, v58
+	s_nop 1
+	v_cndmask_b32_e32 v33, v33, v34, vcc
+	v_cmp_lt_f32_e32 vcc, 0, v59
+	s_nop 1
+	v_cndmask_b32_e32 v33, v33, v35, vcc
+	v_cmp_gt_f32_e32 vcc, s78, v32
+	v_cmp_neq_f32_e64 s[6:7], 0, v32
+	s_and_b64 s[6:7], vcc, s[6:7]
+	s_and_saveexec_b64 s[48:49], s[6:7]
+	s_cbranch_execnz .LBB0_119
+.LBB0_93:
+	s_or_b64 exec, exec, s[48:49]
+	v_sqrt_f32_e32 v32, v27
+	s_nop 0
+	v_add_u32_e32 v34, -1, v32
+	v_add_u32_e32 v35, 1, v32
+	v_fma_f32 v58, -v34, v32, v27
+	v_fma_f32 v59, -v35, v32, v27
+	v_cmp_ge_f32_e32 vcc, 0, v58
+	s_nop 1
+	v_cndmask_b32_e32 v32, v32, v34, vcc
+	v_cmp_lt_f32_e32 vcc, 0, v59
+	s_nop 1
+	v_cndmask_b32_e32 v32, v32, v35, vcc
+	v_cmp_gt_f32_e32 vcc, s78, v27
+	v_cmp_neq_f32_e64 s[6:7], 0, v27
+	s_and_b64 s[6:7], vcc, s[6:7]
+	s_and_saveexec_b64 s[48:49], s[6:7]
+	s_cbranch_execnz .LBB0_120
+.LBB0_94:
+	s_or_b64 exec, exec, s[48:49]
+	v_add_u32_e32 v27, -1, v31
+	v_add_u32_e32 v34, 1, v31
+	v_fma_f32 v35, -v27, v31, v28
+	v_fma_f32 v58, -v34, v31, v28
+	v_cmp_ge_f32_e32 vcc, 0, v35
+	s_nop 1
+	v_cndmask_b32_e32 v27, v31, v27, vcc
+	v_cmp_lt_f32_e32 vcc, 0, v58
+	s_nop 1
+	v_cndmask_b32_e32 v27, v27, v34, vcc
+	v_cmp_gt_f32_e32 vcc, s78, v28
+	v_cmp_neq_f32_e64 s[6:7], 0, v28
+	s_and_b64 s[6:7], vcc, s[6:7]
+	s_and_saveexec_b64 s[48:49], s[6:7]
+	s_cbranch_execnz .LBB0_121
+.LBB0_95:
+	s_or_b64 exec, exec, s[48:49]
+	v_sqrt_f32_e32 v28, v26
+	s_nop 0
+	v_add_u32_e32 v31, -1, v28
+	v_add_u32_e32 v34, 1, v28
+	v_fma_f32 v35, -v31, v28, v26
+	v_fma_f32 v58, -v34, v28, v26
+	v_cmp_ge_f32_e32 vcc, 0, v35
+	s_nop 1
+	v_cndmask_b32_e32 v28, v28, v31, vcc
+	v_cmp_lt_f32_e32 vcc, 0, v58
+	s_nop 1
+	v_cndmask_b32_e32 v28, v28, v34, vcc
+	v_cmp_gt_f32_e32 vcc, s78, v26
+	v_cmp_neq_f32_e64 s[6:7], 0, v26
+	s_and_b64 s[6:7], vcc, s[6:7]
+	s_and_saveexec_b64 s[48:49], s[6:7]
+	s_cbranch_execnz .LBB0_122
+.LBB0_96:
+	s_or_b64 exec, exec, s[48:49]
+	v_add_f32_e32 v13, v13, v29
+	v_cmp_ge_f32_e32 vcc, s36, v13
+	v_mov_b32_e32 v26, s36
+	s_nop 0
+	v_cndmask_b32_e32 v26, v26, v13, vcc
+	v_add_f32_e32 v22, v22, v33
+	v_cmp_ge_f32_e32 vcc, v26, v22
+	s_nop 1
+	v_cndmask_b32_e32 v29, v26, v22, vcc
+	v_add_f32_e32 v24, v24, v32
+	v_cmp_ge_f32_e32 vcc, v29, v24
+	s_nop 1
+	v_cndmask_b32_e32 v31, v29, v24, vcc
+	v_add_f32_e32 v27, -1.0, v27
+	v_cmp_ge_f32_e32 vcc, v31, v27
+	s_nop 1
+	v_cndmask_b32_e32 v32, v31, v27, vcc
+	v_cmp_nlt_f32_e32 vcc, s36, v13
+	s_nop 1
+	v_cndmask_b32_e64 v13, -1.0, 0, vcc
+	v_cmp_lt_f32_e32 vcc, v26, v22
+	s_nop 1
+	v_cndmask_b32_e32 v13, 1.0, v13, vcc
+	v_cmp_lt_f32_e32 vcc, v29, v24
+	s_nop 1
+	v_cndmask_b32_e32 v13, 2.0, v13, vcc
+	v_cmp_lt_f32_e32 vcc, v31, v27
+	s_nop 1
+	v_cndmask_b32_e32 v13, 0, v13, vcc
+	v_add_f32_e32 v22, v25, v28
+	v_cmp_lt_f32_e32 vcc, v32, v22
+	s_nop 1
+	v_cndmask_b32_e32 v29, v51, v13, vcc
+	v_cmp_ge_f32_e32 vcc, v32, v22
+	s_nop 1
+	v_cndmask_b32_e32 v34, v32, v22, vcc
+.LBB0_97:
+	s_or_b64 exec, exec, s[8:9]
+	v_and_b32_e32 v25, 0x7fffffff, v12
+	v_cmp_gt_f32_e32 vcc, s3, v34
+	v_cmp_ngt_f32_e64 s[6:7], s3, v34
+	v_fma_f32 v24, s37, v34, v37
+	v_add_u32_e32 v13, 1, v39
+	s_and_saveexec_b64 s[8:9], s[6:7]
+	s_xor_b64 s[48:49], exec, s[8:9]
+	s_cbranch_execz .LBB0_99
+	v_cmp_le_f32_e64 s[6:7], s36, v37
+	v_cmp_le_i32_e64 s[8:9], s38, v13
+	s_or_b64 s[8:9], s[6:7], s[8:9]
+	s_waitcnt lgkmcnt(1)
+	v_cmp_gt_f32_e64 s[6:7], v24, v38
+	s_or_b64 s[72:73], s[8:9], s[6:7]
+.LBB0_99:
+	s_or_saveexec_b64 s[50:51], s[48:49]
+	s_mov_b64 s[48:49], 0
+	s_xor_b64 exec, exec, s[50:51]
+	v_cmp_gt_f32_e64 s[6:7], s36, v37
+	v_cmp_ngt_f32_e64 s[8:9], s36, v37
+	s_and_b64 s[48:49], s[6:7], exec
+	s_andn2_b64 s[6:7], s[72:73], exec
+	s_and_b64 s[8:9], s[8:9], exec
+	s_or_b64 s[72:73], s[6:7], s[8:9]
+	s_or_b64 exec, exec, s[50:51]
+	v_max3_f32 v6, |v6|, |v7|, |v8|
+	v_mov_b32_e32 v7, s29
+	v_fmamk_f32 v6, v6, 0x37000000, v7
+	v_add_f32_e64 v7, s28, |v11|
+	v_fmamk_f32 v7, v7, 0x36000000, v45
+	v_sub_f32_e32 v7, v11, v7
+	v_sub_f32_e32 v6, v7, v6
+	v_and_b32_e32 v22, 0xff, v10
+	s_mov_b32 s6, 0x3b03126f
+	v_cmp_gt_f32_e64 s[6:7], s6, v25
+	s_mov_b32 s8, 0x3f7ffff0
+	v_fma_f32 v7, v11, s8, -v12
+	v_cmp_lt_f32_e64 s[8:9], s30, v7
+	s_and_b64 s[6:7], s[6:7], s[8:9]
+	v_mov_b32_e32 v7, s36
+	v_cndmask_b32_e64 v7, v24, v7, s[72:73]
+	v_cndmask_b32_e32 v8, v7, v37, vcc
+	v_cndmask_b32_e64 v7, v36, -1.0, s[72:73]
+	v_cndmask_b32_e64 v36, v7, v29, s[48:49]
+	v_bitop3_b32 v7, v10, s93, v10 bitop3:0x3f
+	v_cndmask_b32_e64 v7, 0, v7, s[6:7]
+	v_cndmask_b32_e64 v39, v13, v7, s[48:49]
+	v_cndmask_b32_e64 v0, v0, 6, s[72:73]
+	v_cndmask_b32_e64 v0, v0, 5, s[48:49]
+	v_mov_b32_e32 v7, v37
+	v_mov_b32_e32 v37, v8
+.LBB0_102:
+	s_or_b64 exec, exec, s[10:11]
+	s_bcnt1_i32_b64 s4, s[4:5]
+	s_add_i32 s69, s69, s4
+	s_andn2_b64 vcc, exec, s[84:85]
+	s_cbranch_vccnz .LBB0_88
+	v_cmp_gt_u32_e64 s[10:11], 3, v0
+	v_lshlrev_b32_e32 v8, 1, v22
+	v_not_b32_e32 v22, v22
+	s_mov_b32 s76, s67
+	s_branch .LBB0_106
+.LBB0_104:
+	v_cmp_gt_u32_e32 vcc, 3, v0
+	s_and_b64 s[10:11], s[10:11], vcc
+	s_add_i32 s76, s76, -1
+	s_cmp_eq_u32 s76, 0
+	s_cselect_b64 s[4:5], -1, 0
+.LBB0_105:
+	s_andn2_b64 vcc, exec, s[4:5]
+	s_cbranch_vccz .LBB0_88
+.LBB0_106:
+	v_cndmask_b32_e64 v10, 0, 1, s[10:11]
+	v_cmp_ne_u32_e64 s[4:5], 0, v10
+	s_mov_b64 vcc, s[4:5]
+	s_cbranch_vccz .LBB0_115
+	v_fma_f32 v28, v15, v37, v18
+	v_fma_f32 v29, v16, v37, v19
+	v_fma_f32 v31, v17, v37, v14
+	v_cndmask_b32_e64 v10, 0, v8, s[10:11]
+	v_lshlrev_b32_e32 v10, 4, v10
+	ds_read_b128 v[24:27], v10 offset:26624
+	ds_read_b128 v[10:13], v10 offset:26640
+	s_waitcnt lgkmcnt(0)
+	v_cmp_eq_u32_sdwa vcc, v12, v52 src0_sel:BYTE_0 src1_sel:DWORD
+	s_nop 1
+	v_cndmask_b32_e32 v11, 0, v11, vcc
+	v_cndmask_b32_e32 v10, 0, v10, vcc
+	v_cndmask_b32_e32 v12, 0, v27, vcc
+	v_cndmask_b32_e64 v27, v27, 0, vcc
+	v_sub_f32_e32 v24, v28, v24
+	v_sub_f32_e32 v25, v29, v25
+	v_sub_f32_e32 v26, v31, v26
+	v_sub_f32_e64 v12, |v24|, v12
+	v_sub_f32_e64 v10, |v25|, v10
+	v_sub_f32_e64 v11, |v26|, v11
+	v_max_f32_e32 v24, 0, v12
+	v_max_f32_e32 v25, 0, v10
+	v_max_f32_e32 v26, 0, v11
+	v_mul_f32_e32 v26, v26, v26
+	v_fmac_f32_e32 v26, v25, v25
+	v_fmac_f32_e32 v26, v24, v24
+	v_max3_f32 v10, v12, v10, v11
+	v_min_f32_e32 v10, 0, v10
+	v_sqrt_f32_e32 v11, v26
+	s_nop 0
+	v_add_u32_e32 v12, -1, v11
+	v_add_u32_e32 v24, 1, v11
+	v_fma_f32 v25, -v12, v11, v26
+	v_fma_f32 v32, -v24, v11, v26
+	v_cmp_ge_f32_e32 vcc, 0, v25
+	s_nop 1
+	v_cndmask_b32_e32 v11, v11, v12, vcc
+	v_cmp_lt_f32_e32 vcc, 0, v32
+	s_nop 1
+	v_cndmask_b32_e32 v11, v11, v24, vcc
+	v_add_f32_e32 v10, v10, v11
+	v_sub_f32_e32 v10, v10, v27
+	v_max3_f32 v12, |v28|, |v29|, |v31|
+	v_add_f32_e32 v11, v28, v29
+	v_add_f32_e32 v11, v31, v11
+	v_sub_f32_e32 v11, v11, v11
+	v_cmp_eq_f32_e32 vcc, 0, v11
+	v_sub_f32_e32 v11, v37, v7
+	v_mul_f32_e32 v11, 0xbf800004, v11
+	v_add_f32_e32 v11, v6, v11
+	v_add_f32_e32 v12, 0x3b03126f, v12
+	v_mov_b32_e32 v24, s29
+	v_fmamk_f32 v12, v12, 0x37000000, v24
+	v_cmp_eq_f32_e64 s[6:7], 0, v26
+	v_cmp_le_f32_e64 s[8:9], s78, v26
+	s_or_b64 s[6:7], s[6:7], s[8:9]
+	s_and_b64 s[6:7], vcc, s[6:7]
+	v_sub_f32_e32 v24, v11, v12
+	v_cmp_gt_f32_e32 vcc, v24, v10
+	s_and_b64 s[6:7], s[6:7], vcc
+	v_cmp_gt_f32_e32 vcc, s33, v10
+	s_and_b64 s[94:95], vcc, s[6:7]
+	s_and_b64 s[72:73], s[10:11], s[94:95]
+	v_cndmask_b32_e64 v24, 0, 1, s[72:73]
+	v_cmp_ne_u32_e32 vcc, 0, v24
+	s_cbranch_vccz .LBB0_116
+	s_and_saveexec_b64 s[88:89], s[72:73]
+	s_cbranch_execz .LBB0_114
+	v_cmp_gt_f32_e64 s[6:7], s3, v10
+	v_cmp_ngt_f32_e64 s[8:9], s3, v10
+	v_fma_f32 v25, s37, v10, v37
+	v_add_u32_e32 v24, 1, v39
+	s_and_saveexec_b64 s[10:11], s[8:9]
+	s_xor_b64 s[50:51], exec, s[10:11]
+	v_cmp_le_f32_e64 s[8:9], s36, v37
+	v_cmp_le_i32_e64 s[10:11], s38, v24
+	s_or_b64 s[10:11], s[8:9], s[10:11]
+	v_cmp_gt_f32_e64 s[8:9], v25, v38
+	s_or_b64 s[48:49], s[10:11], s[8:9]
+	s_or_saveexec_b64 s[52:53], s[50:51]
+	s_mov_b64 s[50:51], 0
+	s_xor_b64 exec, exec, s[52:53]
+	v_cmp_gt_f32_e64 s[8:9], s36, v37
+	v_cmp_ngt_f32_e64 s[10:11], s36, v37
+	s_and_b64 s[50:51], s[8:9], exec
+	s_andn2_b64 s[8:9], s[48:49], exec
+	s_and_b64 s[10:11], s[10:11], exec
+	s_or_b64 s[48:49], s[8:9], s[10:11]
+	s_or_b64 exec, exec, s[52:53]
+	v_fmamk_f32 v12, v12, 0x40400000, v46
+	v_fma_f32 v12, |v11|, s98, v12
+	v_sub_f32_e32 v11, v11, v12
+	v_cmp_gt_f32_e64 s[8:9], v11, v10
+	s_and_b64 s[8:9], s[8:9], s[94:95]
+	v_mov_b32_e32 v10, s36
+	v_cndmask_b32_e64 v10, v25, v10, s[48:49]
+	v_cndmask_b32_e64 v37, v10, v37, s[6:7]
+	v_cndmask_b32_e64 v10, v36, -1.0, s[48:49]
+	v_cndmask_b32_e64 v36, v10, v13, s[50:51]
+	v_cndmask_b32_e64 v10, 0, v22, s[8:9]
+	v_cndmask_b32_e64 v39, v24, v10, s[50:51]
+	v_cndmask_b32_e64 v0, v0, 6, s[48:49]
+	v_cndmask_b32_e64 v0, v0, 5, s[50:51]
+.LBB0_114:
+	s_or_b64 exec, exec, s[88:89]
+	s_bcnt1_i32_b64 s6, vcc
+	s_add_i32 s69, s69, s6
+	s_add_i32 s31, s31, s6
+	s_mov_b64 s[6:7], -1
+	s_mov_b64 s[10:11], s[72:73]
+	s_branch .LBB0_117
+.LBB0_115:
+	s_mov_b64 vcc, exec
+	s_mov_b64 s[4:5], -1
+	s_cbranch_execz .LBB0_104
+	s_branch .LBB0_105
+.LBB0_116:
+	s_mov_b64 s[6:7], 0
+.LBB0_117:
+	s_add_i32 s55, s55, 1
+	s_bcnt1_i32_b64 s4, s[4:5]
+	s_add_i32 s34, s34, s4
+	s_andn2_b64 vcc, exec, s[6:7]
+	s_mov_b64 s[4:5], -1
+	s_cbranch_vccnz .LBB0_105
+	s_branch .LBB0_104
+.LBB0_118:
+	v_cmp_gt_f32_e32 vcc, s78, v33
+	v_mul_f32_e32 v29, 0x4f800000, v33
+	s_nop 0
+	v_cndmask_b32_e32 v29, v33, v29, vcc
+	v_sqrt_f32_e32 v33, v29
+	s_nop 0
+	v_add_u32_e32 v34, -1, v33
+	v_fma_f32 v35, -v34, v33, v29
+	v_cmp_ge_f32_e64 s[6:7], 0, v35
+	s_nop 1
+	v_cndmask_b32_e64 v34, v33, v34, s[6:7]
+	v_add_u32_e32 v35, 1, v33
+	v_fma_f32 v33, -v35, v33, v29
+	v_cmp_lt_f32_e64 s[6:7], 0, v33
+	s_nop 1
+	v_cndmask_b32_e64 v33, v34, v35, s[6:7]
+	v_mul_f32_e32 v34, 0x37800000, v33
+	v_cndmask_b32_e32 v33, v33, v34, vcc
+	v_mov_b32_e32 v34, 0x260
+	v_cmp_class_f32_e32 vcc, v29, v34
+	s_nop 1
+	v_cndmask_b32_e32 v29, v33, v29, vcc
+	s_branch .LBB0_92
+.LBB0_119:
+	v_cmp_gt_f32_e32 vcc, s78, v32
+	v_mul_f32_e32 v33, 0x4f800000, v32
+	s_nop 0
+	v_cndmask_b32_e32 v32, v32, v33, vcc
+	v_sqrt_f32_e32 v33, v32
+	s_nop 0
+	v_add_u32_e32 v34, -1, v33
+	v_fma_f32 v35, -v34, v33, v32
+	v_cmp_ge_f32_e64 s[6:7], 0, v35
+	s_nop 1
+	v_cndmask_b32_e64 v34, v33, v34, s[6:7]
+	v_add_u32_e32 v35, 1, v33
+	v_fma_f32 v33, -v35, v33, v32
+	v_cmp_lt_f32_e64 s[6:7], 0, v33
+	s_nop 1
+	v_cndmask_b32_e64 v33, v34, v35, s[6:7]
+	v_mul_f32_e32 v34, 0x37800000, v33
+	v_cndmask_b32_e32 v33, v33, v34, vcc
+	v_mov_b32_e32 v34, 0x260
+	v_cmp_class_f32_e32 vcc, v32, v34
+	s_nop 1
+	v_cndmask_b32_e32 v33, v33, v32, vcc
+	s_branch .LBB0_93
+.LBB0_120:
+	v_cmp_gt_f32_e32 vcc, s78, v27
+	v_mul_f32_e32 v32, 0x4f800000, v27
+	s_nop 0
+	v_cndmask_b32_e32 v27, v27, v32, vcc
+	v_sqrt_f32_e32 v32, v27
+	s_nop 0
+	v_add_u32_e32 v34, -1, v32
+	v_fma_f32 v35, -v34, v32, v27
+	v_cmp_ge_f32_e64 s[6:7], 0, v35
+	s_nop 1
+	v_cndmask_b32_e64 v34, v32, v34, s[6:7]
+	v_add_u32_e32 v35, 1, v32
+	v_fma_f32 v32, -v35, v32, v27
+	v_cmp_lt_f32_e64 s[6:7], 0, v32
+	s_nop 1
+	v_cndmask_b32_e64 v32, v34, v35, s[6:7]
+	v_mul_f32_e32 v34, 0x37800000, v32
+	v_cndmask_b32_e32 v32, v32, v34, vcc
+	v_mov_b32_e32 v34, 0x260
+	v_cmp_class_f32_e32 vcc, v27, v34
+	s_nop 1
+	v_cndmask_b32_e32 v32, v32, v27, vcc
+	s_branch .LBB0_94
+.LBB0_121:
+	v_cmp_gt_f32_e32 vcc, s78, v28
+	v_mul_f32_e32 v27, 0x4f800000, v28
+	s_nop 0
+	v_cndmask_b32_e32 v27, v28, v27, vcc
+	v_sqrt_f32_e32 v28, v27
+	s_nop 0
+	v_add_u32_e32 v31, -1, v28
+	v_fma_f32 v34, -v31, v28, v27
+	v_cmp_ge_f32_e64 s[6:7], 0, v34
+	s_nop 1
+	v_cndmask_b32_e64 v31, v28, v31, s[6:7]
+	v_add_u32_e32 v34, 1, v28
+	v_fma_f32 v28, -v34, v28, v27
+	v_cmp_lt_f32_e64 s[6:7], 0, v28
+	s_nop 1
+	v_cndmask_b32_e64 v28, v31, v34, s[6:7]
+	v_mul_f32_e32 v31, 0x37800000, v28
+	v_cndmask_b32_e32 v28, v28, v31, vcc
+	v_mov_b32_e32 v31, 0x260
+	v_cmp_class_f32_e32 vcc, v27, v31
+	s_nop 1
+	v_cndmask_b32_e32 v27, v28, v27, vcc
+	s_branch .LBB0_95
+.LBB0_122:
+	v_cmp_gt_f32_e32 vcc, s78, v26
+	v_mul_f32_e32 v28, 0x4f800000, v26
+	s_nop 0
+	v_cndmask_b32_e32 v26, v26, v28, vcc
+	v_sqrt_f32_e32 v28, v26
+	s_nop 0
+	v_add_u32_e32 v31, -1, v28
+	v_fma_f32 v34, -v31, v28, v26
+	v_cmp_ge_f32_e64 s[6:7], 0, v34
+	s_nop 1
+	v_cndmask_b32_e64 v31, v28, v31, s[6:7]
+	v_add_u32_e32 v34, 1, v28
+	v_fma_f32 v28, -v34, v28, v26
+	v_cmp_lt_f32_e64 s[6:7], 0, v28
+	s_nop 1
+	v_cndmask_b32_e64 v28, v31, v34, s[6:7]
+	v_mul_f32_e32 v31, 0x37800000, v28
+	v_cndmask_b32_e32 v28, v28, v31, vcc
+	v_mov_b32_e32 v31, 0x260
+	v_cmp_class_f32_e32 vcc, v26, v31
+	s_nop 1
+	v_cndmask_b32_e32 v28, v28, v26, vcc
+	s_branch .LBB0_96
+.LBB0_123:
+	s_add_i32 s86, s69, s86
+	s_add_i32 s1, s66, s1
+	s_add_i32 s79, s31, s79
+	s_add_i32 s65, s55, s65
+	s_add_i32 s64, s34, s64
+	s_mov_b32 s66, s97
+	s_mov_b32 s69, s92
+	s_mov_b32 s76, s54
+	s_mov_b32 s55, s71
+	s_mov_b32 s97, 0xd800000
+	s_mov_b32 s92, 0x82fffffe
+	s_mov_b32 s54, s70
diff --git a/raymarchrenderer_amd/_lib.py b/raymarchrenderer_amd/_lib.py
--- a/raymarchrenderer_amd/_lib.py
+++ b/raymarchrenderer_amd/_lib.py
@@ -16,7 +16,7 @@
     "rmr_render_spp", "rmr_render_tiles", "rmr_read_accum", "rmr_write_accum",
     "rmr_accum_device_ptr", "rmr_bind_accum", "rmr_save_bmp", "rmr_encode_bmp",
     "rmr_save_accum", "rmr_load_accum", "rmr_sync", "rmr_get_stats", "rmr_reset_stats", "rmr_get_section_cycles", "rmr_get_counters", "rmr_get_counters_n", "rmr_set_culling",
-    "rmr_set_kernel", "rmr_set_tuning", "rmr_set_grid_reserve", "rmr_trace_samples", "rmr_abi_sizes", "rmr_set_jit", "rmr_set_instrument", "rmr_jit_compile_scene", "rmr_set_env_map",
+    "rmr_set_kernel", "rmr_set_tuning", "rmr_set_grid_reserve", "rmr_set_trail_steps", "rmr_trace_samples", "rmr_abi_sizes", "rmr_set_jit", "rmr_set_instrument", "rmr_jit_compile_scene", "rmr_set_env_map",
     "rmr_scene_compile", "rmr_scene_view", "rmr_scene_free", "rmr_display", "rmr_display_device",
     "rmr_srgb_thresholds", "rmr_candidate_grid", "rmr_set_call_batching", "rmr_set_launch_streams", "rmr_get_launch_streams",
     "rmr_default_denoise_params", "rmr_render_guides", "rmr_read_guide", "rmr_guide_device_ptr", "rmr_denoise",
@@ -108,6 +108,7 @@
         "rmr_set_kernel": (C.c_int, [vp, C.c_int]),
         "rmr_set_tuning": (C.c_int, [vp, C.c_int, C.c_int, C.c_longlong]),
         "rmr_set_grid_reserve": (C.c_int, [vp, C.c_int]),
+        "rmr_set_trail_steps": (C.c_int, [vp, C.c_int]),
         "rmr_set_call_batching": (C.c_int, [vp, C.c_int]),
         "rmr_set_launch_streams": (C.c_int, [vp, C.c_int]),
         "rmr_get_launch_streams": (C.c_int, [vp]),
diff --git a/raymarchrenderer_amd/csrc/rmr_api.cpp b/raymarchrenderer_amd/csrc/rmr_api.cpp
--- a/raymarchrenderer_amd/csrc/rmr_api.cpp
+++ b/raymarchrenderer_amd/csrc/rmr_api.cpp
@@ -23,6 +23,7 @@
 #include "rmr_camera.hpp"
 #include "rmr_ray_check.h"
 #include "rmr_jit.hpp"
+#include "rmr_trail_rule.h"
 #include "scene.hpp"
 #include "temporal.hpp"
 #include "tonemap.hpp"
@@ -173,6 +174,7 @@
     int refill_threshold = -1;
     int lane_slots = -1;
     int park_threshold = 0, slot_threshold = 0;
+    int trail_steps = -1;
     int jit_slots = -1;
     int full_threshold = 40 | (8 << 8);
     int cull = RMR_CULL_ESCAPE | RMR_CULL_NPC | RMR_CULL_APPROX | RMR_CULL_EYE;
@@ -511,6 +513,8 @@
     k.park_t = facts.park_t();
     k.slot_t = facts.slot_t();
     k.slot_t_small = facts.slot_t_small();
+    k.trail = facts.trail;
+    k.trail_k = facts.trail_k();
     c->jit_loaded.push_back(k);
     jk = k;
     ready = true;
@@ -948,7 +952,9 @@
             const bool small = P.n_units < (uint64_t)gp.grid * (uint64_t)(jk.block / 64) * (uint64_t)jk.chunk *
                                                (uint64_t)rmr::JitFacts::kSlotSmallClaims;
             const int batch = c->slot_threshold > 0 ? c->slot_threshold : (small ? jk.slot_t_small : jk.slot_t);
-            P.shade_threshold = park | (batch << 8);
+            int trail = !jk.trail ? 0 : (c->trail_steps >= 0 ? c->trail_steps : jk.trail_k);
+            if (!(P.step_mult > 0.0f) || !std::isfinite(P.step_mult)) trail = 0;
+            P.shade_threshold = park | (batch << 8) | (std::min(trail, (int)rmr::kTrailMaxSteps) << 16);
             P.refill_threshold = refill_for(c->refill_threshold, park);
         }
         if ((r = submit_launch(c, P, S, use_jit, gp.grid, rays ? c->d_rays : nullptr, !rl))) return r;
@@ -1712,6 +1718,13 @@
     }
     if (grid_per_cu >= 0) c->grid_per_cu = grid_per_cu;
     if (samp_budget_bytes > 0) c->samp_budget = (size_t)samp_budget_bytes;
+    return RMR_OK;
+}
+
+int rmr_set_trail_steps(rmr_ctx* c, int steps) {
+    if (!c || steps < -1 || steps > rmr::kTrailMaxSteps) return RMR_E_INVALID;
+    RMR_FLUSH(c);
+    c->trail_steps = steps;
     return RMR_OK;
 }
 
diff --git a/raymarchrenderer_amd/csrc/rmr_internal.h b/raymarchrenderer_amd/csrc/rmr_internal.h
--- a/raymarchrenderer_amd/csrc/rmr_internal.h
+++ b/raymarchrenderer_amd/csrc/rmr_internal.h
@@ -40,8 +40,11 @@
 constexpr size_t kQueueBytes = 8192;
 constexpr int kQueueWordStride = 32;
 
-constexpr int kCounterSlots = 32;
+constexpr int kCounterSlots = 34;
 constexpr int kCntOverflow = 16;
+constexpr int kCntTrailSteps = 31;
+constexpr int kCntTrailPasses = 32;
+constexpr int kCntTrailLanes = 33;
 constexpr int kCntProfClaim = 17;
 constexpr int kCntProfRays = 18;
 constexpr int kCntProfUhits = 19;
diff --git a/raymarchrenderer_amd/csrc/rmr_jit.cpp b/raymarchrenderer_amd/csrc/rmr_jit.cpp
--- a/raymarchrenderer_amd/csrc/rmr_jit.cpp
+++ b/raymarchrenderer_amd/csrc/rmr_jit.cpp
@@ -107,6 +107,7 @@
 constexpr int kSlotsDefault = 1;
 constexpr int kBatchProbesDefault = 1;
 constexpr int kSlotOverflowDefault = 1;
+constexpr int kTrailDefault = 1;
 
 std::string var_decls() {
     std::string d = "    V3 nv0 = v3s(0.0f)";
@@ -155,6 +156,7 @@
     bool sched_mc = false;
     int fast_waves = 0;
     bool am_direct = false;
+    int trail = 0;
     const bool inline_map = s.prims.size() <= kMaxInlinePrims;
     bool has_mb = false;
     for (const rmr_prim& q : s.prims) has_mb = has_mb || q.type == RMR_PRIM_MANDELBULB;
@@ -229,6 +231,18 @@
     cert = approx && !prog && s.variant != RMR_VARIANT_RM2 && s.prims.size() <= 256;
     if (const char* e = RMR_ENV("RMR_JIT_CERT")) cert = cert && std::atoi(e) != 0;
     for (const rmr_prim& q : s.prims) cert = cert && am_packable(q.mat_id);
+    {
+        int sl = slots;
+        if (sl < 0) {
+            sl = kSlotsDefault;
+            if (const char* e = RMR_ENV("RMR_JIT_SLOTS")) sl = std::atoi(e) != 0;
+        }
+        int bp = kBatchProbesDefault;
+        if (const char* e = RMR_ENV("RMR_JIT_BPROBES")) bp = std::atoi(e) != 0;
+        int tr = kTrailDefault;
+        if (const char* e = RMR_ENV("RMR_JIT_TRAIL")) tr = std::atoi(e);
+        if (cert && s.variant == RMR_VARIANT_RM1 && !prog && sl != 0 && bp != 0 && (tr == 1 || tr == 2)) trail = tr;
+    }
     o << "struct JitMap {\n    static constexpr bool kCache = false;\n    static constexpr bool kCounts = false;\n"
       << "    static constexpr bool kStepped = " << (stepped ? "RMR_MB_STEPPED" : "false") << ";\n"
       << "    static constexpr bool kCert = " << (cert ? "true" : "false") << ";\n";
@@ -256,7 +270,10 @@
         if (cert)
             o << "    static RMR_D V2 eval(const KParams& P, V3 p) {\n        int w;\n        bool c;\n"
               << "        return eval_c(P, p, w, c);\n    }\n"
-              << "    static RMR_D V2 eval_c(const KParams& P, V3 p, int& w, bool& cert) {\n        AMin m;\n";
+              << (trail ? "    static RMR_D V2 eval_c(const KParams& P, V3 p, int& w, bool& cert) {\n        float s2;\n"
+                          "        return eval_t(P, p, w, cert, s2);\n    }\n"
+                          "    static RMR_D V2 eval_t(const KParams& P, V3 p, int& w, bool& cert, float& s2) {\n        AMin m;\n"
+                        : "    static RMR_D V2 eval_c(const KParams& P, V3 p, int& w, bool& cert) {\n        AMin m;\n");
         else
             o << "    static RMR_D V2 eval(const KParams& P, V3 p) {\n        AMin m;\n";
         if (any_loaded) o << "        CPrim* pr = (CPrim*)P.prims;\n";
@@ -297,6 +314,7 @@
         o << "        V2 d = " << (cert ? "am_result_packed" : "am_result") << "(P, m);\n"
           << "        const bool amb = !am_unique(m, " << r2 << ") | am_far(P, m);\n";
         if (cert) o << "        w = am_w_of(m.id);\n        cert = am_normal_cert(P, m);\n";
+        if (cert && trail) o << "        s2 = m.s2;\n";
         bool ambcount = false;
         if (const char* e = RMR_ENV("RMR_JIT_AMBCOUNT")) ambcount = std::atoi(e) != 0;
         if (ambcount) {
@@ -447,6 +465,10 @@
     if (const char* e = RMR_ENV("RMR_JIT_OVERFLOW")) overflow = std::atoi(e) != 0;
     if (slots_on && overflow) src.insert(src.find('\n') + 1, "#define RMR_SLOT_OVERFLOW 1\n");
     if (facts) facts->overflow = slots_on && overflow != 0;
+    const bool trail_on = slots_on && bprobes && trail != 0;
+    if (trail_on && trail == 1 && s.prims.size() <= 8) src.insert(src.find('\n') + 1, "#define RMR_TRAIL_LDS 1\n");
+    if (trail_on) src.insert(src.find('\n') + 1, "#define RMR_TRAIL_STEPS 1\n");
+    if (facts) facts->trail = trail_on;
     if (am_direct) src.insert(src.find('\n') + 1, "#ifndef RMR_AM_DIRECT\n#define RMR_AM_DIRECT 1\n#endif\n");
     if (sched_mc && fast_waves)
         src.insert(src.find('\n') + 1, "#ifndef RMR_FAST_WAVES\n#define RMR_FAST_WAVES " + std::to_string(fast_waves) + "\n#endif\n");
diff --git a/raymarchrenderer_amd/csrc/rmr_jit.hpp b/raymarchrenderer_amd/csrc/rmr_jit.hpp
--- a/raymarchrenderer_amd/csrc/rmr_jit.hpp
+++ b/raymarchrenderer_amd/csrc/rmr_jit.hpp
@@ -28,6 +28,8 @@
     bool slots = false;
     int park_t = 0, slot_t = 0;
     int slot_t_small = 0;
+    bool trail = false;
+    int trail_k = 0;
 };
 
 struct JitFacts {
@@ -35,6 +37,8 @@
     bool cache = false, general = false, prog = false, cert = false;
     bool slots_ok = false, slots = false;
     bool overflow = false;
+    bool trail = false;
+    int trail_k() const { return trail ? 2 : 0; }
     int chunk() const { return (cache || slots) ? 64 : 128; }
     int park_t() const { return 8; }
     int slot_t() const { return overflow ? 48 : 32; }
diff --git a/raymarchrenderer_amd/csrc/rmr_trace.h b/raymarchrenderer_amd/csrc/rmr_trace.h
--- a/raymarchrenderer_amd/csrc/rmr_trace.h
+++ b/raymarchrenderer_amd/csrc/rmr_trace.h
@@ -5,6 +5,7 @@
 #include "rmr_math.h"
 #include "rmr_internal.h"
 #include "rmr_slot_rule.h"
+#include "rmr_trail_rule.h"
 
 namespace rmr {
 
@@ -1988,6 +1989,23 @@
 #ifndef RMR_SLOT_OVERFLOW
 #define RMR_SLOT_OVERFLOW 0
 #endif
+#ifndef RMR_TRAIL_STEPS
+#define RMR_TRAIL_STEPS 0
+#endif
+#ifndef RMR_TRAIL_LDS
+#define RMR_TRAIL_LDS 0
+#endif
+constexpr int kTrailLdsPrims = 8;
+RMR_D float trail_dist(const float4* q, V3 p, float& mid, float& len2, bool& box) {
+    const float4 a = q[0], b = q[1];
+    box = (__float_as_int(b.z) & 0xff) == RMR_PRIM_BOX;
+    const V3 h = box ? v3(a.w, b.x, b.y) : v3s(0.0f);
+    const float rad = box ? 0.0f : a.w;
+    mid = b.w;
+    const V3 qq = vabs(p - v3(a.x, a.y, a.z)) - h;
+    len2 = trail_len2(qq.x, qq.y, qq.z);
+    return (trail_k(qq.x, qq.y, qq.z) + sqrt_cr_big(len2)) - rad;
+}
 #ifndef RMR_EYE_CHUNK
 #define RMR_EYE_CHUNK 1
 #endif
@@ -2004,11 +2022,14 @@
     mbs.i = -1;
     mbs.fin = false;
     WCount maps = 0, iters = 0, shades = 0, fulls = 0, shaded = 0, bmaps = 0, ovfs = 0;
+    WCount tsteps = 0, tpasses = 0, tlanes = 0;
     constexpr bool SLOTS = RMR_LANE_SLOTS && PERSIST && VAR == RMR_VARIANT_RM1 && CERT && MAP::kCert && !MAP::kCache &&
                            !MAP::kStepped && !RAYS;
     constexpr bool BP = SLOTS && RMR_BATCH_PROBES;
     constexpr bool EYEC = SLOTS && RMR_EYE_CHUNK;
     constexpr bool OVF = SLOTS && RMR_SLOT_OVERFLOW;
+    constexpr bool TRAIL = BP && RMR_TRAIL_STEPS;
+    constexpr bool TRAIL_LDS = TRAIL && RMR_TRAIL_LDS;
     constexpr uint32_t CHUNK = MAP::kCache ? RMR_CHUNK_CACHE : (SLOTS ? RMR_CHUNK_SLOTS : RMR_CHUNK);
     const uint32_t n_units = (uint32_t)P.n_units;
     const uint32_t CK = P.chunk_units - 1u < CHUNK ? P.chunk_units : CHUNK;
@@ -2027,6 +2048,7 @@
     }
     const int T = P.shade_threshold, TR = P.refill_threshold;
     const int PK = T & 0xff, T2 = (T >> 8) & 0xff;
+    const int KT = TRAIL ? (T >> 16) & 3 : 0;
     int sst = 0;
     uint32_t nev = 0;
     const bool eye1 = HO && !MAP::kCache && !RAYS && P.eye_step != 0;
@@ -2083,6 +2105,12 @@
 #define RMR_PRIM_DIST(k, p, mid, j) (dp_lds ? prim_dist_tab(s_dp + kTabStep * (k), p, mid, j) : prim_dist(P, k, p, mid, j))
     static_assert(!RMR_NPC_TAB_SOA || MAP::kCache, "an SoA table kernel reads dtab as the LDS copy only");
 #define RMR_DTAB (dp_lds ? (const float4*)s_dp : (const float4*)P.dprims)
+    __shared__ float4 s_tp[TRAIL_LDS ? 2 * kTrailLdsPrims : 1];
+    if constexpr (TRAIL_LDS) {
+        for (int i = (int)threadIdx.x; i < 2 * P.n_prims && i < 2 * kTrailLdsPrims; i += (int)blockDim.x)
+            s_tp[i] = ((const float4*)P.dprims)[i];
+        __syncthreads();
+    }
     const int wv = __builtin_amdgcn_readfirstlane((threadIdx.x >> 6) & 3);
     uint32_t chunk_base = 0;
 #ifdef RMR_WAVE_TIMES
@@ -2374,6 +2402,7 @@
         } else if (amask) {
             uint64_t am = amask;
             uint32_t lmaps = 0, liters = 0;
+            uint32_t ltsteps = 0, ltpasses = 0, ltlanes = 0;
             const int TL = SLOTS ? __popcll(__ballot(is_shade(L.phase))) + PK : T;
 #ifdef RMR_PROFILE
             const uint64_t wait0 = __ballot(is_shade(L.phase));
@@ -2387,11 +2416,22 @@
                 else lost_idle += (uint64_t)__popcll(__ballot(L.phase == PH_IDLE));
                 if constexpr (SLOTS) ready_wait += (uint64_t)__popcll(__ballot(sst == 2));
 #endif
+                float tr_anchor = 0.0f, tr_t0 = 0.0f;
+                int tr_w = 0;
                 if (is_active(L.phase)) {
                     const V3 p = BP ? vfma(L.d, L.t, L.o) : RMR_MARCH_POINT(L);
                     if constexpr (!MAP::kCounts)
                         RMR_COUNT(P.counters, active_lanes(), (uint64_t)P.flops_static, (uint64_t)P.transc_static);
-                    if constexpr (BP) {
+                    if constexpr (TRAIL) {
+                        int w;
+                        bool cert;
+                        float s2;
+                        const V2 m = MAP::eval_t(P, p, w, cert, s2);
+                        tr_anchor = trail_anchor(s2, P.am_r2, npc_eps(P, p));
+                        tr_t0 = L.t;
+                        tr_w = w;
+                        march_update<HO, false, true, true>(P, L, m, w, cert);
+                    } else if constexpr (BP) {
                         int w;
                         bool cert;
                         const V2 m = MAP::eval_c(P, p, w, cert);
@@ -2410,6 +2450,36 @@
                 }
                 lmaps += (uint32_t)__popcll(am);
                 liters++;
+                if constexpr (TRAIL) {
+                    bool q = is_active(L.phase) && !L.inside;
+                    for (int k = 0; k < KT; k++, q = q && is_active(L.phase)) {
+                        const uint64_t qm = __ballot(q);
+                        if (!qm) break;
+                        const V3 p = vfma(L.d, L.t, L.o);
+                        float mid, len2;
+                        bool box;
+                        const float F = trail_dist((TRAIL_LDS ? (const float4*)s_tp : (const float4*)P.dprims) + 2 * (q ? tr_w : 0),
+                                                   p, mid, len2, box);
+                        const TrailStep ts = trail_rule(tr_anchor, tr_t0, L.t, trail_linf(p.x, p.y, p.z), trail_finite(p.x, p.y, p.z),
+                                                        F, len2, P.npc_eps0, P.am_dmax);
+                        const bool ok = q && ts.accept;
+                        const uint64_t um = __ballot(ok);
+                        ltpasses++;
+                        ltlanes += (uint32_t)__popcll(qm);
+                        if (!um) break;
+#ifdef RMR_COUNT_FLOPS
+                        {
+                            const uint64_t nb = (uint64_t)__popcll(__ballot(ok && box));
+                            RMR_COUNT(P.counters, (uint64_t)__popcll(um) - nb, 10 + 2, 1);
+                            RMR_COUNT(P.counters, nb, 22 + 2, 1);
+                        }
+#endif
+                        if (ok) march_update<HO, false, true, true>(P, L, v2(F, mid), tr_w, ts.cert);
+                        q = ok;
+                        lmaps += (uint32_t)__popcll(um);
+                        ltsteps += (uint32_t)__popcll(um);
+                    }
+                }
                 const uint64_t sm = __ballot(is_shade(L.phase));
                 am = __ballot(is_active(L.phase));
 #ifdef RMR_PROFILE
@@ -2419,6 +2489,11 @@
             }
             maps += (WCount)__builtin_amdgcn_readfirstlane(lmaps);
             iters += (WCount)__builtin_amdgcn_readfirstlane(liters);
+            if constexpr (TRAIL) {
+                tsteps += (WCount)__builtin_amdgcn_readfirstlane(ltsteps);
+                tpasses += (WCount)__builtin_amdgcn_readfirstlane(ltpasses);
+                tlanes += (WCount)__builtin_amdgcn_readfirstlane(ltlanes);
+            }
         }
         RMR_STAMP(c2);
         if constexpr (SLOTS) {
@@ -2630,8 +2705,14 @@
                 atomicAdd(P.counters + 8, (unsigned long long)shaded);
                 if (CERT) atomicAdd(P.counters + 14, (unsigned long long)bmaps);
                 if (OVF) atomicAdd(P.counters + kCntOverflow, (unsigned long long)ovfs);
+                if (TRAIL) {
+                    atomicAdd(P.counters + kCntTrailSteps, (unsigned long long)tsteps);
+                    atomicAdd(P.counters + kCntTrailPasses, (unsigned long long)tpasses);
+                    atomicAdd(P.counters + kCntTrailLanes, (unsigned long long)tlanes);
+                }
             }
             maps = iters = shades = fulls = shaded = bmaps = ovfs = 0;
+            tsteps = tpasses = tlanes = 0;
         }
         if (last) break;
     }
diff --git a/raymarchrenderer_amd/csrc/rmr_trail_rule.h b/raymarchrenderer_amd/csrc/rmr_trail_rule.h
--- /dev/null
+++ b/raymarchrenderer_amd/csrc/rmr_trail_rule.h
@@ -0,0 +1,48 @@
+#pragma once
+#ifndef __HIPCC_RTC__
+#include <math.h>
+#endif
+
+#if defined(__HIPCC__) || defined(__HIPCC_RTC__)
+#define RMR_TRAIL_HD __host__ __device__ inline
+#else
+#define RMR_TRAIL_HD inline
+#endif
+
+namespace rmr {
+
+constexpr float kTrailProbeDelta = 0.0010001f;
+constexpr int kTrailMaxSteps = 3;
+
+RMR_TRAIL_HD float trail_linf(float x, float y, float z) { return fmaxf(fabsf(x), fmaxf(fabsf(y), fabsf(z))); }
+RMR_TRAIL_HD float trail_eps(float linf, float eps0) { return fmaf(linf, 0x1p-17f, eps0); }
+RMR_TRAIL_HD bool trail_finite(float x, float y, float z) {
+    const float s = (x + y) + z;
+    return s - s == 0.0f;
+}
+RMR_TRAIL_HD float trail_anchor(float s2, float r2, float eps_p0) {
+    return (s2 - fmaf(fabsf(s2) + r2, 0x1p-19f, 0x1p-39f)) - eps_p0;
+}
+RMR_TRAIL_HD float trail_k(float qx, float qy, float qz) { return fminf(fmaxf(qx, fmaxf(qy, qz)), 0.0f); }
+RMR_TRAIL_HD float trail_len2(float qx, float qy, float qz) {
+    const float ox = fmaxf(qx, 0.0f), oy = fmaxf(qy, 0.0f), oz = fmaxf(qz, 0.0f);
+    return fmaf(ox, ox, fmaf(oy, oy, oz * oz));
+}
+
+struct TrailStep {
+    bool accept;
+    bool cert;
+};
+RMR_TRAIL_HD TrailStep trail_rule(float anchor, float t0, float t, float linf, bool fin, float F, float len2, float eps0,
+                                  float am_dmax) {
+    const float delta = (t - t0) * (1.0f + 0x1p-21f);
+    const float b = anchor - delta;
+    const float eps = trail_eps(linf + 0.002f, eps0);
+    const bool big = (len2 == 0.0f) | (len2 >= 0x1p-96f);
+    TrailStep r;
+    r.accept = fin & big & (b - eps > F) & (F < am_dmax);
+    r.cert = r.accept & (b - fmaf(fabsf(b), 0x1p-20f, fmaf(3.0f, eps, 2.0f * kTrailProbeDelta)) > F);
+    return r;
+}
+
+}
diff --git a/raymarchrenderer_amd/renderer.py b/raymarchrenderer_amd/renderer.py
--- a/raymarchrenderer_amd/renderer.py
+++ b/raymarchrenderer_amd/renderer.py
@@ -143,6 +143,9 @@
             p = 127 if lane_slots is False else min(64, int(park or 0))
             st |= 1 << 23 | p << 16 | min(64, int(slot_batch or 0)) << 24
         self._chk(self._L.rmr_set_tuning(self._ctx, st, int(grid_per_cu), int(samp_budget)))
+
+    def set_trail_steps(self, steps):
+        self._chk(self._L.rmr_set_trail_steps(self._ctx, int(steps)))
 
     def set_grid_reserve(self, blocks):
         self._chk(self._L.rmr_set_grid_reserve(self._ctx, int(blocks)))
@@ -662,9 +665,9 @@
     def reset_stats(self):
         self._chk(self._L.rmr_reset_stats(self._ctx))
 
-    def counters(self):
-        raw = (C.c_uint64 * 32)()
-        self._chk(self._L.rmr_get_counters_n(self._ctx, raw, 32))
+    def counters(self, n=32):
+        raw = (C.c_uint64 * n)()
+        self._chk(self._L.rmr_get_counters_n(self._ctx, raw, n))
         return [int(v) for v in raw]
 
 
```

After: 3579 Msamples/s, median of 6. 7.1% higher.
